# RohanDoshi2018/ZeroshotSemanticSegmentation

Hardware: AMD Instinct MI355X
Metric: train_Mpixels_per_sec (higher is better)
Workload: dtype bf16; 1 GPU; PASCAL-Context 512x512 phase 1: FCN32s (the reference has no FCN8s) + 300-d pixel projection, 512x512, K=59 (49 seen / 10 unseen), Adam lr 1e-5, train step fwd+cosine loss+infer_lbl+bwd+optimizer; per_gpu_batch=8, global_batch=8, head=fused-from-coarse, parallelism=dp1

## Files before the change

include/szn.h:

```cpp
#ifndef SZN_H_
#define SZN_H_
#include <stddef.h>
#include <stdint.h>
#ifdef __cplusplus
extern "C" {
#endif

typedef void* szn_stream_t;

enum { SZN_OK = 0, SZN_ERR_ARG = -1, SZN_ERR_LAUNCH = -2, SZN_ERR_UNSUPPORTED = -3 };
enum { SZN_F32 = 0, SZN_BF16 = 1, SZN_F16 = 2, SZN_BF16X3 = 3 };

#define SZN_MAX_CLASSES 256
typedef struct szn_class_set {
    uint64_t w[4];
} szn_class_set;

const char* szn_last_error(void);
const char* szn_last_kernel(void);
const char* szn_prev_kernel(void);
int szn_version(void);
int szn_knob_count(void);
const char* szn_knob_name(int i);
typedef struct {
    char name[128];
    char arch[32];
    int compute_units;
    int wavefront;
    int lds_bytes_per_block;
    int64_t hbm_bytes;
    int clock_mhz;
} szn_device_info_t;
int szn_device_info(int device, szn_device_info_t* out );
int szn_stream_create_cu_mask(int n_words, const uint32_t* mask , szn_stream_t* out );
int szn_stream_destroy(szn_stream_t stream);

typedef struct szn_call_result {
    int colsum_rows;
    float work_fraction;
} szn_call_result_t;

typedef struct {
    int dtype;
    int B, Hi, Wi, Ci;
    int Ho, Wo, Co;
    int KH, KW, pad;
    int ldi, ldo, ldg;
    int relu;
    int out_f32;
    void* workspace;
    size_t workspace_bytes;
    float* colsum;
    void* pool_out;
    float* colsum_slab;
    int colsum_slab_rows;
    void* pool_code;
    int pool_only;
    int cb_on;
    int cb_rect[4];
    int cb_const[4];
    int reserved_cus;
    void* dw_lp;
    int dw_lp_dtype;
    szn_call_result_t* result;
} szn_conv_desc_t;

int szn_conv2d_fwd(const szn_conv_desc_t* d, const void* in, const void* w, const float* bias,
                   const void* gate, const float* chan_scale, void* out, szn_stream_t stream);

int szn_pack_weight_dgrad(int dtype, int Co, int KH, int KW, int Ci, const void* w, void* wT,
                          szn_stream_t stream);
int szn_pack_weight_dgrad_batch(int dtype, int n, const void* const* w, void* const* wT, const int* Co, const int* K,
                                const int* Ci, szn_stream_t stream);

int szn_conv2d_dgrad(const szn_conv_desc_t* d, const void* dout, const void* wT, const void* gate,
                     const float* chan_scale, void* din, szn_stream_t stream);
int szn_conv2d_dgrad_border_region(const szn_conv_desc_t* d, int region[8]);
int szn_conv2d_dgrad_border_finish(const szn_conv_desc_t* d, const void* dout, const void* wT, const void* gate,
                                   const float* skip_sum, float* colsum, void* workspace, szn_stream_t stream);

size_t szn_conv2d_dgrad_gemm_workspace_bytes(const szn_conv_desc_t* d);
int szn_conv2d_dgrad_gemm(const szn_conv_desc_t* d, const void* dout, const void* wG, void* din,
                          szn_stream_t stream);
int szn_conv2d_dgrad_gemm_native_supported(const szn_conv_desc_t* d);
size_t szn_conv2d_dgrad_gemm_native_workspace_bytes(const szn_conv_desc_t* d);
int szn_conv2d_dgrad_gemm_native(const szn_conv_desc_t* d, const void* dout, const void* w, void* din,
                                 szn_stream_t stream);

int szn_conv2d_wgrad(const szn_conv_desc_t* d, const void* in, const void* dout, float* dw,
                     int accumulate, szn_stream_t stream);
typedef struct szn_adam_args {
    float* param; float* exp_avg; float* exp_avg_sq;
    void* w_lp; int w_lp_dtype;
    float lr, beta1, beta2, eps, weight_decay;
    int step;
    float grad_scale;
    int grad_optional;
} szn_adam_args_t;
int szn_conv2d_wgrad_adam_supported(const szn_conv_desc_t* d);
int szn_conv2d_wgrad_adam(const szn_conv_desc_t* d, const void* x, const void* dout, float* dw,
                          const szn_adam_args_t* opt, szn_stream_t stream);

int szn_bias_grad(int dtype, long M, int Co, int ldd, const void* dout, float* db, int accumulate,
                  szn_stream_t stream);
int szn_bias_grad_slab(int dtype, long M, int Co, int ldd, const void* dout, float* db, int accumulate,
                       float* colsum_slab, int colsum_slab_rows, int* colsum_rows_out , szn_stream_t stream);
int szn_colsum_reduce_batch(int n, const float* const* slabs, const int* rows, const int* C, float* const* out,
                            szn_stream_t stream);

int szn_gemm_proj_fwd(int dtype, long M, int K, int N, int ldo, const void* x, const void* w,
                      const float* bias, float* out_f32, szn_stream_t stream);
int szn_gemm_proj_dgrad(int dtype, long M, int K, int N, int ldd, const void* dout, const void* wT,
                        const void* gate, const float* chan_scale, void* dx, szn_stream_t stream);
int szn_gemm_proj_wgrad(int dtype, long M, int K, int N, int ldd, const void* x, const void* dout,
                        float* dw, int accumulate, szn_stream_t stream);

int szn_conv1_1_fwd(int dtype, int B, int H, int W, int pad, const float* x_nchw, const float* w,
                    const float* bias, void* out, szn_stream_t stream);
int szn_conv1_1_fwd_c(int dtype, int B, int H, int W, int pad, const float* x_nchw, const float* w,
                      const float* bias, void* out, const int cut[8], szn_stream_t stream);
int szn_conv1_1_wgrad_c(int dtype, int B, int H, int W, int pad, const float* x_nchw, const void* dout, float* dw,
                        int accumulate, void* workspace, const int cut[8], szn_stream_t stream);
size_t szn_conv1_1_wgrad_workspace_bytes(int dtype, int B, int H, int W, int pad);
int szn_conv1_1_wgrad(int dtype, int B, int H, int W, int pad, const float* x_nchw,
                      const void* dout, float* dw, float* db, int accumulate, void* workspace,
                      szn_stream_t stream);
int szn_conv1_1_wgrad_reads(int dtype, int B, int H, int W, int pad, int rect[4]);

int szn_maxpool2x2_ceil_fwd(int dtype, int B, int Hi, int Wi, int C, const void* in, void* out,
                            szn_stream_t stream);
int szn_maxpool2x2_ceil_bwd(int dtype, int B, int Hi, int Wi, int C, const void* in,
                            const void* out, const void* dout, void* din, float* colsum ,
                            float* colsum_slab , int colsum_slab_rows,
                            int* colsum_rows_out , szn_stream_t stream);
int szn_maxpool2x2_ceil_fwd_code(int dtype, int B, int Hi, int Wi, int C, const void* in, void* out, void* code ,
                                 szn_stream_t stream);
int szn_maxpool2x2_ceil_bwd_code(int dtype, int B, int Hi, int Wi, int C, const void* code, const void* dout, void* din,
                                 float* colsum, float* colsum_slab, int colsum_slab_rows, int* colsum_rows_out, szn_stream_t stream);
int szn_maxpool2x2_ceil_bwd_code_gather(int dtype, int B, int Hi, int Wi, int C, const void* code, const void* dsrc, int Hs, int Ws,
                                        const int* ytab, const int* xtab, void* din, float* colsum, float* colsum_slab,
                                        int colsum_slab_rows, int* colsum_rows_out, szn_stream_t stream);
int szn_maxpool2x2_ceil_bwd_code_cb(int dtype, int B, int Hi, int Wi, int C, const void* code, const void* dout, void* din,
                                    float* colsum, float* colsum_slab, int colsum_slab_rows, int* colsum_rows_out, const int* skip_regions,
                                    int n_regions, float* skip_sum, float* skip_slab, szn_stream_t stream);
int szn_conv2d_wgrad_cb_region(const szn_conv_desc_t* d, int region[8]);

int szn_bilinear_up32_crop_fwd(int B, int h, int w, int E, int ldc, int c0, int H, int W, int crop,
                               const float* coarse, float* score_nchw, szn_stream_t stream);
int szn_bilinear_up32_crop_bwd(int B, int h, int w, int E, int ldc, int c0, int H, int W, int crop,
                               const float* dscore_nchw, float* dcoarse, szn_stream_t stream);

int szn_bilinear_up_crop_fwd(int stride, int B, int h, int w, int E, int ldc, int c0, int H, int W, int crop,
                             const float* coarse, float* score_nchw, szn_stream_t stream);
int szn_bilinear_up_crop_bwd(int stride, int B, int h, int w, int E, int ldc, int c0, int H, int W, int crop,
                             const float* dscore_nchw, float* dcoarse, szn_stream_t stream);
int szn_bilinear_up2_nhwc_fwd(int B, int h, int w, int C, int ld, const float* in, float* out, szn_stream_t stream);
int szn_bilinear_up2_nhwc_bwd(int B, int h, int w, int C, int ld, const float* dout, float* din, szn_stream_t stream);

int szn_deconv64s32_fwd(int B, int h, int w, int C, int ldc, int c0, int H, int W, int crop,
                        const float* coarse, const float* weight, float* out_nchw,
                        szn_stream_t stream);
int szn_deconv64s32_dgrad(int B, int h, int w, int C, int ldc, int c0, int H, int W, int crop,
                          const float* dout_nchw, const float* weight, float* dcoarse,
                          szn_stream_t stream);
int szn_deconv64s32_wgrad(int B, int h, int w, int C, int ldc, int c0, int H, int W, int crop,
                          const float* coarse, const float* dout_nchw, float* dweight,
                          int accumulate, szn_stream_t stream);

size_t szn_seenmask_head_workspace_bytes(int B, int h, int w, int H, int W, int crop);
int szn_seenmask_head(int B, int h, int w, int ldc, int c0, int H, int W, int crop, const float* coarse,
                      const float* weight, const int64_t* target, int n_class, uint64_t seen_bits, float* loss,
                      float* stats, int64_t* conf, int64_t* pred, float* dscore2, float* dweight, void* workspace,
                      szn_stream_t stream);
int szn_seenmask_head_k(int B, int h, int w, int ldc, int c0, int H, int W, int crop, const float* coarse,
                        const float* weight, const int64_t* target, int n_class, const szn_class_set* seen, float* loss,
                        float* stats, int64_t* conf, int64_t* pred, float* dscore2, float* dweight, void* workspace,
                        szn_stream_t stream);
int szn_seenmask_margin(int B, int h, int w, int ldc, int c0, int H, int W, int crop,
                        const float* coarse, const float* weight, float* margin, szn_stream_t stream);
size_t szn_seenmask_score_wgrad_workspace_bytes(long M, int F);
int szn_seenmask_score_wgrad(int dtype, long M, int F, int ldf, const void* feat, const float* dscore2, float* dw,
                             float* db, void* workspace, szn_stream_t stream);

size_t szn_loss_workspace_bytes(int B, int H, int W);
int szn_cosine_loss_fwd(int B, int E, int H, int W, int K, const float* score,
                        const int64_t* target, const float* embed, const float* target_embed,
                        float* loss, float* stats, void* workspace, szn_stream_t stream);
int szn_cosine_loss_bwd(int B, int E, int H, int W, int K, const float* score,
                        const int64_t* target, const float* embed, const float* target_embed,
                        const float* stats, const float* gout, float* dscore, szn_stream_t stream);
int szn_mse_loss_fwd(int B, int E, int H, int W, int K, const float* score, const int64_t* target,
                     const float* embed, const float* target_embed, float* loss, float* stats,
                     void* workspace, szn_stream_t stream);
int szn_mse_loss_bwd(int B, int E, int H, int W, int K, const float* score, const int64_t* target,
                     const float* embed, const float* target_embed, const float* stats,
                     const float* gout, float* dscore, szn_stream_t stream);
int szn_ce2d_fwd(int B, int C, int H, int W, const float* score, const int64_t* target, const float* weight,
                 int size_average, float* loss, float* stats, int64_t* pred, void* workspace, szn_stream_t stream);
int szn_ce2d_bwd(int B, int C, int H, int W, const float* score, const int64_t* target, const float* weight,
                 int size_average, const float* stats, const float* gout, float* dscore, szn_stream_t stream);

int szn_embed_argmax(int B, int E, int H, int W, int K, const float* score, const float* embed,
                     int mode, uint64_t unseen_bits, const float* seenmask, const int64_t* target,
                     int64_t* pred, szn_stream_t stream);
int szn_embed_argmax_k(int B, int E, int H, int W, int K, const float* score, const float* embed,
                       int mode, const szn_class_set* unseen, const float* seenmask, const int64_t* target,
                       int64_t* pred, szn_stream_t stream);

int szn_confusion_hist(long npix, int K, const int64_t* label_true, const int64_t* label_pred,
                       uint64_t unseen_bits, int64_t* hist, szn_stream_t stream);
int szn_confusion_hist_k(long npix, int K, const int64_t* label_true, const int64_t* label_pred,
                         const szn_class_set* unseen, int64_t* hist, szn_stream_t stream);

size_t szn_fused_head_workspace_bytes(int B, int h, int w, int E, int K);
int szn_fused_head(int B, int h, int w, int E, int ldc, int c0, int H, int W, int crop, int K,
                   const float* coarse, const float* embed, const int64_t* target,
                   float* loss, float* stats, int64_t* pred, int dcoarse_dtype, void* dcoarse,
                   void* workspace, szn_stream_t stream);
int szn_fused_head_strided(int stride, int B, int h, int w, int E, int ldc, int c0, int H, int W, int crop, int K,
                           const float* coarse, const float* embed, const int64_t* target, float* loss, float* stats,
                           int64_t* pred, int dcoarse_dtype, void* dcoarse, void* workspace, szn_stream_t stream);
int szn_fused_head_prepare(int E, int K, const float* embed, void* workspace, szn_stream_t stream);
int szn_fused_head_prepared(int stride, int B, int h, int w, int E, int ldc, int c0, int H, int W, int crop, int K,
                            const float* coarse, const float* embed, const int64_t* target, float* loss, float* stats,
                            int64_t* pred, int dcoarse_dtype, void* dcoarse, void* workspace, szn_stream_t stream);
int szn_fused_head_grouped(int stride, int B, int h, int w, int E, int ldc, int c0, int H, int W, int crop, int K,
                           const float* coarse, const float* embed, const int64_t* target, const szn_class_set* unseen,
                           int group_mode, const int64_t* group_map, float* loss, float* stats, int64_t* pred,
                           int dcoarse_dtype, void* dcoarse, void* workspace, szn_stream_t stream);
// ... 161 lines not shown
```

zeroshotsemanticsegmentation_amd/_lib.py:

```python
import ctypes as C
import os

import torch

_HERE = os.path.dirname(os.path.abspath(__file__))
LIB_PATH = os.environ.get("SZN_LIB_PATH") or os.path.join(_HERE, "lib", "libszn_hip.so")

SZN_F32, SZN_BF16, SZN_F16 = 0, 1, 2
SZN_BF16X3 = 3


class SznError(RuntimeError):
    pass


class CallResult(C.Structure):
    _fields_ = [("colsum_rows", C.c_int), ("work_fraction", C.c_float)]


class ConvDesc(C.Structure):
    _fields_ = [(n, C.c_int) for n in (
        "dtype", "B", "Hi", "Wi", "Ci", "Ho", "Wo", "Co", "KH", "KW", "pad", "ldi", "ldo", "ldg", "relu", "out_f32")] + [
        ("workspace", C.c_void_p), ("workspace_bytes", C.c_size_t), ("colsum", C.c_void_p), ("pool_out", C.c_void_p),
        ("colsum_slab", C.c_void_p), ("colsum_slab_rows", C.c_int), ("pool_code", C.c_void_p), ("pool_only", C.c_int),
        ("cb_on", C.c_int), ("cb_rect", C.c_int * 4), ("cb_const", C.c_int * 4), ("reserved_cus", C.c_int),
        ("dw_lp", C.c_void_p), ("dw_lp_dtype", C.c_int), ("result", C.POINTER(CallResult))]

    def __init__(self, *a, **kw):
        super().__init__(*a, **kw)
        self.res = CallResult(0, 1.0)
        self.result = C.pointer(self.res)


class DeviceInfo(C.Structure):
    _fields_ = [("name", C.c_char * 128), ("arch", C.c_char * 32), ("compute_units", C.c_int),
                ("wavefront", C.c_int), ("lds_bytes_per_block", C.c_int), ("hbm_bytes", C.c_int64),
                ("clock_mhz", C.c_int)]


class AdamArgs(C.Structure):
    _fields_ = [("param", C.c_void_p), ("exp_avg", C.c_void_p), ("exp_avg_sq", C.c_void_p), ("w_lp", C.c_void_p),
                ("w_lp_dtype", C.c_int), ("lr", C.c_float), ("beta1", C.c_float), ("beta2", C.c_float), ("eps", C.c_float),
                ("weight_decay", C.c_float), ("step", C.c_int), ("grad_scale", C.c_float), ("grad_optional", C.c_int)]


MAX_CLASSES = 256
AUG_NPARAM = 9


class ClassSet(C.Structure):
    _fields_ = [("w", C.c_uint64 * 4)]


def class_set(classes):
    cs = ClassSet()
    any_ = False
    for k in classes or []:
        k = int(k)
        if not 0 <= k < MAX_CLASSES:
            raise SznError("class index %d outside [0, %d)" % (k, MAX_CLASSES))
        cs.w[k >> 6] |= 1 << (k & 63)
        any_ = True
    return C.byref(cs) if any_ else None


MS_MAX_VIEWS = 16
CALIB_MAX_GAMMAS = 64
SEEN_SWEEP_MAX_TAUS = 64
PSEUDO_BINS = 1024
OHEM_BINS = 1024


class MsView(C.Structure):
    _fields_ = [("coarse", C.c_void_p)] + [(n, C.c_int) for n in ("h", "w", "ldc", "c0", "Hs", "Ws", "flip")]


_P, _I, _L, _F, _U64, _SZ, _I64 = C.c_void_p, C.c_int, C.c_long, C.c_float, C.c_uint64, C.c_size_t, C.c_int64
_D = C.POINTER(ConvDesc)
_IP = C.POINTER(C.c_int)
_CS = C.POINTER(ClassSet)
_MV = C.POINTER(MsView)
_FP = C.POINTER(C.c_float)

SIGNATURES = {
    "szn_last_error": (C.c_char_p, []),
    "szn_last_kernel": (C.c_char_p, []),
    "szn_prev_kernel": (C.c_char_p, []),
    "szn_version": (_I, []),
    "szn_knob_count": (_I, []),
    "szn_knob_name": (C.c_char_p, [_I]),
    "szn_device_info": (_I, [_I, C.POINTER(DeviceInfo)]),
    "szn_stream_create_cu_mask": (_I, [_I, C.POINTER(C.c_uint32), C.POINTER(C.c_void_p)]),
    "szn_stream_destroy": (_I, [C.c_void_p]),
    "szn_conv2d_fwd": (_I, [_D, _P, _P, _P, _P, _P, _P, _P]),
    "szn_pack_weight_dgrad": (_I, [_I, _I, _I, _I, _I, _P, _P, _P]),
    "szn_pack_weight_dgrad_batch": (_I, [_I, _I, _P, _P, _P, _P, _P, _P]),
    "szn_conv2d_dgrad": (_I, [_D, _P, _P, _P, _P, _P, _P]),
    "szn_conv2d_dgrad_border_region": (_I, [_D, _P]),
    "szn_conv2d_dgrad_border_finish": (_I, [_D, _P, _P, _P, _P, _P, _P, _P]),
    "szn_conv2d_dgrad_gemm_workspace_bytes": (C.c_size_t, [_D]),
    "szn_conv2d_dgrad_gemm": (_I, [_D, _P, _P, _P, _P]),
    "szn_conv2d_dgrad_gemm_native_supported": (_I, [_D]),
    "szn_conv2d_dgrad_gemm_native_workspace_bytes": (C.c_size_t, [_D]),
    "szn_conv2d_dgrad_gemm_native": (_I, [_D, _P, _P, _P, _P]),
    "szn_conv2d_wgrad": (_I, [_D, _P, _P, _P, _I, _P]),
    "szn_conv2d_wgrad_adam_supported": (_I, [_D]),
    "szn_conv2d_wgrad_adam": (_I, [_D, _P, _P, _P, C.POINTER(AdamArgs), _P]),
    "szn_bias_grad": (_I, [_I, _L, _I, _I, _P, _P, _I, _P]),
    "szn_bias_grad_slab": (_I, [_I, _L, _I, _I, _P, _P, _I, _P, _I, _IP, _P]),
    "szn_colsum_reduce_batch": (_I, [_I, _P, _P, _P, _P, _P]),
    "szn_gemm_proj_fwd": (_I, [_I, _L, _I, _I, _I, _P, _P, _P, _P, _P]),
    "szn_gemm_proj_dgrad": (_I, [_I, _L, _I, _I, _I, _P, _P, _P, _P, _P, _P]),
    "szn_gemm_proj_wgrad": (_I, [_I, _L, _I, _I, _I, _P, _P, _P, _I, _P]),
    "szn_conv1_1_fwd": (_I, [_I, _I, _I, _I, _I, _P, _P, _P, _P, _P]),
    "szn_conv1_1_fwd_c": (_I, [_I, _I, _I, _I, _I, _P, _P, _P, _P, _P, _P]),
    "szn_conv1_1_wgrad_c": (_I, [_I, _I, _I, _I, _I, _P, _P, _P, _I, _P, _P, _P]),
    "szn_conv1_1_wgrad_workspace_bytes": (_SZ, [_I, _I, _I, _I, _I]),
    "szn_conv1_1_wgrad": (_I, [_I, _I, _I, _I, _I, _P, _P, _P, _P, _I, _P, _P]),
    "szn_conv1_1_wgrad_reads": (_I, [_I, _I, _I, _I, _I, C.POINTER(C.c_int)]),
    "szn_maxpool2x2_ceil_fwd": (_I, [_I, _I, _I, _I, _I, _P, _P, _P]),
    "szn_maxpool2x2_ceil_bwd": (_I, [_I, _I, _I, _I, _I, _P, _P, _P, _P, _P, _P, _I, _IP, _P]),
    "szn_maxpool2x2_ceil_fwd_code": (_I, [_I, _I, _I, _I, _I, _P, _P, _P, _P]),
    "szn_maxpool2x2_ceil_bwd_code": (_I, [_I, _I, _I, _I, _I, _P, _P, _P, _P, _P, _I, _IP, _P]),
    "szn_maxpool2x2_ceil_bwd_code_gather": (_I, [_I, _I, _I, _I, _I, _P, _P, _I, _I, _P, _P, _P, _P, _P, _I, _IP, _P]),
    "szn_maxpool2x2_ceil_bwd_code_cb": (_I, [_I, _I, _I, _I, _I, _P, _P, _P, _P, _P, _I, _IP, _P, _I, _P, _P, _P]),
    "szn_conv2d_wgrad_cb_region": (_I, [_D, _P]),
    "szn_bilinear_up32_crop_fwd": (_I, [_I] * 9 + [_P, _P, _P]),
    "szn_bilinear_up32_crop_bwd": (_I, [_I] * 9 + [_P, _P, _P]),
    "szn_bilinear_up_crop_fwd": (_I, [_I] * 10 + [_P, _P, _P]),
    "szn_bilinear_up_crop_bwd": (_I, [_I] * 10 + [_P, _P, _P]),
    "szn_bilinear_up2_nhwc_fwd": (_I, [_I] * 5 + [_P, _P, _P]),
    "szn_bilinear_up2_nhwc_bwd": (_I, [_I] * 5 + [_P, _P, _P]),
    "szn_deconv64s32_fwd": (_I, [_I] * 9 + [_P, _P, _P, _P]),
    "szn_deconv64s32_dgrad": (_I, [_I] * 9 + [_P, _P, _P, _P]),
    "szn_deconv64s32_wgrad": (_I, [_I] * 9 + [_P, _P, _P, _I, _P]),
    "szn_seenmask_head_workspace_bytes": (_SZ, [_I] * 6),
    "szn_seenmask_head": (_I, [_I] * 8 + [_P, _P, _P, _I, _U64] + [_P] * 8),
    "szn_seenmask_head_k": (_I, [_I] * 8 + [_P, _P, _P, _I, _CS] + [_P] * 8),
    "szn_seenmask_margin": (_I, [_I] * 8 + [_P, _P, _P, _P]),
    "szn_seenmask_score_wgrad_workspace_bytes": (_SZ, [_L, _I]),
    "szn_seenmask_score_wgrad": (_I, [_I, _L, _I, _I, _P, _P, _P, _P, _P, _P]),
    "szn_loss_workspace_bytes": (_SZ, [_I, _I, _I]),
    "szn_cosine_loss_fwd": (_I, [_I] * 5 + [_P] * 8),
    "szn_cosine_loss_bwd": (_I, [_I] * 5 + [_P] * 8),
    "szn_mse_loss_fwd": (_I, [_I] * 5 + [_P] * 8),
    "szn_mse_loss_bwd": (_I, [_I] * 5 + [_P] * 8),
    "szn_ce2d_fwd": (_I, [_I] * 4 + [_P, _P, _P, _I, _P, _P, _P, _P, _P]),
    "szn_ce2d_bwd": (_I, [_I] * 4 + [_P, _P, _P, _I, _P, _P, _P, _P]),
    "szn_embed_argmax": (_I, [_I] * 5 + [_P, _P, _I, _U64, _P, _P, _P, _P]),
    "szn_embed_argmax_k": (_I, [_I] * 5 + [_P, _P, _I, _CS, _P, _P, _P, _P]),
    "szn_confusion_hist": (_I, [_L, _I, _P, _P, _U64, _P, _P]),
    "szn_confusion_hist_k": (_I, [_L, _I, _P, _P, _CS, _P, _P]),
    "szn_fused_head_workspace_bytes": (_SZ, [_I] * 5),
    "szn_fused_head": (_I, [_I] * 10 + [_P] * 6 + [_I, _P, _P, _P]),
    "szn_fused_head_strided": (_I, [_I] * 11 + [_P] * 6 + [_I, _P, _P, _P]),
    "szn_fused_head_prepare": (_I, [_I, _I, _P, _P, _P]),
    "szn_fused_head_prepared": (_I, [_I] * 11 + [_P] * 6 + [_I, _P, _P, _P]),
    "szn_fused_head_grouped": (_I, [_I] * 11 + [_P, _P, _P, _CS, _I, _P, _P, _P, _P, _I, _P, _P, _P]),
    "szn_fused_head_grouped_prepared": (_I, [_I] * 11 + [_P, _P, _P, _CS, _I, _P, _P, _P, _P, _I, _P, _P, _P]),
    "szn_fused_mse_head": (_I, [_I] * 11 + [_P, _P, _P, _CS, _I, _P, _P, _P, _P, _I, _P, _P, _P]),
    "szn_fused_mse_head_prepared": (_I, [_I] * 11 + [_P, _P, _P, _CS, _I, _P, _P, _P, _P, _I, _P, _P, _P]),
    "szn_fused_simce_head": (_I, [_I] * 11 + [_P, _P, _P, _CS, _I, _P, _CS, _F, _P, _P, _P, _I, _P, _P, _P]),
    "szn_fused_simce_head_prepared": (_I, [_I] * 11 + [_P, _P, _P, _CS, _I, _P, _CS, _F, _P, _P, _P, _I, _P, _P, _P]),
    "szn_fused_rank_head": (_I, [_I] * 11 + [_P, _P, _P, _CS, _I, _P, _CS, _F, _I, _P, _P, _P, _I, _P, _P, _P]),
    "szn_fused_rank_head_prepared": (_I, [_I] * 11 + [_P, _P, _P, _CS, _I, _P, _CS, _F, _I, _P, _P, _P, _I, _P, _P, _P]),
    "szn_fused_simce_bias_head": (_I, [_I] * 11 + [_P, _P, _P, _CS, _I, _P, _CS, _F, _CS, _F, _I64, _P, _P, _P, _I, _P, _P, _P]),
    "szn_fused_simce_bias_head_prepared": (_I, [_I] * 11 + [_P, _P, _P, _CS, _I, _P, _CS, _F, _CS, _F, _I64, _P, _P, _P, _I, _P, _P, _P]),
    "szn_fused_ce_head_workspace_bytes": (_SZ, [_I] * 5),
    "szn_fused_ce_head": (_I, [_I] * 10 + [_P, _P, _P, _I, _P, _P, _P, _I, _P, _P, _P]),
    "szn_adam_step": (_I, [_L, _P, _P, _P, _P, _F, _F, _F, _F, _F, _I, _F, _P, _I, _P]),
    "szn_sgd_momentum_step": (_I, [_L, _P, _P, _P, _F, _F, _F, _I, _F, _P, _I, _P]),
    "szn_adam_step_g16": (_I, [_L, _P, _P, _I, _P, _P, _F, _F, _F, _F, _F, _I, _F, _P, _I, _P]),
    "szn_sgd_momentum_step_g16": (_I, [_L, _P, _P, _I, _P, _F, _F, _F, _I, _F, _P, _I, _P]),
    "szn_grad_check_finite": (_I, [_L, _P, _P, _P]),
    "szn_adam_step_scaled": (_I, [_L, _P, _P, _P, _P, _F, _F, _F, _F, _F, _P, _F, _P, _I, _P]),
    "szn_sgd_momentum_step_scaled": (_I, [_L, _P, _P, _P, _F, _F, _F, _P, _F, _P, _I, _P]),
    "szn_loss_scale_update": (_I, [_P, _F, _F, _I, _F, _F, _P]),
    "szn_cast": (_I, [_I, _I, _L, _P, _P, _P]),
    "szn_band_remap": (_I, [_I, _I, _I, _I, _I, _I, _I, _P, _P, _P, _P, _P]),
    "szn_band_fold": (_I, [_I, _I, _I, _I, _I, _P, _I, _P, _I, _P]),
    "szn_dropout2d_mask": (_I, [_L, _F, _U64, _U64, _P, _P]),
    "szn_proj_fp8_workspace_bytes": (_SZ, [_L, _I, _I]),
    "szn_proj_fp8_fwd": (_I, [_I, _I, _L, _I, _I, _I, _P, _P, _P, _P, _P, _P]),
    "szn_proj_fp8_bwd_workspace_bytes": (_SZ, [_L, _I, _I]),
    "szn_proj_fp8_dgrad": (_I, [_I, _I, _L, _I, _I, _I, _P, _P, _P, _I, _I, _P, _I, _I, _P, _I, _P, _P]),
    "szn_proj_fp8_wgrad": (_I, [_I, _I, _L, _I, _I, _I, _I, _P, _P, _P, _P, _P]),
    "szn_image_u8_to_bgr_f32": (_I, [_I, _I, _I, _P, C.POINTER(C.c_double), _P, _P]),
    "szn_augment_u8": (_I, [_I, _I, _I, _P, _P, _P, C.POINTER(C.c_double), _I, _I, _P, _P, _P]),
    "szn_resize_flip_f32": (_I, [_I, _I, _I, _P, _I, _I, _I, _P, _P]),
    "szn_ms_head_workspace_bytes": (_SZ, [_I, _I, _I, _I, _I, _MV]),
    "szn_ms_head": (_I, [_I] * 8 + [_MV, _P, _CS, _I, _P, _P, _P, _P, _P, _P]),
    "szn_calib_head_workspace_bytes": (_SZ, [_I] * 7),
    "szn_calib_head": (_I, [_I] * 11 + [_P, _P, _P, _CS, _I, _FP, _P, _I, _P, _P, _P]),
    "szn_seen_sweep_head_workspace_bytes": (_SZ, [_I] * 7),
    "szn_seen_sweep_head": (_I, [_I] * 11 + [_P, _P, _P, _CS, _P, _I, _FP, _P, _I, _P, _P, _P]),
    "szn_seen_sweep_head_tabled": (_I, [_I] * 11 + [_P, _P, _P, _CS, _P, _I, _FP, _P, _I, _P, _P, _P]),
    "szn_pseudo_head_workspace_bytes": (_SZ, [_I] * 8),
    "szn_pseudo_head": (_I, [_I] * 11 + [_P, _P, _P, _CS, _F, _F, _I, _I64] + [_P] * 8),
    "szn_ohem_head_workspace_bytes": (_SZ, [_I] * 8),
    "szn_ohem_head": (_I, [_I] * 11 + [_P, _P, _P, _CS, _I, _F, _I64] + [_P] * 7),
    "szn_viz_segmentation": (_I, [_I, _I, _I, _P, _I, C.POINTER(C.c_double), _P, _P, _I, _CS, _U64, _P, _L, _L, _P]),
    "szn_viz_seenmask": (_I, [_I, _I, _I, _P, _I, C.POINTER(C.c_double), _P, _P, _U64, _P, _L, _L, _P]),
}

_lib = None


def load():
    global _lib
    if _lib is not None:
        return _lib
    if not os.path.exists(LIB_PATH):
        raise SznError("libszn_hip.so not found at %s -- run `python -c 'import __graft_entry__ as g; g.build()'` "
                       "(the product path has no CPU fallback)" % LIB_PATH)
    lib = C.CDLL(LIB_PATH)
    for name, (res, args) in SIGNATURES.items():
        fn = getattr(lib, name)
        fn.restype = res
        fn.argtypes = args
    _lib = lib
    return lib


def check(rc, what):
    if rc != 0:
        raise SznError("%s failed (%d): %s" % (what, rc, load().szn_last_error().decode()))


def last_kernel():
    return load().szn_last_kernel().decode()


def rows_out():
    return C.c_int(0)


def prev_kernel():
    return load().szn_prev_kernel().decode()


def stream_ptr():
    return C.c_void_p(torch.cuda.current_stream().cuda_stream)


def ptr(t):
    if t is None:
        return None
    return C.c_void_p(t.data_ptr())


# ... 15 lines not shown
```

zeroshotsemanticsegmentation_amd/csrc/szn_conv.hip:

```cpp
#include "szn_common.h"

typedef __attribute__((ext_vector_type(4))) uint32_t u32x4_t;
typedef __attribute__((ext_vector_type(2))) uint32_t u32x2_t;

namespace {

template <typename T> struct Mma;
template <> struct Mma<bf16_raw> {
    static __device__ __forceinline__ u32x4_t frag(const u32x4_t& f) { return f; }
    static __device__ __forceinline__ void run(f32x4_t& acc, const u32x4_t& a, const u32x4_t& b) {
        acc = __builtin_amdgcn_mfma_f32_16x16x32_bf16(__builtin_bit_cast(bf16x8_t, a),
                                                      __builtin_bit_cast(bf16x8_t, b), acc, 0, 0, 0);
    }
};
template <> struct Mma<f16_raw> {
    static __device__ __forceinline__ u32x4_t frag(const u32x4_t& f) { return f; }
    static __device__ __forceinline__ void run(f32x4_t& acc, const u32x4_t& a, const u32x4_t& b) { acc = mfma16<f16_raw>(a, b, acc); }
};
template <> struct Mma<float> {
    static __device__ __forceinline__ u32x4_t frag(const u32x4_t& f) { return f; }
    static __device__ __forceinline__ void run(f32x4_t& acc, const u32x4_t& a, const u32x4_t& b) {
        acc = __builtin_amdgcn_mfma_f32_16x16x4f32(__uint_as_float(a.x), __uint_as_float(b.x), acc, 0, 0, 0);
        acc = __builtin_amdgcn_mfma_f32_16x16x4f32(__uint_as_float(a.y), __uint_as_float(b.y), acc, 0, 0, 0);
        acc = __builtin_amdgcn_mfma_f32_16x16x4f32(__uint_as_float(a.z), __uint_as_float(b.z), acc, 0, 0, 0);
// ... 424 lines not shown
template <typename T>
__global__ __launch_bounds__(256) void bias_grad_kernel(const T* __restrict__ dout, float* __restrict__ db, long M, int Co,
                                                        int ldd, int rows_per_block, float* __restrict__ slab) {
    constexpr int CH = elem<T>::kPer16B;
    __shared__ float red[256 * CH];
    const int cpr = (Co + CH - 1) / CH;
    const long r0 = (long)blockIdx.x * rows_per_block;
    const long r1 = min(M, r0 + rows_per_block);
    for (int cg = 0; cg < cpr; cg += 256) {
        const int ncg = min(256, cpr - cg);
        const int rl = 256 / ncg;
        const int chunk = threadIdx.x % ncg, lr = threadIdx.x / ncg;
        float acc[CH];
#pragma unroll
        for (int e = 0; e < CH; ++e) acc[e] = 0.f;
        if (lr < rl) {
            const T* p = dout + (long)(cg + chunk) * CH;
            for (long r = r0 + lr; r < r1; r += rl) {
                const u32x4_t v = *(const u32x4_t*)(p + r * ldd);
                const T* ve = (const T*)&v;
#pragma unroll
                for (int e = 0; e < CH; ++e) acc[e] += elem<T>::ld(ve + e);
            }
        }
        __syncthreads();
        if (lr < rl) {
#pragma unroll
            for (int e = 0; e < CH; ++e) red[(lr * ncg + chunk) * CH + e] = acc[e];
        }
        __syncthreads();
        for (int i = threadIdx.x; i < ncg * CH; i += 256) {
            float s = 0.f;
            for (int l = 0; l < rl; ++l) s += red[l * ncg * CH + i];
            const int n = cg * CH + i;
            if (n < Co) {
                if (slab) slab[(long)blockIdx.x * Co + n] = s;
                else if (s != 0.f) atomicAdd(db + n, s);
            }
        }
    }
}

template <typename T>
int launch_conv(const ConvArgs& a, hipStream_t st) {
    const size_t lds = 4 * OPB;
    static bool attr_done = false;
    if (!attr_done) {
        (void)hipFuncSetAttribute((const void*)conv_igemm<T>, hipFuncAttributeMaxDynamicSharedMemorySize, (int)lds);
        attr_done = true;
    }
    hipLaunchKernelGGL(conv_igemm<T>, dim3(a.mtiles * a.ntiles), dim3(256), lds, st, a);
    SZN_CHECK_LAUNCH((std::is_same<T, f32x3_t>::value ? "conv_igemm+bf16x3" : "conv_igemm"));
    return SZN_OK;
}

int check_desc(const szn_conv_desc_t* d) {
    if (!d) SZN_FAIL(SZN_ERR_ARG, "conv: null descriptor");
    if (!szn_store_f32(d->dtype) && !szn_is16(d->dtype)) SZN_FAIL(SZN_ERR_ARG, "conv: bad dtype %d", d->dtype);
    if (d->B <= 0 || d->Hi <= 0 || d->Wi <= 0 || d->Ci <= 0 || d->Co <= 0 || d->KH <= 0 || d->KW <= 0 || d->pad < 0)
        SZN_FAIL(SZN_ERR_ARG, "conv: non-positive dimension");
    if (d->Ho != d->Hi + 2 * d->pad - d->KH + 1 || d->Wo != d->Wi + 2 * d->pad - d->KW + 1 || d->Ho <= 0 || d->Wo <= 0)
        SZN_FAIL(SZN_ERR_ARG, "conv: Ho/Wo (%d,%d) inconsistent with Hi/Wi (%d,%d) pad %d k %dx%d", d->Ho, d->Wo, d->Hi,
                 d->Wi, d->pad, d->KH, d->KW);
    if ((long)d->B * d->Ho * d->Wo >= (1L << 31) || (long)d->B * d->Hi * d->Wi >= (1L << 31))
        SZN_FAIL(SZN_ERR_UNSUPPORTED, "conv: more than 2^31 pixels");
    return SZN_OK;
}

}

int szn_conv2d_fwd_v1(const szn_conv_desc_t* d, const void* in, const void* w, const float* bias, const void* gate,
                      const float* chan_scale, void* out, szn_stream_t stream) {
    int rc = check_desc(d);
    if (rc) return rc;
    const int bke = szn_is16(d->dtype) ? 64 : 32;
    if (d->Ci % bke) SZN_FAIL(SZN_ERR_UNSUPPORTED, "conv2d_fwd: Ci=%d must be a multiple of %d", d->Ci, bke);
    if (d->ldi < d->Ci || d->ldo < d->Co || (d->ldi % (bke / 8)))
        SZN_FAIL(SZN_ERR_ARG, "conv2d_fwd: bad pixel strides ldi=%d ldo=%d", d->ldi, d->ldo);
    if (!in || !w || !out) SZN_FAIL(SZN_ERR_ARG, "conv2d_fwd: null pointer");
    if (((uintptr_t)in | (uintptr_t)w | (uintptr_t)out) & 15) SZN_FAIL(SZN_ERR_ARG, "conv2d_fwd: pointers must be 16-B aligned");
    ConvArgs a;
    a.in = (const char*)in; a.w = (const char*)w; a.bias = bias; a.gate = (const char*)gate; a.cscale = chan_scale;
    a.out = (char*)out;
    a.B = d->B; a.Hi = d->Hi; a.Wi = d->Wi; a.Ci = d->Ci; a.Ho = d->Ho; a.Wo = d->Wo; a.Co = d->Co;
    a.KH = d->KH; a.KW = d->KW; a.pad = d->pad; a.ldi = d->ldi; a.ldo = d->ldo; a.ldg = d->ldg;
    a.relu = d->relu; a.out_f32 = d->out_f32;
    a.M = d->B * d->Ho * d->Wo; a.HoWo = d->Ho * d->Wo;
    a.mtiles = szn_div_up(a.M, TILE); a.ntiles = szn_div_up(a.Co, TILE);
    rc = d->dtype == SZN_BF16 ? launch_conv<bf16_raw>(a, (hipStream_t)stream)
       : d->dtype == SZN_F16 ? launch_conv<f16_raw>(a, (hipStream_t)stream)
       : d->dtype == SZN_BF16X3 ? launch_conv<f32x3_t>(a, (hipStream_t)stream) : launch_conv<float>(a, (hipStream_t)stream);
    if (rc || !d->colsum) return rc;
    if (d->out_f32 && szn_is16(d->dtype)) SZN_FAIL(SZN_ERR_UNSUPPORTED, "conv2d_fwd(v1): colsum with out_f32 is unsupported");
    return szn_bias_grad_slab(szn_store_f32(d->dtype) ? SZN_F32 : d->dtype, a.M, d->Co, d->ldo, out, d->colsum, 1, d->colsum_slab,
                              d->colsum_slab_rows, nullptr, stream);
}

extern "C" int szn_pack_weight_dgrad(int dtype, int Co, int KH, int KW, int Ci, const void* w, void* wT,
                                     szn_stream_t stream) {
    if (!w || !wT || Co <= 0 || Ci <= 0 || KH <= 0 || KW <= 0) SZN_FAIL(SZN_ERR_ARG, "pack_weight_dgrad: bad argument");
    dim3 grid(szn_div_up(Ci, 32), szn_div_up(Co, 32), KH * KW);
    if (szn_is16(dtype) && (Co & 7) == 0 && (Ci & 63) == 0 && !(((uintptr_t)w | (uintptr_t)wT) & 15)) {
        hipLaunchKernelGGL(pack_dgrad16_kernel, dim3(Ci / 64, (Co + 63) / 64, KH * KW), dim3(256), 0, (hipStream_t)stream,
                           (const uint16_t*)w, (uint16_t*)wT, Co, KH, KW, Ci);
        SZN_CHECK_LAUNCH("pack_dgrad16_kernel");
        return SZN_OK;
    }
    if (szn_is16(dtype))
        hipLaunchKernelGGL(pack_dgrad_kernel<uint16_t>, grid, dim3(256), 0, (hipStream_t)stream, (const uint16_t*)w,
                           (uint16_t*)wT, Co, KH, KW, Ci);
    else if (szn_store_f32(dtype))
        hipLaunchKernelGGL(pack_dgrad_kernel<float>, grid, dim3(256), 0, (hipStream_t)stream, (const float*)w, (float*)wT,
                           Co, KH, KW, Ci);
    else
        SZN_FAIL(SZN_ERR_ARG, "pack_weight_dgrad: bad dtype %d", dtype);
    SZN_CHECK_LAUNCH("pack_dgrad_kernel");
    return SZN_OK;
}

extern "C" int szn_pack_weight_dgrad_batch(int dtype, int n, const void* const* w, void* const* wT, const int* Co, const int* K,
                                           const int* Ci, szn_stream_t stream) {
    if (n <= 0 || !w || !wT || !Co || !K || !Ci) SZN_FAIL(SZN_ERR_ARG, "pack_weight_dgrad_batch: bad argument");
    if (!szn_is16(dtype)) SZN_FAIL(SZN_ERR_UNSUPPORTED, "pack_weight_dgrad_batch: 16-bit images only (use szn_pack_weight_dgrad)");
    if (n > kPackMax) SZN_FAIL(SZN_ERR_UNSUPPORTED, "pack_weight_dgrad_batch: at most %d layers per call", kPackMax);
    PackBatch pb;
    long blocks = 0;
    for (int i = 0; i < n; ++i) {
        if (!w[i] || !wT[i] || Co[i] <= 0 || K[i] <= 0 || Ci[i] <= 0) SZN_FAIL(SZN_ERR_ARG, "pack_weight_dgrad_batch: bad item %d", i);
        if ((Co[i] & 63) || (Ci[i] & 63) || (((uintptr_t)w[i] | (uintptr_t)wT[i]) & 15))
            SZN_FAIL(SZN_ERR_UNSUPPORTED, "pack_weight_dgrad_batch: item %d needs Co, Ci multiples of 64 and 16-B aligned images", i);
        pb.it[i].w = (const uint16_t*)w[i]; pb.it[i].wT = (uint16_t*)wT[i];
        pb.it[i].Co = Co[i]; pb.it[i].K = K[i]; pb.it[i].Ci = Ci[i]; pb.it[i].block0 = (int)blocks;
        blocks += (long)(Ci[i] / 64) * (Co[i] / 64) * K[i] * K[i];
        if (blocks > 0x7fffffffL) SZN_FAIL(SZN_ERR_UNSUPPORTED, "pack_weight_dgrad_batch: too many tiles");
    }
    pb.n = n;
    hipLaunchKernelGGL(pack_dgrad16_batch_kernel, dim3((unsigned)blocks), dim3(256), 0, (hipStream_t)stream, pb);
    SZN_CHECK_LAUNCH("pack_dgrad16_batch_kernel");
    return SZN_OK;
}

extern "C" int szn_conv2d_dgrad(const szn_conv_desc_t* d, const void* dout, const void* wT, const void* gate,
                                const float* chan_scale, void* din, szn_stream_t stream) {
    int rc = check_desc(d);
    if (rc) return rc;
    szn_conv_desc_t s = *d;
    s.Hi = d->Ho; s.Wi = d->Wo; s.Ci = d->Co;
    s.Ho = d->Hi; s.Wo = d->Wi; s.Co = d->Ci;
    s.pad = d->KH - 1 - d->pad;
    if (d->KH != d->KW || s.pad < 0) SZN_FAIL(SZN_ERR_UNSUPPORTED, "conv2d_dgrad: needs a square kernel with pad <= K-1");
    s.ldi = d->ldo; s.ldo = d->ldi;
    s.relu = 0;
    return szn_conv2d_fwd(&s, dout, wT, nullptr, gate, chan_scale, din, stream);
}

template <typename T>
__global__ __launch_bounds__(256) void col2im_kernel(const float* __restrict__ Y, T* __restrict__ din, int B, int Hi, int Wi,
                                                     int Ci, int Ho, int Wo, int KH, int KW, int pad, int ldi) {
    const int c4n = Ci >> 2;
    const long total = (long)B * Hi * Wi * c4n;
    const long N = (long)KH * KW * Ci;
    for (long idx = (long)blockIdx.x * 256 + threadIdx.x; idx < total; idx += (long)gridDim.x * 256) {
        const int c4 = (int)(idx % c4n);
        const long p = idx / c4n;
        const int iw = (int)(p % Wi);
        const long t = p / Wi;
        const int ih = (int)(t % Hi), b = (int)(t / Hi);
        const int kh0 = max(0, ih + pad - (Ho - 1)), kh1 = min(KH - 1, ih + pad);
        const int kw0 = max(0, iw + pad - (Wo - 1)), kw1 = min(KW - 1, iw + pad);
        f32x4_t acc = {0.f, 0.f, 0.f, 0.f};
        for (int kh = kh0; kh <= kh1; ++kh) {
            const int oh = ih + pad - kh;
            const float* yrow = Y + (((long)b * Ho + oh) * Wo + (iw + pad)) * N + (long)kh * KW * Ci + c4 * 4;
            f32x4_t a0 = {0.f, 0.f, 0.f, 0.f}, a1 = a0;
            int kw = kw0;
#pragma unroll 4
            for (; kw + 1 <= kw1; kw += 2) {
                a0 += *(const f32x4_t*)(yrow - (long)kw * N + (long)kw * Ci);
                a1 += *(const f32x4_t*)(yrow - (long)(kw + 1) * N + (long)(kw + 1) * Ci);
            }
            if (kw <= kw1) a0 += *(const f32x4_t*)(yrow - (long)kw * N + (long)kw * Ci);
            acc += a0 + a1;
        }
        T* o = din + p * ldi + c4 * 4;
#pragma unroll
        for (int e = 0; e < 4; ++e) elem<T>::st(o + e, acc[e]);
    }
}

static int launch_col2im(const szn_conv_desc_t* d, const float* Y, void* din, szn_stream_t stream);
int szn_conv_wgrad_wide_try(const szn_conv_desc_t* d, const void* in, const void* dout, float* dw, int accumulate,
                            int min_tiles, szn_stream_t stream, const szn_adam_args_t* opt = nullptr);

extern "C" size_t szn_conv2d_dgrad_gemm_workspace_bytes(const szn_conv_desc_t* d) {
    if (!d || d->B <= 0 || d->Ho <= 0 || d->Wo <= 0 || d->KH <= 0 || d->KW <= 0 || d->Ci <= 0) return 0;
    return (size_t)d->B * d->Ho * d->Wo * d->KH * d->KW * d->Ci * sizeof(float);
}

extern "C" int szn_conv2d_dgrad_gemm(const szn_conv_desc_t* d, const void* dout, const void* wG, void* din,
                                     szn_stream_t stream) {
    int rc = check_desc(d);
    if (rc) return rc;
    if (!dout || !wG || !din) SZN_FAIL(SZN_ERR_ARG, "conv2d_dgrad_gemm: null pointer");
    if (d->Ci & 3) SZN_FAIL(SZN_ERR_UNSUPPORTED, "conv2d_dgrad_gemm: Ci must be a multiple of 4");
    const size_t need = szn_conv2d_dgrad_gemm_workspace_bytes(d);
    if (!d->workspace || d->workspace_bytes < need || ((uintptr_t)d->workspace & 15))
        SZN_FAIL(SZN_ERR_ARG, "conv2d_dgrad_gemm: needs a 16-B aligned workspace of %zu bytes", need);
    if (d->B * d->Ho >= 32000 || d->Wo >= 32000) SZN_FAIL(SZN_ERR_UNSUPPORTED, "conv2d_dgrad_gemm: map too large");
    const long N = (long)d->KH * d->KW * d->Ci;
    if (N >= (1L << 31)) SZN_FAIL(SZN_ERR_UNSUPPORTED, "conv2d_dgrad_gemm: KH*KW*Ci too large");
    szn_conv_desc_t g = {};
    g.dtype = d->dtype; g.B = 1; g.Hi = d->B * d->Ho; g.Wi = d->Wo; g.Ci = d->Co;
    g.Ho = g.Hi; g.Wo = g.Wi; g.Co = (int)N; g.KH = 1; g.KW = 1; g.pad = 0;
    g.ldi = d->ldo; g.ldo = (int)N; g.ldg = 0; g.relu = 0; g.out_f32 = 1;
    g.workspace = nullptr; g.workspace_bytes = 0; g.colsum = nullptr;
    rc = szn_conv2d_fwd(&g, dout, wG, nullptr, nullptr, nullptr, d->workspace, stream);
    if (rc) return rc;
    return launch_col2im(d, (const float*)d->workspace, din, stream);
}

static int launch_col2im(const szn_conv_desc_t* d, const float* Y, void* din, szn_stream_t stream) {
    const long total = (long)d->B * d->Hi * d->Wi * (d->Ci >> 2);
    long blocks = (total + 255) / 256;
    if (blocks > 65536) blocks = 65536;
    if (d->dtype == SZN_BF16)
        hipLaunchKernelGGL(col2im_kernel<bf16_raw>, dim3((unsigned)blocks), dim3(256), 0, (hipStream_t)stream,
                           Y, (bf16_raw*)din, d->B, d->Hi, d->Wi, d->Ci, d->Ho, d->Wo, d->KH, d->KW,
                           d->pad, d->ldi);
    else if (d->dtype == SZN_F16)
        hipLaunchKernelGGL(col2im_kernel<f16_raw>, dim3((unsigned)blocks), dim3(256), 0, (hipStream_t)stream,
                           Y, (f16_raw*)din, d->B, d->Hi, d->Wi, d->Ci, d->Ho, d->Wo, d->KH, d->KW,
                           d->pad, d->ldi);
    else
        hipLaunchKernelGGL(col2im_kernel<float>, dim3((unsigned)blocks), dim3(256), 0, (hipStream_t)stream,
                           Y, (float*)din, d->B, d->Hi, d->Wi, d->Ci, d->Ho, d->Wo, d->KH, d->KW,
                           d->pad, d->ldi);
    SZN_CHECK_LAUNCH("col2im_kernel");
    return SZN_OK;
}

__global__ __launch_bounds__(256) void transpose_pad16_kernel(const uint16_t* __restrict__ src, uint16_t* __restrict__ dst, int M, int Mp,
                                                              int C) {
    __shared__ uint16_t tile[64][66];
    const int m0 = blockIdx.y * 64, c0 = blockIdx.x * 64;
    const int c8 = threadIdx.x & 7, r0 = threadIdx.x >> 3;
#pragma unroll
    for (int p = 0; p < 2; ++p) {
        const int r = r0 + 32 * p;
        uint4 v = make_uint4(0u, 0u, 0u, 0u);
        if (m0 + r < M) v = *(const uint4*)(src + (long)(m0 + r) * C + c0 + c8 * 8);
        uint32_t* d32 = (uint32_t*)&tile[r][c8 * 8];
        d32[0] = v.x; d32[1] = v.y; d32[2] = v.z; d32[3] = v.w;
    }
    __syncthreads();
#pragma unroll
    for (int p = 0; p < 2; ++p) {
        const int c = r0 + 32 * p;
        uint32_t o[4];
#pragma unroll
        for (int e = 0; e < 4; ++e)
            o[e] = (uint32_t)tile[c8 * 8 + 2 * e][c] | ((uint32_t)tile[c8 * 8 + 2 * e + 1][c] << 16);
        if (m0 + c8 * 8 < Mp) *(uint4*)(dst + (long)(c0 + c) * Mp + m0 + c8 * 8) = make_uint4(o[0], o[1], o[2], o[3]);
    }
}

static bool dgrad_native_shape_ok(const szn_conv_desc_t* d) {
    if (!d || !szn_is16(d->dtype) || d->KH != d->KW || d->ldo != d->Co || (d->Ci & 3)) return false;
    const long M = (long)d->B * d->Ho * d->Wo, N = (long)d->KH * d->KW * d->Ci;
    if (M < 256 || N < 256 || (N & 7) || (d->Co & 63) || M >= (1L << 22) || N >= (1L << 31)) return false;
    const long cot = (M + 255) / 256, cit = (N + 255) / 256;
    if (cot * cit < 96) return false;
    if (cot * 256 * cit * 256 > M * N * 5 / 4 && cot * cit > 256) return false;
    return (size_t)d->Co * N * 2 < 0xffff0000ul && (size_t)d->Co * M * 2 < 0xffff0000ul;
}

extern "C" int szn_conv2d_dgrad_gemm_native_supported(const szn_conv_desc_t* d) { return dgrad_native_shape_ok(d) ? 1 : 0; }

extern "C" size_t szn_conv2d_dgrad_gemm_native_workspace_bytes(const szn_conv_desc_t* d) {
    const size_t y = szn_conv2d_dgrad_gemm_workspace_bytes(d);
    if (!y) return 0;
    const size_t Mp = ((size_t)d->B * d->Ho * d->Wo + 7) / 8 * 8;
    return (y + 255) / 256 * 256 + (size_t)d->Co * Mp * 2;
}

extern "C" int szn_conv2d_dgrad_gemm_native(const szn_conv_desc_t* d, const void* dout, const void* w, void* din,
                                            szn_stream_t stream) {
    int rc = check_desc(d);
    if (rc) return rc;
    if (!dout || !w || !din) SZN_FAIL(SZN_ERR_ARG, "conv2d_dgrad_gemm_native: null pointer");
    if (!dgrad_native_shape_ok(d)) SZN_FAIL(SZN_ERR_UNSUPPORTED, "conv2d_dgrad_gemm_native: shape not supported (use szn_conv2d_dgrad_gemm)");
    const size_t need = szn_conv2d_dgrad_gemm_native_workspace_bytes(d);
    if (!d->workspace || d->workspace_bytes < need || ((uintptr_t)d->workspace & 15))
        SZN_FAIL(SZN_ERR_ARG, "conv2d_dgrad_gemm_native: needs a 16-B aligned workspace of %zu bytes", need);
    const int M = d->B * d->Ho * d->Wo;
    const long N = (long)d->KH * d->KW * d->Ci;
    float* Y = (float*)d->workspace;
    void* doutT = (char*)d->workspace + (szn_conv2d_dgrad_gemm_workspace_bytes(d) + 255) / 256 * 256;
    const int Mp = (M + 7) / 8 * 8;
    if (Mp == M) {
        rc = szn_pack_weight_dgrad(d->dtype, M, 1, 1, d->Co, dout, doutT, stream);
        if (rc) return rc;
    } else {
        if ((uintptr_t)dout & 15) SZN_FAIL(SZN_ERR_ARG, "conv2d_dgrad_gemm_native: dout must be 16-B aligned");
        hipLaunchKernelGGL(transpose_pad16_kernel, dim3(d->Co / 64, (Mp + 63) / 64), dim3(256), 0, (hipStream_t)stream, (const uint16_t*)dout,
                           (uint16_t*)doutT, M, Mp, d->Co);
        SZN_CHECK_LAUNCH("transpose_pad16_kernel");
// ... 111 lines not shown
```

zeroshotsemanticsegmentation_amd/csrc/szn_conv1_1_wgrad.hip:

```cpp
#include "szn_common.h"
#include "szn_cb.h"

typedef __attribute__((ext_vector_type(4))) uint32_t u32x4_t;
typedef __attribute__((ext_vector_type(2))) uint32_t u32x2_t;
typedef __attribute__((address_space(3))) void* ldsptr_t;

namespace {

struct C11Args {
    const char* dout; const float* x; float* ws;
    unsigned dout_bytes, x_bytes;
    int B, H, W, pad, Ho, Wo;
    int oh_lo, nrows, seg_lo, nsegx;
    long nseg;
    BandCut cut;
    int Hc, Wc;
};

constexpr unsigned kOOB1 = 0x80000000u;
constexpr int RING1 = 3;

constexpr int PS1 = 36;
constexpr int PATCH1 = 9 * PS1 * 4;

// ... 73 lines not shown
#pragma unroll
        for (int k = 0; k < 5; ++k) {
            const int idx = lane + 64 * k;
            const int row = (idx * 1928) >> 16;
            const int c = idx - row * 34;
            const int ci = (row * 11) >> 5, kh = row - ci * 3;
            const int ih = oh + kh - a.pad, iw = ow0 + c - a.pad;
            const bool ok = idx < 306 && (unsigned)ih < (unsigned)a.H && (unsigned)iw < (unsigned)a.W;
            const unsigned off = ok ? (((unsigned)(b * 3 + ci)) * plane + (unsigned)(ih * a.W + iw)) * 4u : kOOB1;
            xr[k] = __uint_as_float(__builtin_amdgcn_raw_buffer_load_b32(rsX, off, 0, 0));
        }
    };
    auto stage_store = [&](const float (&xr)[5]) {
#pragma unroll
        for (int k = 0; k < 5; ++k) {
            const int idx = lane + 64 * k;
            const int row = (idx * 1928) >> 16;
            if (idx < 306) patch[row * PS1 + (idx - row * 34)] = xr[k];
        }
    };
    int poff[2];
#pragma unroll
    for (int f = 0; f < 2; ++f) {
        const int t = r16 + 16 * f;
        poff[f] = t < 27 ? ((int)tci[f] * 3 + t / 9) * PS1 + tkw[f] + 4 * g : -1;
    }
    auto patch_read = [&](float (&xv)[2][8]) {
#pragma unroll
        for (int f = 0; f < 2; ++f) {
            const float* pp = patch + (poff[f] < 0 ? 0 : poff[f]);
#pragma unroll
            for (int e = 0; e < 8; ++e) {
                const float v = pp[e < 4 ? e : 16 + e - 4];
                xv[f][e] = poff[f] < 0 ? 0.f : v;
            }
        }
    };

    f32x4_t acc[4][2];
#pragma unroll
    for (int i = 0; i < 4; ++i)
#pragma unroll
        for (int f = 0; f < 2; ++f) acc[i][f] = f32x4_t{0.f, 0.f, 0.f, 0.f};

    const long nwaves = (long)gridDim.x * 4;
    const long s0 = (long)blockIdx.x * 4 + w;
    if constexpr (STAGED) {
        float xr[5] = {0.f, 0.f, 0.f, 0.f, 0.f};
        if (s0 < a.nseg) { issue_dma(s0, 0); stage_load(s0, xr); }
        if (s0 + nwaves < a.nseg) issue_dma(s0 + nwaves, 1);
        int stage = 0;
        for (long s = s0; s < a.nseg; s += nwaves) {
            stage_store(xr);
            float xn[2][8];
            patch_read(xn);
            u32x4_t xf[2];
#pragma unroll
            for (int f = 0; f < 2; ++f) {
                xf[f].x = pack2<T>(xn[f][0], xn[f][1]);
                xf[f].y = pack2<T>(xn[f][2], xn[f][3]);
                xf[f].z = pack2<T>(xn[f][4], xn[f][5]);
                xf[f].w = pack2<T>(xn[f][6], xn[f][7]);
            }
            const bool more1 = s + nwaves < a.nseg, more2 = s + 2 * nwaves < a.nseg;
            if (more1) stage_load(s + nwaves, xr);
            if (more2) issue_dma(s + 2 * nwaves, stage >= 1 ? stage - 1 : 2);
            if (more2) asm volatile("s_waitcnt vmcnt(13)" ::: "memory");
            else if (more1) asm volatile("s_waitcnt vmcnt(9)" ::: "memory");
            else asm volatile("s_waitcnt vmcnt(0)" ::: "memory");
            const char* sb = ring + stage * 4096;
            u32x4_t df[4];
#pragma unroll
            for (int i = 0; i < 4; ++i) {
                const bf16x4_t lo = __builtin_amdgcn_ds_read_tr16_b64_v4bf16((lp_t)(sb + offA[i]));
                const bf16x4_t hi = __builtin_amdgcn_ds_read_tr16_b64_v4bf16((lp_t)(sb + 2048 + offA[i]));
                const u32x2_t l2 = __builtin_bit_cast(u32x2_t, lo), h2 = __builtin_bit_cast(u32x2_t, hi);
                df[i] = u32x4_t{l2.x, l2.y, h2.x, h2.y};
            }
#pragma unroll
            for (int i = 0; i < 4; ++i)
#pragma unroll
                for (int f = 0; f < 2; ++f)
                    acc[i][f] = mfma16<T>(df[i], xf[f], acc[i][f]);
            asm volatile("s_waitcnt lgkmcnt(0)" ::: "memory");
            stage = stage == 2 ? 0 : stage + 1;
        }
    } else {
    float xn[2][8];
    if (s0 < a.nseg) { issue_dma(s0, 0); gather(s0, xn); }
    if (s0 + nwaves < a.nseg) issue_dma(s0 + nwaves, 1);
    int stage = 0;
    for (long s = s0; s < a.nseg; s += nwaves) {
        u32x4_t xf[2];
#pragma unroll
        for (int f = 0; f < 2; ++f) {
            xf[f].x = pack2<T>(xn[f][0], xn[f][1]);
            xf[f].y = pack2<T>(xn[f][2], xn[f][3]);
            xf[f].z = pack2<T>(xn[f][4], xn[f][5]);
            xf[f].w = pack2<T>(xn[f][6], xn[f][7]);
        }
        const bool more1 = s + nwaves < a.nseg, more2 = s + 2 * nwaves < a.nseg;
        if (more1) gather(s + nwaves, xn);
        if (more2) issue_dma(s + 2 * nwaves, stage >= 1 ? stage - 1 : 2);
        if (more2) asm volatile("s_waitcnt vmcnt(24)" ::: "memory");
        else if (more1) asm volatile("s_waitcnt vmcnt(20)" ::: "memory");
        else asm volatile("s_waitcnt vmcnt(0)" ::: "memory");
        const char* sb = ring + stage * 4096;
        u32x4_t df[4];
#pragma unroll
        for (int i = 0; i < 4; ++i) {
            const bf16x4_t lo = __builtin_amdgcn_ds_read_tr16_b64_v4bf16((lp_t)(sb + offA[i]));
            const bf16x4_t hi = __builtin_amdgcn_ds_read_tr16_b64_v4bf16((lp_t)(sb + 2048 + offA[i]));
            const u32x2_t l2 = __builtin_bit_cast(u32x2_t, lo), h2 = __builtin_bit_cast(u32x2_t, hi);
            df[i] = u32x4_t{l2.x, l2.y, h2.x, h2.y};
        }
#pragma unroll
        for (int i = 0; i < 4; ++i)
#pragma unroll
            for (int f = 0; f < 2; ++f)
                acc[i][f] = mfma16<T>(df[i], xf[f], acc[i][f]);
        asm volatile("s_waitcnt lgkmcnt(0)" ::: "memory");
        stage = stage == 2 ? 0 : stage + 1;
    }
    }

    __syncthreads();
    float* red = (float*)smem;
#pragma unroll
    for (int i = 0; i < 4; ++i)
#pragma unroll
        for (int f = 0; f < 2; ++f)
#pragma unroll
            for (int e = 0; e < 4; ++e) red[(w * 64 + 16 * i + 4 * g + e) * 32 + 16 * f + r16] = acc[i][f][e];
    __syncthreads();
    float* slab = a.ws + (size_t)blockIdx.x * 2048;
    for (int idx = tid; idx < 2048; idx += 256)
        slab[idx] = (red[idx] + red[2048 + idx]) + (red[4096 + idx] + red[6144 + idx]);
#endif
}

__global__ __launch_bounds__(256) void conv1_1_wgrad_reduce(const float* __restrict__ ws, float* __restrict__ dw, int nblocks,
                                                            int accumulate) {
    const int i = blockIdx.x * 8 + (threadIdx.x >> 5), l = threadIdx.x & 31;
    const bool ok = i < 64 * 27;
    const int co = ok ? i / 27 : 0, t = ok ? i - co * 27 : 0;
    float s = 0.f;
    if (ok)
        for (int b = l; b < nblocks; b += 32) s += ws[(size_t)b * 2048 + co * 32 + t];
#pragma unroll
    for (int d = 16; d >= 1; d >>= 1) s += __shfl_xor(s, d, 32);
    if (ok && l == 0) dw[i] = accumulate ? dw[i] + s : s;
}

}

static bool c11_geometry(int dtype, int B, int H, int W, int pad, int& oh_lo, int& oh_hi, int& seg_lo, int& seg_hi) {
    if (!szn_is16(dtype) || B <= 0 || H <= 0 || W <= 0 || pad < 0) return false;
    const int Ho = H + 2 * pad - 2, Wo = W + 2 * pad - 2;
    const size_t dout_bytes = (size_t)B * Ho * Wo * 128, x_bytes = (size_t)B * 3 * H * W * 4;
    if (Ho <= 0 || Wo <= 0 || dout_bytes >= 0x7fff0000ul || x_bytes >= 0x7fff0000ul) return false;
    oh_lo = pad - 2; if (oh_lo < 0) oh_lo = 0;
    oh_hi = pad + H; if (oh_hi > Ho) oh_hi = Ho;
    int ow_lo = pad - 2; if (ow_lo < 0) ow_lo = 0;
    int ow_hi = pad + W; if (ow_hi > Wo) ow_hi = Wo;
    if (oh_hi <= oh_lo || ow_hi <= ow_lo) return false;
    seg_lo = ow_lo / 32; seg_hi = (ow_hi + 31) / 32;
    return true;
}

extern "C" int szn_conv1_1_wgrad_reads(int dtype, int B, int H, int W, int pad, int rect[4]) {
    if (!rect) return 0;
    const int Ho = H + 2 * pad - 2, Wo = W + 2 * pad - 2;
    rect[0] = 0; rect[1] = Ho; rect[2] = 0; rect[3] = Wo;
    int oh_lo, oh_hi, seg_lo, seg_hi;
    if (!c11_geometry(dtype, B, H, W, pad, oh_lo, oh_hi, seg_lo, seg_hi)) return 0;
    rect[0] = oh_lo; rect[1] = oh_hi; rect[2] = seg_lo * 32; rect[3] = seg_hi * 32 < Wo ? seg_hi * 32 : Wo;
    return (rect[0] > 0 || rect[1] < Ho || rect[2] > 0 || rect[3] < Wo) ? 1 : 0;
}

int szn_conv1_1_wgrad_fused_try(int dtype, int B, int H, int W, int pad, const float* x, const void* dout, float* dw, int accumulate,
                                void* workspace, size_t workspace_bytes, szn_stream_t stream, const int* cutv) {
    const int Ho = H + 2 * pad - 2, Wo = W + 2 * pad - 2;
    int oh_lo, oh_hi, seg_lo, seg_hi;
    if (!c11_geometry(dtype, B, H, W, pad, oh_lo, oh_hi, seg_lo, seg_hi)) return 1;
    C11Args a;
    a.cut = BandCut{0, 0, Ho, Ho, 0, 0, Wo, Wo};
    if (cutv) a.cut = BandCut{cutv[0], cutv[1], cutv[2], cutv[3], cutv[4], cutv[5], cutv[6], cutv[7]};
    a.Hc = Ho - (a.cut.ye - a.cut.ya) - (a.cut.ye2 - a.cut.ya2); a.Wc = Wo - (a.cut.xe - a.cut.xa) - (a.cut.xe2 - a.cut.xa2);
    const size_t dout_bytes = (size_t)B * a.Hc * a.Wc * 128, x_bytes = (size_t)B * 3 * H * W * 4;
    a.dout = (const char*)dout; a.x = x; a.ws = (float*)workspace;
    a.dout_bytes = (unsigned)dout_bytes; a.x_bytes = (unsigned)x_bytes;
    a.B = B; a.H = H; a.W = W; a.pad = pad; a.Ho = Ho; a.Wo = Wo;
    a.oh_lo = oh_lo; a.nrows = oh_hi - oh_lo;
    a.seg_lo = seg_lo; a.nsegx = seg_hi - seg_lo;
    a.nseg = (long)B * a.nrows * a.nsegx;
    long blocks = (a.nseg + 4 * 16 - 1) / (4 * 16);
    if (blocks > 768) blocks = 768;
    if (blocks < 1) blocks = 1;
    if (workspace_bytes < (size_t)blocks * 2048 * sizeof(float)) return 1;
    hipStream_t st = (hipStream_t)stream;
    if (dtype == SZN_F16) hipLaunchKernelGGL((conv1_1_wgrad_kernel<f16_raw, true>), dim3((unsigned)blocks), dim3(256), 0, st, a);
    else hipLaunchKernelGGL((conv1_1_wgrad_kernel<bf16_raw, true>), dim3((unsigned)blocks), dim3(256), 0, st, a);
    SZN_CHECK_LAUNCH("conv1_1_wgrad_kernel");
    hipLaunchKernelGGL(conv1_1_wgrad_reduce, dim3(64 * 27 / 8), dim3(256), 0, st, (const float*)workspace, dw,
                       (int)blocks, accumulate);
    SZN_CHECK_LAUNCH("conv1_1_wgrad_reduce");
    return SZN_OK;
}
```

zeroshotsemanticsegmentation_amd/csrc/szn_conv_igemm.hip:

```cpp
#include "szn_common.h"
#include "szn_epilogue.h"
#include "szn_wide_args.h"

typedef __attribute__((ext_vector_type(4))) uint32_t u32x4_t;
typedef __attribute__((ext_vector_type(2))) uint32_t u32x2_t;
typedef __attribute__((address_space(3))) void* ldsptr_t;

int szn_conv2d_fwd_v1(const szn_conv_desc_t* d, const void* in, const void* w, const float* bias, const void* gate,
                      const float* chan_scale, void* out, szn_stream_t stream);
int szn_proj_stream_try(const szn_conv_desc_t* d, const void* in, const void* w, const float* bias, const void* gate,
                        const float* chan_scale, void* out, int min_tiles, szn_stream_t stream);
int szn_conv_8ph_launch(const void* args, int dtype, int bn, szn_stream_t stream);
int szn_conv_wide_try(const szn_conv_desc_t* d, const void* in, const void* w, const float* bias, const void* gate,
                      const float* chan_scale, void* out, unsigned in_bytes, unsigned w_bytes, int min_tiles,
                      float* ws, int nsplit, int chunks_per_split, szn_stream_t stream);
int szn_conv_regw_try(const szn_conv_desc_t* d, const void* in, const void* w, const float* bias, const void* gate,
                     const float* chan_scale, void* out, int min_tiles, szn_stream_t stream);
#include <stdlib.h>

namespace {

template <typename T> struct Mma2;
template <> struct Mma2<bf16_raw> {
    static __device__ __forceinline__ u32x4_t frag(const u32x4_t& f) { return f; }
    static __device__ __forceinline__ void run(f32x4_t& acc, const u32x4_t& a, const u32x4_t& b) {
        acc = __builtin_amdgcn_mfma_f32_16x16x32_bf16(__builtin_bit_cast(bf16x8_t, a), __builtin_bit_cast(bf16x8_t, b), acc,
                                                      0, 0, 0);
    }
};
template <> struct Mma2<f16_raw> {
    static __device__ __forceinline__ u32x4_t frag(const u32x4_t& f) { return f; }
    static __device__ __forceinline__ void run(f32x4_t& acc, const u32x4_t& a, const u32x4_t& b) { acc = mfma16<f16_raw>(a, b, acc); }
};
template <> struct Mma2<float> {
    static __device__ __forceinline__ u32x4_t frag(const u32x4_t& f) { return f; }
    static __device__ __forceinline__ void run(f32x4_t& acc, const u32x4_t& a, const u32x4_t& b) {
        acc = __builtin_amdgcn_mfma_f32_16x16x4f32(__uint_as_float(a.x), __uint_as_float(b.x), acc, 0, 0, 0);
        acc = __builtin_amdgcn_mfma_f32_16x16x4f32(__uint_as_float(a.y), __uint_as_float(b.y), acc, 0, 0, 0);
        acc = __builtin_amdgcn_mfma_f32_16x16x4f32(__uint_as_float(a.z), __uint_as_float(b.z), acc, 0, 0, 0);
        acc = __builtin_amdgcn_mfma_f32_16x16x4f32(__uint_as_float(a.w), __uint_as_float(b.w), acc, 0, 0, 0);
    }
};

template <> struct Mma2<f32x3_t> {
    static __device__ __forceinline__ u32x4_t frag(const u32x4_t& f) { return x3_split(f); }
    static __device__ __forceinline__ void run(f32x4_t& acc, const u32x4_t& a, const u32x4_t& b) { acc = x3_mma(a, b, acc); }
};

struct Conv2Args {
    const char* in; const char* w; const float* bias; const char* gate; const float* cscale; char* out;
    float* ws;
    float* colsum;
    float* cslab;
    unsigned in_bytes, w_bytes;
    int B, Hi, Wi, Ci, Ho, Wo, Co, KH, KW, pad;
    int ldi, ldo, ldg, relu, out_f32;
    int M, HoWo, mtiles, ntiles, nsplit, chunks_per_split;
    int direct_ep;
};

__device__ __forceinline__ int xcd_remap2(int bid, int nwg) {
    const int q = nwg >> 3, r = nwg & 7, xcd = bid & 7, idx = bid >> 3;
    return (xcd < r ? xcd * (q + 1) : r * (q + 1) + (xcd - r) * q) + idx;
}

constexpr unsigned kOOB = 0x80000000u;

template <typename T, int WNF>
__global__ __launch_bounds__(512, 2) void conv_igemm_v2(Conv2Args a) {
#if defined(__HIP_DEVICE_COMPILE__)
    constexpr int ES = sizeof(T);
    constexpr int BKE = 128 / ES;
    constexpr int BM = 256, BN = 32 * WNF;
    constexpr int STAGE = (BM + BN) * 128;
    constexpr int NB = BN / 64;
    constexpr int LPC = 4 + NB;
    extern __shared__ __attribute__((aligned(16))) char smem[];

    const int tid = threadIdx.x, lane = tid & 63;
    const int w = __builtin_amdgcn_readfirstlane(tid >> 6);
    const int wm = w >> 1, wn = w & 1;
    const int g = lane >> 4, r16 = lane & 15;

    const int nwg = a.mtiles * a.ntiles;
    const int lid = xcd_remap2(blockIdx.x, nwg);
    const int nt = lid % a.ntiles, mt = lid / a.ntiles;
    const int m0 = mt * BM, n0 = nt * BN;
    const int split = blockIdx.y;

    const auto rsA = __builtin_amdgcn_make_buffer_rsrc((void*)a.in, 0, (int)a.in_bytes, 0x00020000);
    const auto rsB = __builtin_amdgcn_make_buffer_rsrc((void*)a.w, 0, (int)a.w_bytes, 0x00020000);

    const int chunkA = (lane & 7) ^ (lane >> 3);
    unsigned baseA[4];
    int ohw[4];
#pragma unroll
    for (int i = 0; i < 4; ++i) {
        const int m = m0 + 32 * w + 8 * i + (lane >> 3);
        if (m < a.M) {
            const int b = m / a.HoWo, r = m - b * a.HoWo;
            const int oh = r / a.Wo, ow = r - oh * a.Wo;
            const int ih0 = oh - a.pad, iw0 = ow - a.pad;
            ohw[i] = (ih0 << 16) | (iw0 & 0xffff);
            const long px = ((long)(b * a.Hi + ih0) * a.Wi + iw0);
            baseA[i] = (unsigned)((px * a.ldi + chunkA * (16 / ES)) * ES);
        } else {
            ohw[i] = 0x7fff7fff;
            baseA[i] = 0;
        }
    }
    unsigned voffB[NB];
#pragma unroll
    for (int i = 0; i < NB; ++i) {
        const int n = n0 + (BN / 8) * w + 8 * i + (lane >> 3);
        voffB[i] = (n < a.Co) ? (unsigned)(((long)n * a.KH * a.KW * a.Ci + chunkA * (16 / ES)) * ES) : kOOB;
    }

    const int cpt = a.Ci / BKE;
    const int kbeg = split * a.chunks_per_split;
    const int kend = min(a.KH * a.KW * cpt, kbeg + a.chunks_per_split);
    const int nK = kend - kbeg;
    int itap = kbeg / cpt, ic = kbeg - itap * cpt;
    unsigned voffA[4];
    auto set_tap = [&]() {
        const int kh = itap / a.KW, kw = itap - kh * a.KW;
        const unsigned tapoff = (unsigned)((kh * a.Wi + kw) * a.ldi * ES);
#pragma unroll
        for (int i = 0; i < 4; ++i) {
            const int ih = (ohw[i] >> 16) + kh, iw = (int)(short)(ohw[i] & 0xffff) + kw;
            const bool ok = (unsigned)ih < (unsigned)a.Hi && (unsigned)iw < (unsigned)a.Wi;
            voffA[i] = ok ? baseA[i] + tapoff : kOOB;
        }
    };
    auto issue = [&](int stage) {
        char* sb = smem + stage * STAGE;
        const int soffA = ic * 128;
        const int soffB = (itap * a.Ci) * ES + ic * 128;
#pragma unroll
        for (int i = 0; i < 4; ++i)
            __builtin_amdgcn_raw_ptr_buffer_load_lds(rsA, (ldsptr_t)(sb + (32 * w + 8 * i) * 128), 16, voffA[i], soffA, 0, 0);
#pragma unroll
        for (int i = 0; i < NB; ++i)
            __builtin_amdgcn_raw_ptr_buffer_load_lds(rsB, (ldsptr_t)(sb + BM * 128 + ((BN / 8) * w + 8 * i) * 128), 16, voffB[i],
                                                     soffB, 0, 0);
        if (++ic == cpt) { ic = 0; ++itap; set_tap(); }
    };

    f32x4_t acc[WNF][4];
#pragma unroll
    for (int i = 0; i < WNF; ++i)
#pragma unroll
        for (int j = 0; j < 4; ++j) acc[i][j] = f32x4_t{0.f, 0.f, 0.f, 0.f};

    set_tap();
    if (nK > 0) issue(0);
    if (nK > 1) issue(1);
    const int offs0 = ((g ^ (r16 & 7)) << 4), offs1 = (((4 + g) ^ (r16 & 7)) << 4);
    int stage = 0;
    for (int kc = 0; kc < nK; ++kc) {
        if (kc + 1 < nK) asm volatile("s_waitcnt vmcnt(%0)" ::"i"(LPC) : "memory");
        else asm volatile("s_waitcnt vmcnt(0)" ::: "memory");
        __builtin_amdgcn_s_barrier();
        const bool fill = kc + 2 < nK;
        const int turn = w >> 1;
        if (fill && turn == 0) issue(stage >= 1 ? stage - 1 : 2);
        const char* sp = smem + stage * STAGE + (wm * 64 + r16) * 128;
        const char* sw = smem + stage * STAGE + BM * 128 + (wn * (BN / 2) + r16) * 128;
#pragma unroll
        for (int s = 0; s < 2; ++s) {
            const int off = s ? offs1 : offs0;
// ... 142 lines not shown
#pragma unroll
            for (int e = 0; e < 8; ++e) red[row0 * BN + cc * 8 + e] = cs[e];
        }
        __syncthreads();
        if (tid < BN && n0 + tid < a.Co) {
            float t = 0.f;
            for (int r = 0; r < 512 / CPR; ++r) t += red[r * BN + tid];
            if (a.cslab) a.cslab[(long)(m0 >> 8) * a.Co + n0 + tid] = t;
            else if (t != 0.f) atomicAdd(a.colsum + n0 + tid, t);
        }
    }
#endif
}

template <typename T>
__global__ __launch_bounds__(256) void splitk_epilogue(const float* __restrict__ ws, Conv2Args a) {
    const long total = (long)a.M * a.Co;
    const T* __restrict__ gate = (const T*)a.gate;
    const bool out32 = a.out_f32 || sizeof(T) == 4;
    const bool v4 = !(a.Co & 3) && !(a.ldo & 3) && (!gate || !(a.ldg & 3)) && !((uintptr_t)ws & 15) &&
                    !((uintptr_t)a.bias & 15) && !((uintptr_t)a.cscale & 15) && !((uintptr_t)a.out & (out32 ? 15 : 7));
    if (v4) {
        const int c4n = a.Co >> 2;
        const long tot4 = total >> 2;
        for (long i4 = (long)blockIdx.x * 256 + threadIdx.x; i4 < tot4; i4 += (long)gridDim.x * 256) {
            const int n = (int)(i4 % c4n) * 4;
            const long m = i4 / c4n;
            f32x4_t x = {0.f, 0.f, 0.f, 0.f};
            for (int sp = 0; sp < a.nsplit; ++sp) x += *(const f32x4_t*)(ws + (long)sp * total + i4 * 4);
            if (a.bias) x += *(const f32x4_t*)(a.bias + n);
            if (a.relu) { x[0] = fmaxf(x[0], 0.f); x[1] = fmaxf(x[1], 0.f); x[2] = fmaxf(x[2], 0.f); x[3] = fmaxf(x[3], 0.f); }
            if (gate) {
#pragma unroll
                for (int e = 0; e < 4; ++e) x[e] = (elem<T>::ld(gate + m * a.ldg + n + e) > 0.f) ? x[e] : 0.f;
            }
            if (a.cscale) x *= *(const f32x4_t*)(a.cscale + (m / a.HoWo) * a.Co + n);
            if (a.out_f32 || sizeof(T) == 4) *(f32x4_t*)((float*)a.out + m * a.ldo + n) = x;
            else {
                uint2 o;
                o.x = pack2<T>(x[0], x[1]); o.y = pack2<T>(x[2], x[3]);
                *(uint2*)((uint16_t*)a.out + m * a.ldo + n) = o;
            }
        }
        return;
    }
    for (long idx = (long)blockIdx.x * 256 + threadIdx.x; idx < total; idx += (long)gridDim.x * 256) {
        const int n = (int)(idx % a.Co);
        const long m = idx / a.Co;
        float x = 0.f;
        for (int sp = 0; sp < a.nsplit; ++sp) x += ws[(long)sp * total + idx];
        if (a.bias) x += a.bias[n];
        if (a.relu) x = fmaxf(x, 0.f);
        if (gate) x = (elem<T>::ld(gate + m * a.ldg + n) > 0.f) ? x : 0.f;
        if (a.cscale) x *= a.cscale[(m / a.HoWo) * a.Co + n];
        if (a.out_f32 || sizeof(T) == 4) ((float*)a.out)[m * a.ldo + n] = x;
        else ((uint16_t*)a.out)[m * a.ldo + n] = to_bits16<T>(x);
    }
}

template <typename T>
__global__ __launch_bounds__(256) void splitk_epilogue_cs(const float* __restrict__ ws, Conv2Args a, int rpb) {
    __shared__ f32x4_t part[256];
    const long total = (long)a.M * a.Co;
    const T* __restrict__ gate = (const T*)a.gate;
    const int c4n = a.Co >> 2, RL = 256 / c4n;
    const int c4 = threadIdx.x % c4n, rl = threadIdx.x / c4n, n = c4 * 4;
    const long m0 = (long)blockIdx.x * rpb, m1 = m0 + rpb < a.M ? m0 + rpb : a.M;
    f32x4_t cs = {0.f, 0.f, 0.f, 0.f};
    auto finish = [&](long m, f32x4_t x, uint2 gq) {
        if (a.bias) x += *(const f32x4_t*)(a.bias + n);
        if (a.relu) { x[0] = fmaxf(x[0], 0.f); x[1] = fmaxf(x[1], 0.f); x[2] = fmaxf(x[2], 0.f); x[3] = fmaxf(x[3], 0.f); }
        if (gate) {
            if (sizeof(T) == 2) {
                const uint16_t g0 = (uint16_t)(gq.x & 0xffffu), g1 = (uint16_t)(gq.x >> 16), g2 = (uint16_t)(gq.y & 0xffffu), g3 = (uint16_t)(gq.y >> 16);
                x[0] = from_bits16<T>(g0) > 0.f ? x[0] : 0.f; x[1] = from_bits16<T>(g1) > 0.f ? x[1] : 0.f;
                x[2] = from_bits16<T>(g2) > 0.f ? x[2] : 0.f; x[3] = from_bits16<T>(g3) > 0.f ? x[3] : 0.f;
            } else {
#pragma unroll
                for (int e = 0; e < 4; ++e) x[e] = (elem<T>::ld(gate + m * a.ldg + n + e) > 0.f) ? x[e] : 0.f;
            }
        }
        if (a.cscale) x *= *(const f32x4_t*)(a.cscale + (m / a.HoWo) * a.Co + n);
        cs += x;
        if (a.out_f32 || sizeof(T) == 4) *(f32x4_t*)((float*)a.out + m * a.ldo + n) = x;
        else {
            uint2 o;
            o.x = pack2<T>(x[0], x[1]); o.y = pack2<T>(x[2], x[3]);
            *(uint2*)((uint16_t*)a.out + m * a.ldo + n) = o;
        }
    };
    long m = m0 + rl;
    for (; m + 3L * RL < m1; m += 4L * RL) {
        f32x4_t x[4];
        uint2 gq[4];
#pragma unroll
        for (int u = 0; u < 4; ++u) {
            const long i4 = (m + (long)u * RL) * c4n + c4;
            x[u] = f32x4_t{0.f, 0.f, 0.f, 0.f};
            for (int sp = 0; sp < a.nsplit; ++sp) x[u] += *(const f32x4_t*)(ws + (long)sp * total + i4 * 4);
            gq[u] = uint2{0u, 0u};
            if (gate && sizeof(T) == 2) gq[u] = *(const uint2*)((const uint16_t*)gate + (m + (long)u * RL) * a.ldg + n);
        }
#pragma unroll
        for (int u = 0; u < 4; ++u) finish(m + (long)u * RL, x[u], gq[u]);
    }
    for (; m < m1; m += RL) {
        const long i4 = m * c4n + c4;
        f32x4_t x = {0.f, 0.f, 0.f, 0.f};
        for (int sp = 0; sp < a.nsplit; ++sp) x += *(const f32x4_t*)(ws + (long)sp * total + i4 * 4);
        uint2 gq = {0u, 0u};
        if (gate && sizeof(T) == 2) gq = *(const uint2*)((const uint16_t*)gate + m * a.ldg + n);
        finish(m, x, gq);
    }
    part[threadIdx.x] = cs;
    __syncthreads();
    if (rl == 0) {
        f32x4_t t = part[c4];
        for (int r = 1; r < RL; ++r) t += part[r * c4n + c4];
        if (a.cslab) *(f32x4_t*)(a.cslab + (long)blockIdx.x * a.Co + n) = t;
        else {
#pragma unroll
            for (int e = 0; e < 4; ++e) if (t[e] != 0.f) atomicAdd(a.colsum + n + e, t[e]);
        }
    }
}

template <typename T, int WNF>
int launch_v2(const Conv2Args& a, hipStream_t st) {
    constexpr int BN = 32 * WNF;
    const size_t lds = 3 * (256 + BN) * 128;
    static bool attr_done = false;
    if (!attr_done) {
        (void)hipFuncSetAttribute((const void*)conv_igemm_v2<T, WNF>, hipFuncAttributeMaxDynamicSharedMemorySize, (int)lds);
        attr_done = true;
    }
    hipLaunchKernelGGL((conv_igemm_v2<T, WNF>), dim3(a.mtiles * a.ntiles, a.nsplit), dim3(512), lds, st, a);
    SZN_CHECK_LAUNCH((std::is_same<T, f32x3_t>::value ? "conv_igemm_v2+bf16x3" : "conv_igemm_v2"));
    return SZN_OK;
}

}

extern "C" int szn_maxpool2x2_ceil_fwd(int dtype, int B, int Hi, int Wi, int C, const void* in, void* out, szn_stream_t stream);
static int conv2d_fwd_dispatch(const szn_conv_desc_t* d, const void* in, const void* w, const float* bias, const void* gate,
                               const float* chan_scale, void* out, szn_stream_t stream, int* pooled);

static int conv2d_fwd_entry(const szn_conv_desc_t* d, const void* in, const void* w, const float* bias,
                            const void* gate, const float* chan_scale, void* out, szn_stream_t stream);
extern "C" int szn_conv2d_fwd(const szn_conv_desc_t* d, const void* in, const void* w, const float* bias,
                              const void* gate, const float* chan_scale, void* out, szn_stream_t stream) {
    if (!d) SZN_FAIL(SZN_ERR_ARG, "conv2d_fwd: null descriptor");
    szn_note_colsum_rows(0);
    szn_note_work_fraction(1.f);
    const int rc = conv2d_fwd_entry(d, in, w, bias, gate, chan_scale, out, stream);
    szn_publish_result(d);
    return rc;
}

static int conv2d_fwd_entry(const szn_conv_desc_t* d, const void* in, const void* w, const float* bias,
                            const void* gate, const float* chan_scale, void* out, szn_stream_t stream) {
    if (d->colsum_slab && ((uintptr_t)d->colsum_slab & 15)) SZN_FAIL(SZN_ERR_ARG, "conv2d: colsum_slab must be 16-B aligned");
    if (d->pool_out && (!d->relu || d->ldo != d->Co || gate || chan_scale))
        SZN_FAIL(SZN_ERR_ARG, "conv2d_fwd: pool_out needs relu, ldo == Co and no gate / chan_scale");
    if ((d->pool_code || d->pool_only) && !d->pool_out) SZN_FAIL(SZN_ERR_ARG, "conv2d_fwd: pool_code / pool_only need pool_out");
    if (d->pool_code && (((uintptr_t)d->pool_code) & 7)) SZN_FAIL(SZN_ERR_ARG, "conv2d_fwd: pool_code must be 8-B aligned");
    int pooled = 0;
    const int rc = conv2d_fwd_dispatch(d, in, w, bias, gate, chan_scale, out, stream, &pooled);
    if (rc || !d->pool_out || pooled) return rc;
    return szn_maxpool2x2_ceil_fwd_code((d->out_f32 || szn_store_f32(d->dtype)) ? SZN_F32 : d->dtype, d->B, d->Ho, d->Wo, d->Co, out,
                                        d->pool_out, d->pool_code, stream);
}

static int conv2d_fwd_dispatch(const szn_conv_desc_t* d, const void* in, const void* w, const float* bias, const void* gate,
                               const float* chan_scale, void* out, szn_stream_t stream, int* pooled) {
    const size_t es = szn_esize(d->dtype);
    const size_t in_bytes = (size_t)d->B * d->Hi * d->Wi * d->ldi * es;
    const size_t w_bytes = (size_t)d->Co * d->KH * d->KW * d->Ci * es;
    const int bke = (int)(128 / es);
    const bool v2_ok = (szn_is16(d->dtype) || szn_store_f32(d->dtype)) && d->Ci > 0 && (d->Ci % bke) == 0 &&
                       in_bytes < 0x7fff0000ul && w_bytes < 0x7fff0000ul && d->Hi < 32000 && d->Wi < 32000 && d->pad < 16000 &&
                       ((size_t)d->ldi * es) % 16 == 0;
    {
        static const int wide_min0 = szn_knob("SZN_WIDE_MINTILES", 240);
        const int rc = szn_proj_stream_try(d, in, w, bias, gate, chan_scale, out, wide_min0, stream);
        if (rc <= 0) return rc;
    }
    if (!v2_ok) return szn_conv2d_fwd_v1(d, in, w, bias, gate, chan_scale, out, stream);
    if (d->B <= 0 || d->Hi <= 0 || d->Wi <= 0 || d->Co <= 0 || d->KH <= 0 || d->KW <= 0 || d->pad < 0 ||
        d->Ho != d->Hi + 2 * d->pad - d->KH + 1 || d->Wo != d->Wi + 2 * d->pad - d->KW + 1 || d->Ho <= 0 || d->Wo <= 0 ||
        d->ldi < d->Ci || d->ldo < d->Co || !in || !w || !out || (((uintptr_t)in | (uintptr_t)w | (uintptr_t)out) & 15) ||
        (long)d->B * d->Ho * d->Wo >= (1L << 31))
        return szn_conv2d_fwd_v1(d, in, w, bias, gate, chan_scale, out, stream);
    hipStream_t st = (hipStream_t)stream;
    if (d->KH == 3 && d->KW == 3 && d->Ci <= 128 && d->Co <= 128) {
        static const int regw_min = szn_knob("SZN_REGW_MINTILES", 128);
        const int rc = szn_conv_regw_try(d, in, w, bias, gate, chan_scale, out, regw_min, stream);
        if (rc == 0 && d->pool_out) *pooled = 1;
        if (rc <= 0) return rc;
    }
    Conv2Args a;
    a.in = (const char*)in; a.w = (const char*)w; a.bias = bias; a.gate = (const char*)gate; a.cscale = chan_scale;
    a.out = (char*)out; a.ws = nullptr; a.colsum = d->colsum;
    a.in_bytes = (unsigned)in_bytes; a.w_bytes = (unsigned)w_bytes;
    a.B = d->B; a.Hi = d->Hi; a.Wi = d->Wi; a.Ci = d->Ci; a.Ho = d->Ho; a.Wo = d->Wo; a.Co = d->Co;
    a.KH = d->KH; a.KW = d->KW; a.pad = d->pad; a.ldi = d->ldi; a.ldo = d->ldo; a.ldg = d->ldg;
    a.relu = d->relu; a.out_f32 = d->out_f32;
    a.M = d->B * d->Ho * d->Wo; a.HoWo = d->Ho * d->Wo;
    {
        static const int de = szn_knob("SZN_IGEMM_DIRECT", 1);
        const size_t oes = d->out_f32 ? 4 : 2;
        const uintptr_t al = (uintptr_t)out | (uintptr_t)gate | (uintptr_t)bias | (uintptr_t)chan_scale;
        a.direct_ep = de && szn_is16(d->dtype) && (d->Co % 8) == 0 && (((size_t)d->ldo * oes) & 15) == 0 && (al & 15) == 0 &&
                      (!gate || (((size_t)d->ldg * 2) & 15) == 0);
    }
    const bool narrow = d->Co <= 64;
    const int BN = narrow ? 64 : 128;
    a.mtiles = szn_div_up(a.M, 256); a.ntiles = szn_div_up(a.Co, BN);
    a.cslab = d->colsum ? d->colsum_slab : nullptr;
    if (a.cslab && d->colsum_slab_rows < a.mtiles) SZN_FAIL(SZN_ERR_ARG, "conv2d: colsum_slab holds %d rows, %d needed", d->colsum_slab_rows, a.mtiles);
    szn_note_colsum_rows(a.cslab ? a.mtiles : 0);
    const int nK = d->KH * d->KW * (d->Ci / bke);
    a.nsplit = 1; a.chunks_per_split = nK;
    const long tiles = (long)a.mtiles * a.ntiles;
    bool use_wide = false;
    const bool out32_ = d->out_f32 || szn_store_f32(d->dtype);
    const int cs_rpb = 32;
    const long cs_rows = ((long)a.M + cs_rpb - 1) / cs_rpb;
    const bool cs_ok = d->colsum && !(d->Co & 3) && (d->Co >> 2) <= 256 && 256 % (d->Co >> 2) == 0 && !(d->ldo & 3) &&
                       (!gate || !(d->ldg & 3)) && !((uintptr_t)d->workspace & 15) && !((uintptr_t)bias & 15) && !((uintptr_t)chan_scale & 15) &&
                       !((uintptr_t)out & (out32_ ? 15 : 7)) && (!d->colsum_slab || d->colsum_slab_rows >= cs_rows) &&
                       (long)a.mtiles * a.ntiles < 128;
    if (d->workspace && nK >= 64 && (!d->colsum || cs_ok)) {
        static int ncu = 0;
        if (!ncu) {
            int dev = 0; hipDeviceProp_t p;
            if (hipGetDevice(&dev) == hipSuccess && hipGetDeviceProperties(&p, dev) == hipSuccess) ncu = p.multiProcessorCount;
            if (ncu <= 0) ncu = 256;
        }
        const double flops = 2.0 * a.M * (double)d->Co * d->Ci * d->KH * d->KW;
        const double slab = (double)a.M * d->Co * 8.0;
        const long wtiles = (long)a.mtiles * szn_div_up(d->Co, 256);
        const bool wide_ok = d->Co >= 256 && (long)szn_div_up(d->Co, 256) * 256 - d->Co <= 64;
        long best = 1; double best_t = 0; bool best_wide = false;
        for (int cand = 0; cand < (wide_ok ? 2 : 1); ++cand) {
            const long tl = cand ? wtiles : tiles;
            const double rate = cand ? 1.15e15 : 0.95e15;
            for (long ns = 1; ns <= 16 && ns <= nK / 8; ++ns) {
                if (ns > 1 && (size_t)ns * a.M * a.Co * sizeof(float) > d->workspace_bytes) break;
                if (cand && ns == 1) continue;
                const long blocks = tl * ns;
                const double eff = (double)blocks / (double)((blocks + ncu - 1) / ncu * ncu);
                const double t = flops / (rate * eff) + (ns > 1 ? ns * slab / 3.0e12 + 5e-6 : 0.0);
                if ((cand == 0 && ns == 1) || t < best_t * 0.97) { best = ns; best_t = t; best_wide = cand != 0; }
            }
        }
        if (best > 1) {
            a.chunks_per_split = (int)((nK + best - 1) / best);
            a.nsplit = szn_div_up(nK, a.chunks_per_split);
            a.ws = (float*)d->workspace;
            use_wide = best_wide;
        }
    }
    int rc = 1;
    if (a.nsplit == 1 || use_wide) {
        static const int wide_min = szn_knob("SZN_WIDE_MINTILES", 240);
        rc = szn_conv_wide_try(d, in, w, bias, gate, chan_scale, out, a.in_bytes, a.w_bytes, use_wide ? 1 : wide_min, a.ws,
                               a.nsplit, a.chunks_per_split, stream);
        if (rc < 0 || (rc == 0 && a.nsplit == 1)) return rc;
    }
    if (rc != 0) {
        if (d->dtype == SZN_BF16) rc = narrow ? launch_v2<bf16_raw, 2>(a, st) : launch_v2<bf16_raw, 4>(a, st);
        else if (d->dtype == SZN_F16) rc = narrow ? launch_v2<f16_raw, 2>(a, st) : launch_v2<f16_raw, 4>(a, st);
        else if (d->dtype == SZN_BF16X3) rc = narrow ? launch_v2<f32x3_t, 2>(a, st) : launch_v2<f32x3_t, 4>(a, st);
        else rc = narrow ? launch_v2<float, 2>(a, st) : launch_v2<float, 4>(a, st);
        if (rc) return rc;
    }
    if (a.nsplit > 1 && a.colsum) {
        a.cslab = d->colsum_slab;
        szn_note_colsum_rows(a.cslab ? (int)cs_rows : 0);
        if (d->dtype == SZN_BF16)
            hipLaunchKernelGGL(splitk_epilogue_cs<bf16_raw>, dim3((unsigned)cs_rows), dim3(256), 0, st, (const float*)a.ws, a, cs_rpb);
        else if (d->dtype == SZN_F16)
            hipLaunchKernelGGL(splitk_epilogue_cs<f16_raw>, dim3((unsigned)cs_rows), dim3(256), 0, st, (const float*)a.ws, a, cs_rpb);
        else
            hipLaunchKernelGGL(splitk_epilogue_cs<float>, dim3((unsigned)cs_rows), dim3(256), 0, st, (const float*)a.ws, a, cs_rpb);
        SZN_CHECK_LAUNCH("splitk_epilogue_cs");
        return SZN_OK;
    }
    if (a.nsplit > 1) {
        long blocks = ((long)a.M * a.Co / 4 + 255) / 256;
        if (blocks > 8192) blocks = 8192;
        if (blocks < 1) blocks = 1;
        if (d->dtype == SZN_BF16)
            hipLaunchKernelGGL(splitk_epilogue<bf16_raw>, dim3((unsigned)blocks), dim3(256), 0, st, (const float*)a.ws, a);
        else if (d->dtype == SZN_F16)
            hipLaunchKernelGGL(splitk_epilogue<f16_raw>, dim3((unsigned)blocks), dim3(256), 0, st, (const float*)a.ws, a);
        else
            hipLaunchKernelGGL(splitk_epilogue<float>, dim3((unsigned)blocks), dim3(256), 0, st, (const float*)a.ws, a);
        SZN_CHECK_LAUNCH("splitk_epilogue");
    }
    return SZN_OK;
}
```

zeroshotsemanticsegmentation_amd/csrc/szn_conv_regw.hip:

```cpp
#include "szn_common.h"
#include "szn_cb.h"
#include <algorithm>

typedef __attribute__((ext_vector_type(4))) uint32_t u32x4_t;
typedef __attribute__((ext_vector_type(2))) uint32_t u32x2_t;
typedef __attribute__((address_space(3))) void* ldsptr_t;

namespace {

struct RwArgs {
    const char* in; const char* w; const float* bias; const char* gate; char* out; float* colsum;
    float* cslab;
    char* pool;
    unsigned char* pcode;
    int skip_x;
    CbGeom cb;
    int dg_on, gy0, gy1, gx0, gx1, sy0, sy1, sx0, sx1;
    unsigned gref;
    unsigned in_bytes, gate_bytes;
    unsigned out_bytes, pool_bytes;
    int Hp, Wp;
    int B, Hi, Wi, Ho, Wo, pad;
    int ldi, ldo, ldg, relu;
    int tiles_x, tiles_y, ntiles;
};

constexpr unsigned kOOBr = 0x80000000u;
constexpr unsigned kOOBst = 0xfffffff0u;
constexpr int PWr = 18;

__device__ __forceinline__ float row16_sum(float x) {
    x += __uint_as_float(__builtin_amdgcn_update_dpp(0u, __float_as_uint(x), 0xB1, 0xF, 0xF, true));
    x += __uint_as_float(__builtin_amdgcn_update_dpp(0u, __float_as_uint(x), 0x4E, 0xF, 0xF, true));
    x += __uint_as_float(__builtin_amdgcn_update_dpp(0u, __float_as_uint(x), 0x141, 0xF, 0xF, true));
    x += __uint_as_float(__builtin_amdgcn_update_dpp(0u, __float_as_uint(x), 0x140, 0xF, 0xF, true));
    return x;
}

template <int COG, int CIG>
struct RwGeom {
    static constexpr int PG = 8 / (COG * CIG);
    static constexpr int TR = 4 * PG;
    static constexpr int PROWS = (TR + 2) * PWr;
    static constexpr int RB = 128 * CIG;
    static constexpr int CPR = RB / 16;
    static constexpr int RPP = 1024 / RB;
    static constexpr int NPIECE = (PROWS * RB + 1023) / 1024;
    static constexpr int SLOTS = (NPIECE + 7) / 8;
    static constexpr int PATCHB = NPIECE * 1024;
    static constexpr int NBUF = CIG == 1 ? 3 : 2;
    static constexpr int CO = 32 * COG, CI = 64 * CIG;
    static constexpr int NJ = 4 / CIG;
    static constexpr int OFF_GATE = NBUF * PATCHB;
    static constexpr int OFF_XCH = OFF_GATE + 8 * NJ * 1024;
    static constexpr int OFF_DUMP = OFF_XCH + (CIG == 2 ? 8 * 4096 : 0);
    static constexpr int OFF_BIAS = OFF_DUMP + 1024;
    static constexpr int OFF_RED = OFF_BIAS + CO * 4;
    static constexpr int LDS = OFF_RED + CO * 4;
    static_assert(COG * CIG * PG == 8 && LDS <= 160 * 1024, "wave decomposition / LDS budget");
};

template <typename T, int COG, int CIG, bool GATED, bool COLSUM>
__global__ __launch_bounds__(512) void conv3x3_regw(RwArgs a) {
#if defined(__HIP_DEVICE_COMPILE__)
    typedef RwGeom<COG, CIG> G_;
    constexpr int PG = G_::PG, TR = G_::TR, PROWS = G_::PROWS, RB = G_::RB, CPR = G_::CPR, RPP = G_::RPP;
    constexpr int NPIECE = G_::NPIECE, SLOTS = G_::SLOTS, PATCHB = G_::PATCHB, NBUF = G_::NBUF, CO = G_::CO, CI = G_::CI;
    constexpr int NJ = G_::NJ;
    extern __shared__ __attribute__((aligned(16))) char smem[];
    const int tid = threadIdx.x, lane = tid & 63;
    const int w = __builtin_amdgcn_readfirstlane(tid >> 6);
    const int cig = w % CIG, cog = (w / CIG) % COG, pg = w / (CIG * COG);
    const int g = lane >> 4, r16 = lane & 15;

    const int G = gridDim.x;
    const int vb = (blockIdx.x & 7) * (G >> 3) + (blockIdx.x >> 3);
    const int first = (int)((long)a.ntiles * vb / G), last = (int)((long)a.ntiles * (vb + 1) / G);
    if (first >= last) {
        if constexpr (COLSUM) { if (a.cslab && tid < CO) a.cslab[(long)blockIdx.x * CO + tid] = 0.f; }
        return;
    }

    const auto rsA = __builtin_amdgcn_make_buffer_rsrc((void*)a.in, 0, (int)a.in_bytes, 0x00020000);
    const auto rsG = __builtin_amdgcn_make_buffer_rsrc((void*)(GATED ? a.gate : a.in), 0, (int)(GATED ? a.gate_bytes : 0u), 0x00020000);
    const auto rsO = __builtin_amdgcn_make_buffer_rsrc((void*)a.out, 0, (int)a.out_bytes, 0x00020000);
    const auto rsPo = __builtin_amdgcn_make_buffer_rsrc((void*)((!GATED && a.pool) ? a.pool : a.out), 0, (int)((!GATED && a.pool) ? a.pool_bytes : 0u), 0x00020000);
    const auto rsPc = __builtin_amdgcn_make_buffer_rsrc((void*)((!GATED && a.pcode) ? (char*)a.pcode : a.out), 0, (int)((!GATED && a.pcode) ? a.pool_bytes >> 1 : 0u), 0x00020000);

    u32x4_t W[9][2][2];
    {
        const char* wp = a.w + ((long)(cog * 32 + r16) * 9 * CI + cig * 64 + g * 8) * 2;
#pragma unroll
        for (int tap = 0; tap < 9; ++tap)
#pragma unroll
            for (int s = 0; s < 2; ++s)
#pragma unroll
                for (int i = 0; i < 2; ++i)
                    W[tap][s][i] = *(const u32x4_t*)(wp + ((long)(i * 16) * 9 * CI + tap * CI + s * 32) * 2);
    }
    if (tid < CO) {
        ((float*)(smem + G_::OFF_BIAS))[tid] = a.bias ? a.bias[tid] : 0.f;
        ((float*)(smem + G_::OFF_RED))[tid] = 0.f;
    }

    const int slot = lane % CPR, psub = lane / CPR;
    const unsigned chunkoff = (unsigned)((CPR == 8 ? (slot ^ psub) : (slot ^ ((4 * (w & 3) + psub) & 15))) << 4);
    const int q0 = RPP * w + psub;
    auto tile_of = [&](int t, int& b, int& ty, int& tx) {
        if (a.cb.on) {
            b = t / a.cb.per_image;
            cb_decode(a.cb, t - b * a.cb.per_image, ty, tx);
        } else {
            int bb = t;
            tx = bb % a.tiles_x; bb /= a.tiles_x;
            ty = bb % a.tiles_y; b = bb / a.tiles_y;
        }
    };
    auto step = [&](int& b, int& ty, int& tx) {
        ++tx;
        for (int pass = 0; pass < a.tiles_y + 2; ++pass) {
            if (a.cb.on && ty >= a.cb.fy0 && ty < a.cb.fy1 && tx >= a.cb.fx0 && tx < a.cb.fx1) {
                if (ty < a.cb.wy0 || ty >= a.cb.wy1) tx = a.cb.fx1;
                else if (tx < a.cb.wx0) tx = a.cb.wx0;
                else if (tx >= a.cb.wx1) tx = a.cb.fx1;
            }
            if (tx < a.tiles_x) break;
            tx = 0;
            if (++ty == a.tiles_y) { ty = 0; ++b; }
        }
    };
    int ib, ity, itx;
    tile_of(first, ib, ity, itx);
    int cb_b = ib, cb_ty = ity, cb_tx = itx;
    auto issue = [&](int buf) {
        const int b = ib, ty = ity, tx = itx;
        step(ib, ity, itx);
        const int ih0 = ty * TR - a.pad, iw0 = tx * 16 - a.pad;
        char* base = smem + buf * PATCHB;
        int q0v = q0;
        asm volatile("" : "+v"(q0v));
#pragma unroll
        for (int p = 0; p < SLOTS; ++p) {
            unsigned v = kOOBr;
            const int q = q0v + 8 * RPP * p;
            if (q < PROWS) {
                const int pr = (q * 3641) >> 16, pc = q - pr * PWr;
                const int ih = ih0 + pr, iw = iw0 + pc;
                if ((unsigned)ih < (unsigned)a.Hi && (unsigned)iw < (unsigned)a.Wi)
                    v = (unsigned)(((b * a.Hi + ih) * a.Wi + iw) * a.ldi * 2) + chunkoff;
            }
            const int piece = w + 8 * p;
            char* dst = (piece < NPIECE) ? base + piece * 1024 : smem + G_::OFF_DUMP;
            __builtin_amdgcn_raw_ptr_buffer_load_lds(rsA, (ldsptr_t)dst, 16, v, 0, 0, 0);
        }
    };

    const int cstart = cog * 32 + (g & 1) * 16 + (g >> 1) * 8;
    const int qb = (pg * 4) * PWr + r16;
    const int j0 = CIG == 2 ? 2 * cig : 0;

    issue(0);
    if constexpr (NBUF == 3) {
        if (first + 1 < last) {
            issue(1);
            asm volatile("s_waitcnt vmcnt(%0)" ::"i"(SLOTS) : "memory");
        } else {
            asm volatile("s_waitcnt vmcnt(0)" ::: "memory");
        }
    } else {
        asm volatile("s_waitcnt vmcnt(0)" ::: "memory");
    }
    __syncthreads();

    const bool grpB = CIG == 1 && w >= 4;
    float cst[8];
#pragma unroll
    for (int e = 0; e < 8; ++e) cst[e] = 0.f;
    const float relu_lo = a.relu ? 0.f : -__builtin_inff();
    int buf = 0;
    for (int t = first; t < last; ++t) {
        const bool more = t + NBUF - 1 < last;
        const int b = cb_b, ty = cb_ty, tx = cb_tx;
        step(cb_b, cb_ty, cb_tx);
        const int ow = tx * 16 + r16;
        const int oh0 = ty * TR + pg * 4 + j0;
        const unsigned m0 = (unsigned)((b * a.Ho + oh0) * a.Wo + ow);
        const bool okw = ow < a.Wo;
        bool gconst = false, nostore = false;
        if constexpr (GATED) {
            if (a.dg_on) {
                const int y0 = ty * TR, x0 = tx * 16;
                gconst = y0 + TR <= a.gy0 || y0 >= a.gy1 || x0 + 16 <= a.gx0 || x0 >= a.gx1;
                nostore = y0 + TR <= a.sy0 || y0 >= a.sy1 || x0 + 16 <= a.sx0 || x0 >= a.sx1;
            }
        }
        if constexpr (GATED) {
#pragma unroll
            for (int jj = 0; jj < NJ; ++jj) {
                const bool ok = okw && oh0 + jj < a.Ho;
                const unsigned v = ok ? ((gconst ? a.gref : m0 + jj * a.Wo) * a.ldg + cstart) * 2u : kOOBr;
                __builtin_amdgcn_raw_ptr_buffer_load_lds(rsG, (ldsptr_t)(smem + G_::OFF_GATE + (w * NJ + jj) * 1024), 16, v, 0, 0, 0);
            }
        }
        if (more) issue((buf + NBUF - 1) % NBUF);

        f32x4_t acc[2][4];
#pragma unroll
        for (int i = 0; i < 2; ++i)
#pragma unroll
            for (int j = 0; j < 4; ++j) acc[i][j] = f32x4_t{0.f, 0.f, 0.f, 0.f};
        const char* pb = smem + buf * PATCHB;
        int qbv = qb;
        asm volatile("" : "+v"(qbv));
        u32x4_t P[2][2];
        auto ldP = [&](int step, u32x4_t (&dst)[2]) {
            const int pr = step / 3, kw = step - pr * 3;
            const int q = qbv + pr * PWr + kw;
            const char* rowp = pb + q * RB;
            const int sw = q & (CPR - 1);
            dst[0] = *(const u32x4_t*)(rowp + (((cig * 8 + g) ^ sw) << 4));
            dst[1] = *(const u32x4_t*)(rowp + (((cig * 8 + 4 + g) ^ sw) << 4));
        };
        ldP(0, P[0]);
#pragma unroll
        for (int step = 0; step < 18; ++step) {
            const int pr = step / 3, kw = step - pr * 3;
            if (step + 1 < 18) ldP(step + 1, P[(step + 1) & 1]);
#pragma unroll
            for (int s = 0; s < 2; ++s)
#pragma unroll
                for (int kh = 0; kh < 3; ++kh) {
                    const int j = pr - kh;
                    if (j < 0 || j > 3) continue;
#pragma unroll
                    for (int i = 0; i < 2; ++i)
                        acc[i][j] = mfma16<T>(W[kh * 3 + kw][s][i], P[step & 1][s], acc[i][j]);
                }
            __builtin_amdgcn_sched_barrier(0);
        }

        if constexpr (CIG == 2) {
            f32x4_t* xw = (f32x4_t*)(smem + G_::OFF_XCH + w * 4096) + lane;
            const f32x4_t* xr = (const f32x4_t*)(smem + G_::OFF_XCH + (w ^ 1) * 4096) + lane;
            if (cig == 0) {
#pragma unroll
                for (int jj = 0; jj < 2; ++jj)
#pragma unroll
                    for (int i = 0; i < 2; ++i) xw[(jj * 2 + i) * 64] = acc[i][2 + jj];
            } else {
#pragma unroll
                for (int jj = 0; jj < 2; ++jj)
#pragma unroll
                    for (int i = 0; i < 2; ++i) xw[(jj * 2 + i) * 64] = acc[i][jj];
            }
            asm volatile("s_waitcnt lgkmcnt(0)" ::: "memory");
            __builtin_amdgcn_s_barrier();
            if (cig == 0) {
#pragma unroll
                for (int jj = 0; jj < 2; ++jj)
#pragma unroll
                    for (int i = 0; i < 2; ++i) acc[i][jj] += xr[(jj * 2 + i) * 64];
            } else {
#pragma unroll
                for (int jj = 0; jj < 2; ++jj)
#pragma unroll
                    for (int i = 0; i < 2; ++i) acc[i][jj] = acc[i][2 + jj] + xr[(jj * 2 + i) * 64];
            }
        }

        float bv[8];
        *(f32x4_t*)&bv[0] = *(const f32x4_t*)(smem + G_::OFF_BIAS + cstart * 4);
        *(f32x4_t*)&bv[4] = *(const f32x4_t*)(smem + G_::OFF_BIAS + cstart * 4 + 16);
        if (NBUF == 3 && more) asm volatile("s_waitcnt vmcnt(%0)" ::"i"(SLOTS) : "memory");
        else asm volatile("s_waitcnt vmcnt(0)" ::: "memory");
        if (grpB) {
            asm volatile("s_waitcnt lgkmcnt(0)" ::: "memory");
            __builtin_amdgcn_s_barrier();
        }
        float pm[8];
        u32x4_t pkm = {0u, 0u, 0u, 0u};
#pragma unroll
        for (int e = 0; e < 8; ++e) pm[e] = 0.f;
#pragma unroll
        for (int j = 0; j < NJ; ++j) {
            const bool ok = okw && oh0 + j < a.Ho;
            float v[8];
            u32x4_t gq;
            if constexpr (GATED) gq = *(const u32x4_t*)(smem + G_::OFF_GATE + (w * NJ + j) * 1024 + lane * 16);
#pragma unroll
            for (int c = 0; c < 4; ++c) {
                const auto r = __builtin_amdgcn_permlane16_swap(__float_as_uint(acc[0][j][c]), __float_as_uint(acc[1][j][c]), false, false);
                v[c] = __uint_as_float(r[0]);
                v[4 + c] = __uint_as_float(r[1]);
            }
#pragma unroll
            for (int e = 0; e < 8; ++e) {
                float x = fmaxf(v[e] + bv[e], relu_lo);
                if constexpr (GATED) {
                    const uint32_t gw = gq[e >> 1];
                    const float gv = __uint_as_float((e & 1) ? (gw & 0xffff0000u) : (gw << 16));
                    x = (gv > 0.f) ? x : 0.f;
                }
                v[e] = x;
                if constexpr (COLSUM) cst[e] += ok ? x : 0.f;
            }
            u32x4_t pk;
            pk.x = pack2<T>(v[0], v[1]);
            pk.y = pack2<T>(v[2], v[3]);
            pk.z = pack2<T>(v[4], v[5]);
            pk.w = pack2<T>(v[6], v[7]);
            if (!a.skip_x && !nostore)
                __builtin_amdgcn_raw_buffer_store_b128(pk, rsO, ok ? ((m0 + j * a.Wo) * a.ldo + cstart) * 2u : kOOBst, 0, 0);
            if constexpr (!GATED) {
                if (a.pool && a.pcode) {
                    const u32x4_t pz = ok ? pk : u32x4_t{0u, 0u, 0u, 0u};
                    if ((j & 1) == 0) pkm = pz;
                    else {
                        u32x4_t Mo, Co4;
                        auto pk_max = [](uint32_t x, uint32_t y) { uint32_t r; asm volatile("v_pk_max_u16 %0, %1, %2" : "=v"(r) : "v"(x), "v"(y)); return r; };
                        auto pk_min = [](uint32_t x, uint32_t y) { uint32_t r; asm volatile("v_pk_min_u16 %0, %1, %2" : "=v"(r) : "v"(x), "v"(y)); return r; };
                        auto pk_sub = [](uint32_t x, uint32_t y) { uint32_t r; asm volatile("v_pk_sub_u16 %0, %1, %2" : "=v"(r) : "v"(x), "v"(y)); return r; };
                        auto pk_mad = [](uint32_t x, uint32_t y, uint32_t z) { uint32_t r; asm volatile("v_pk_mad_u16 %0, %1, %2, %3" : "=v"(r) : "v"(x), "v"(y), "v"(z)); return r; };
                        const uint32_t one = 0x00010001u, four = 0x00040004u;
#pragma unroll
                        for (int i = 0; i < 4; ++i) {
                            const uint32_t A = pkm[i], Cq = pz[i];
                            const uint32_t Bq = (uint32_t)__builtin_amdgcn_update_dpp(0, (int)A, 0xB1, 0xF, 0xF, true);
                            const uint32_t Dq = (uint32_t)__builtin_amdgcn_update_dpp(0, (int)Cq, 0xB1, 0xF, 0xF, true);
                            const uint32_t M = pk_max(pk_max(A, Bq), pk_max(Cq, Dq));
                            const uint32_t na = pk_min(pk_sub(M, A), one), nb = pk_min(pk_sub(M, Bq), one), nc = pk_min(pk_sub(M, Cq), one);
                            const uint32_t t = pk_mad(nb, pk_mad(nc, one, one), one);
                            uint32_t code = pk_mad(na, t, 0u);
                            const uint32_t z = pk_min(M, one);
                            code = pk_mad(pk_sub(code, four), z, four);
                            Mo[i] = M;
                            Co4[i] = code;
                        }
                        const int poh = (oh0 + j) >> 1, pw = ow >> 1;
                        const bool pst = (r16 & 1) == 0 && okw && poh < a.Hp;
                        const unsigned pe = (unsigned)((b * a.Hp + poh) * a.Wp + pw) * (32 * COG) + cstart;
                        __builtin_amdgcn_raw_buffer_store_b128(Mo, rsPo, pst ? pe * 2u : kOOBst, 0, 0);
                        u32x2_t cb;
                        cb.x = __builtin_amdgcn_perm(Co4[1], Co4[0], 0x06040200u);
                        cb.y = __builtin_amdgcn_perm(Co4[3], Co4[2], 0x06040200u);
                        __builtin_amdgcn_raw_buffer_store_b64(cb, rsPc, pst ? pe : kOOBst, 0, 0);
                    }
                } else
                if (a.pool) {
                    if ((j & 1) == 0) {
#pragma unroll
                        for (int e = 0; e < 8; ++e) pm[e] = ok ? v[e] : 0.f;
                    } else {
                        float mx[8];
#pragma unroll
                        for (int e = 0; e < 8; ++e) {
                            const float m2 = fmaxf(pm[e], ok ? v[e] : 0.f);
                            const float nb = __uint_as_float(__builtin_amdgcn_update_dpp(0u, __float_as_uint(m2), 0xB1, 0xF, 0xF, true));
                            mx[e] = fmaxf(m2, nb);
                        }
                        const int poh = (oh0 + j) >> 1, pw = ow >> 1;
                        if ((r16 & 1) == 0 && okw && poh < a.Hp) {
                            u32x4_t pq;
                            pq.x = pack2<T>(mx[0], mx[1]);
                            pq.y = pack2<T>(mx[2], mx[3]);
                            pq.z = pack2<T>(mx[4], mx[5]);
                            pq.w = pack2<T>(mx[6], mx[7]);
                            *(u32x4_t*)(a.pool + ((size_t)((b * a.Hp + poh) * a.Wp + pw) * (32 * COG) + cstart) * 2) = pq;
                        }
                    }
                }
            }
        }
        if (!grpB) {
            asm volatile("s_waitcnt lgkmcnt(0)" ::: "memory");
            __builtin_amdgcn_s_barrier();
        }
        buf = (buf == NBUF - 1) ? 0 : buf + 1;
    }
    if constexpr (COLSUM) {
        asm volatile("s_waitcnt vmcnt(0) lgkmcnt(0)" ::: "memory");
        __syncthreads();
        float* pw = (float*)smem;
#pragma unroll
        for (int e = 0; e < 8; ++e) {
            const float x = row16_sum(cst[e]);
            if (r16 == 0) pw[(w * 4 + g) * 8 + e] = x;
        }
        __syncthreads();
        if (tid < CO) {
            const int cogc = tid >> 5, rem = tid & 31;
            const int gc = (((rem & 15) >> 3) << 1) | (rem >> 4), ec = rem & 7;
            float s = 0.f;
#pragma unroll
            for (int ww = 0; ww < 8; ++ww)
                if ((ww / CIG) % COG == cogc) s += pw[(ww * 4 + gc) * 8 + ec];
            if (a.cslab) a.cslab[(long)blockIdx.x * CO + tid] = s;
            else if (s != 0.f) atomicAdd(a.colsum + tid, s);
        }
    }
#endif
}

constexpr int CB_FILL_G = 8;
__global__ __launch_bounds__(256) void regw_const_fill_kernel(CbGeom c, int TR, int Co, int Ho, int Wo, int Hp, int Wp, uint16_t* __restrict__ out,
                                                             int ldo, uint16_t* __restrict__ pool, unsigned char* __restrict__ pcode,
                                                             int ref_oh, int ref_ow) {
    const int ngrp = (c.tiles_x + CB_FILL_G - 1) / CB_FILL_G;
    const int grp = blockIdx.x % ngrp, ty = (blockIdx.x / ngrp) % c.tiles_y, b = blockIdx.x / (ngrp * c.tiles_y);
    if (ty < c.fy0 || ty >= c.fy1) return;
    const int g0 = grp * CB_FILL_G, g1 = g0 + CB_FILL_G;
    const int cpp = Co / 8;
    const bool inwin = ty >= c.wy0 && ty < c.wy1;
    for (int run = 0; run < 2; ++run) {
        int t0, t1;
        if (!inwin) { if (run) break; t0 = c.fx0; t1 = c.fx1; }
        else if (run == 0) { t0 = c.fx0; t1 = c.wx0; }
        else { t0 = c.wx1; t1 = c.fx1; }
        t0 = t0 > g0 ? t0 : g0; t1 = t1 < g1 ? t1 : g1;
        if (t1 <= t0) continue;
        const int x0 = t0 * 16, nx = (t1 - t0) * 16;
        if (out) {
            const uint4* ref = (const uint4*)(out + ((long)ref_oh * Wo + ref_ow) * ldo);
            for (int i = threadIdx.x; i < TR * nx * cpp; i += 256) {
                const int cc = i % cpp, px = i / cpp;
                const int oh = ty * TR + px / nx, ow = x0 + px % nx;
                *(uint4*)(out + ((long)(b * Ho + oh) * Wo + ow) * ldo + cc * 8) = ref[cc];
            }
        }
        if (pool) {
            const int rp = ref_oh >> 1, rq = ref_ow >> 1;
            const uint4* pref = (const uint4*)(pool + ((long)rp * Wp + rq) * Co);
            const uint2* cref = pcode ? (const uint2*)(pcode + ((long)rp * Wp + rq) * Co) : nullptr;
            const int px0 = x0 >> 1, npx = nx >> 1;
            for (int i = threadIdx.x; i < (TR / 2) * npx * cpp; i += 256) {
                const int cc = i % cpp, px = i / cpp;
                const int ph = ty * (TR / 2) + px / npx, pw = px0 + px % npx;
                const long pe = ((long)(b * Hp + ph) * Wp + pw) * Co + cc * 8;
                *(uint4*)(pool + pe) = pref[cc];
                if (cref) *(uint2*)(pcode + pe) = cref[cc];
            }
        }
    }
}

template <typename T, int COG, int CIG, bool GATED, bool COLSUM>
int launch_regw(const RwArgs& a, int grid, hipStream_t st) {
    constexpr int lds = RwGeom<COG, CIG>::LDS;
    static bool attr_done = false;
    if (!attr_done) {
        (void)hipFuncSetAttribute((const void*)conv3x3_regw<T, COG, CIG, GATED, COLSUM>, hipFuncAttributeMaxDynamicSharedMemorySize, lds);
        attr_done = true;
    }
    hipLaunchKernelGGL((conv3x3_regw<T, COG, CIG, GATED, COLSUM>), dim3((unsigned)grid), dim3(512), lds, st, a);
    SZN_CHECK_LAUNCH("conv3x3_regw");
    return SZN_OK;
}

template <typename T, int COG, int CIG>
int launch_regw_flags(const RwArgs& a, int grid, hipStream_t st) {
    if (a.gate) return a.colsum ? launch_regw<T, COG, CIG, true, true>(a, grid, st) : launch_regw<T, COG, CIG, true, false>(a, grid, st);
    return a.colsum ? launch_regw<T, COG, CIG, false, true>(a, grid, st) : launch_regw<T, COG, CIG, false, false>(a, grid, st);
}

}

static bool regw_dgrad_skip_geom(const szn_conv_desc_t* d, int tr, CbGeom& c) {
    const int ty_n = szn_div_up(d->Ho, tr), tx_n = szn_div_up(d->Wo, 16);
    const int y0 = std::max(std::min(d->cb_rect[0], d->cb_const[0]), 0), y1 = std::min(std::max(d->cb_rect[1], d->cb_const[1]), d->Ho);
    const int x0 = std::max(std::min(d->cb_rect[2], d->cb_const[2]), 0), x1 = std::min(std::max(d->cb_rect[3], d->cb_const[3]), d->Wo);
    if (y1 <= y0 || x1 <= x0 || d->pad != 1) return false;
    c = CbGeom{};
    c.on = 1; c.tiles_y = ty_n; c.tiles_x = tx_n;
    c.fy0 = 0; c.fy1 = ty_n; c.fx0 = 0; c.fx1 = tx_n;
    c.wy0 = y0 / tr; c.wy1 = (y1 + tr - 1) / tr; c.wx0 = x0 / 16; c.wx1 = (x1 + 15) / 16;
    cb_finish(c);
    const long all = (long)ty_n * tx_n;
    return c.per_image > 0 && (all - c.per_image) * 10 >= all;
}

int szn_conv_regw_try(const szn_conv_desc_t* d, const void* in, const void* w, const float* bias, const void* gate,
                      const float* chan_scale, void* out, int min_tiles, szn_stream_t stream) {
    if (!szn_is16(d->dtype) || d->KH != 3 || d->KW != 3 || d->pad > 2 || d->out_f32 || chan_scale) return 1;
    if ((d->Ci != 64 && d->Ci != 128) || (d->Co != 64 && d->Co != 128)) return 1;
    if ((d->ldo & 7) || (d->ldi & 7) || (gate && (d->ldg & 7))) return 1;
    if (d->pool_out && (gate || (size_t)d->B * ((d->Ho + 1) / 2) * ((d->Wo + 1) / 2) * d->Co * 2 >= 0xffff0000ul)) return 1;
    const size_t in_bytes = (size_t)d->B * d->Hi * d->Wi * d->ldi * 2;
    const size_t gate_bytes = gate ? (size_t)d->B * d->Ho * d->Wo * d->ldg * 2 : 0;
    if (in_bytes >= 0x7fff0000ul || gate_bytes >= 0x7fff0000ul || (size_t)d->B * d->Ho * d->Wo * d->ldo * 2 >= 0xffff0000ul)
        return 1;
    const int cog = d->Co / 32, cig = d->Ci / 64;
    const int tr = 4 * (8 / (cog * cig));
    RwArgs a;
    a.in = (const char*)in; a.w = (const char*)w; a.bias = bias; a.gate = (const char*)gate; a.out = (char*)out;
    a.colsum = d->colsum;
    a.cslab = d->colsum ? d->colsum_slab : nullptr;
    a.pool = (char*)d->pool_out; a.Hp = (d->Ho + 1) / 2; a.Wp = (d->Wo + 1) / 2;
    a.pcode = a.pool ? (unsigned char*)d->pool_code : nullptr;
    a.skip_x = (a.pool && d->pool_only) ? 1 : 0;
    a.in_bytes = (unsigned)in_bytes; a.gate_bytes = (unsigned)gate_bytes;
    a.out_bytes = (unsigned)((size_t)d->B * d->Ho * d->Wo * d->ldo * 2);
    a.pool_bytes = a.pool ? (unsigned)((size_t)d->B * a.Hp * a.Wp * d->Co * 2) : 0u;
    a.B = d->B; a.Hi = d->Hi; a.Wi = d->Wi; a.Ho = d->Ho; a.Wo = d->Wo; a.pad = d->pad;
    a.ldi = d->ldi; a.ldo = d->ldo; a.ldg = d->ldg; a.relu = d->relu;
    a.tiles_x = szn_div_up(d->Wo, 16); a.tiles_y = szn_div_up(d->Ho, tr);
    const long nt = (long)a.B * a.tiles_y * a.tiles_x;
    if (nt >= (1L << 30) || nt * tr * 16 < (long)min_tiles * 256) return 1;
    a.ntiles = (int)nt;
    CbGeom cb = {};
    bool use_cb = false;
    int ref_oh = 0, ref_ow = 0;
    {
        static const int cbe = szn_knob("SZN_CONST_BORDER", 1);
        if (cbe && d->cb_on && !gate && !d->colsum) {
            cb.tiles_y = a.tiles_y; cb.tiles_x = a.tiles_x;
            cb.fy0 = (std::max(d->cb_const[0], 0) + tr - 1) / tr; cb.fy1 = std::min(d->cb_const[1], d->Ho) / tr;
            cb.fx0 = (std::max(d->cb_const[2], 0) + 15) / 16;     cb.fx1 = std::min(d->cb_const[3], d->Wo) / 16;
            cb.wy0 = std::max(d->cb_rect[0], 0) / tr;             cb.wy1 = (std::min(d->cb_rect[1], d->Ho) + tr - 1) / tr;
            cb.wx0 = std::max(d->cb_rect[2], 0) / 16;             cb.wx1 = (std::min(d->cb_rect[3], d->Wo) + 15) / 16;
            if (cb.fy1 > cb.fy0 && cb.fx1 > cb.fx0 && cb.wy0 - 1 >= cb.fy0 && cb.wy0 - 1 < cb.fy1 && cb.wy1 > cb.wy0 && cb.wx1 > cb.wx0 && cb.wx0 >= cb.fx0 && cb.wx0 < cb.fx1) {
                const int ry = cb.wy0 - 1, rx = cb.wx0;
                cb.wy0 -= 1;
                cb_finish(cb);
                const long kept = (long)cb.per_image * a.B;
                if (kept * 10 <= nt * 9 && cb.nF > 0 && cb.nW > 0) {
                    use_cb = true;
                    cb.on = 1;
                    a.ntiles = (int)kept;
                    ref_oh = ry * tr; ref_ow = rx * 16;
                    szn_note_work_fraction((float)((double)kept / (double)nt));
                }
            }
        }
    }
    a.cb = cb;
    a.dg_on = 0; a.gy0 = a.gy1 = a.gx0 = a.gx1 = a.sy0 = a.sy1 = a.sx0 = a.sx1 = 0; a.gref = 0;
    {
        static const int cbe = szn_knob("SZN_CONST_BORDER", 1);
        if (cbe && d->cb_on && gate && d->cb_rect[0] >= 1 && d->cb_rect[0] <= d->Ho && d->cb_rect[2] >= 0 && d->cb_rect[2] < d->Wo) {
            a.dg_on = 1;
            a.gy0 = d->cb_rect[0]; a.gy1 = d->cb_rect[1]; a.gx0 = d->cb_rect[2]; a.gx1 = d->cb_rect[3];
            a.sy0 = d->cb_const[0]; a.sy1 = d->cb_const[1]; a.sx0 = d->cb_const[2]; a.sx1 = d->cb_const[3];
            a.gref = (unsigned)((d->cb_rect[0] - 1) * d->Wo + d->cb_rect[2]);
            CbGeom sk;
            if (d->cb_on == 2 && d->colsum && regw_dgrad_skip_geom(d, tr, sk)) {
                a.cb = sk;
                a.ntiles = a.B * sk.per_image;
                szn_note_work_fraction((float)sk.per_image / (float)(a.tiles_y * a.tiles_x));
            }
        }
    }
    static int ncu = 0;
    if (!ncu) {
        int dev = 0; hipDeviceProp_t p;
        if (hipGetDevice(&dev) == hipSuccess && hipGetDeviceProperties(&p, dev) == hipSuccess) ncu = p.multiProcessorCount;
        if (ncu <= 0) ncu = 256;
        ncu &= ~7;
        if (ncu < 8) ncu = 8;
    }
    const int ncu_all = ncu;
    int grid_cus = ncu_all;
    if (d->reserved_cus > 0) { grid_cus = (ncu_all - d->reserved_cus) & ~7; if (grid_cus < 8) grid_cus = 8; }
    hipStream_t st = (hipStream_t)stream;
    if (a.cslab && d->colsum_slab_rows < grid_cus) SZN_FAIL(SZN_ERR_ARG, "conv2d: colsum_slab holds %d rows, %d needed", d->colsum_slab_rows, grid_cus);
    szn_note_colsum_rows(a.cslab ? grid_cus : 0);
    int rc;
    if (d->dtype == SZN_F16) {
        if (cog == 2 && cig == 1) rc = launch_regw_flags<f16_raw, 2, 1>(a, grid_cus, st);
        else if (cog == 4 && cig == 1) rc = launch_regw_flags<f16_raw, 4, 1>(a, grid_cus, st);
        else if (cog == 2 && cig == 2) rc = launch_regw_flags<f16_raw, 2, 2>(a, grid_cus, st);
        else rc = launch_regw_flags<f16_raw, 4, 2>(a, grid_cus, st);
    } else if (cog == 2 && cig == 1) rc = launch_regw_flags<bf16_raw, 2, 1>(a, grid_cus, st);
    else if (cog == 4 && cig == 1) rc = launch_regw_flags<bf16_raw, 4, 1>(a, grid_cus, st);
    else if (cog == 2 && cig == 2) rc = launch_regw_flags<bf16_raw, 2, 2>(a, grid_cus, st);
    else rc = launch_regw_flags<bf16_raw, 4, 2>(a, grid_cus, st);
    if (rc || !use_cb) return rc;
    hipLaunchKernelGGL(regw_const_fill_kernel, dim3((unsigned)(a.B * a.tiles_y * ((a.tiles_x + CB_FILL_G - 1) / CB_FILL_G))), dim3(256), 0, st, cb, tr, d->Co, d->Ho, d->Wo, a.Hp, a.Wp,
                       a.skip_x ? nullptr : (uint16_t*)a.out, d->ldo, (uint16_t*)a.pool, a.pcode, ref_oh, ref_ow);
    SZN_CHECK_LAUNCH("conv3x3_regw");
    return SZN_OK;
}

namespace {
struct StripArgs {
    const char* dout; int B, H, W, Co, ldd, is_f16;
    int rect[2][4];
    float* prim;
};
__global__ __launch_bounds__(256) void border_strips_kernel(StripArgs a) {
    __shared__ float red[256][9];
    const int item = blockIdx.x, r = blockIdx.y, b = blockIdx.z;
    const int y0 = a.rect[r][0], y1 = a.rect[r][1], x0 = a.rect[r][2], x1 = a.rect[r][3];
    const int ys[4] = {y0 - 1, y0, y1 - 1, y1}, xs[4] = {x0 - 1, x0, x1 - 1, x1};
    int py, px, n, dy, dx;
    if (item < 4) { py = ys[item]; px = x0; n = x1 - x0; dy = 0; dx = 1; }
    else if (item < 8) { py = y0; px = xs[item - 4]; n = y1 - y0; dy = 1; dx = 0; }
    else { py = ys[(item - 8) >> 2]; px = xs[(item - 8) & 3]; n = 1; dy = 0; dx = 0; }
    const int chunks = a.Co >> 3, ppi = 256 / chunks;
    const int ch = threadIdx.x % chunks, pl = threadIdx.x / chunks;
    float s[8] = {0.f, 0.f, 0.f, 0.f, 0.f, 0.f, 0.f, 0.f};
    auto ld = [&](int i) -> uint4 {
        const int y = py + dy * i, x = px + dx * i;
        if (i >= n || y < 0 || y >= a.H || x < 0 || x >= a.W) return make_uint4(0u, 0u, 0u, 0u);
        return *(const uint4*)(a.dout + ((size_t)((b * a.H + y) * a.W + x) * a.ldd + ch * 8) * 2);
    };
    auto add = [&](const uint4& v) {
        const uint32_t wv[4] = {v.x, v.y, v.z, v.w};
#pragma unroll
        for (int e = 0; e < 4; ++e) {
            const uint16_t lo = (uint16_t)(wv[e] & 0xffffu), hi = (uint16_t)(wv[e] >> 16);
            s[2 * e] += a.is_f16 ? f16_bits_to_f32(lo) : bf16_bits_to_f32(lo);
            s[2 * e + 1] += a.is_f16 ? f16_bits_to_f32(hi) : bf16_bits_to_f32(hi);
        }
    };
    if (pl < ppi)
        for (int q = pl; q < n; q += 8 * ppi) {
            uint4 v[8];
#pragma unroll
            for (int u = 0; u < 8; ++u) v[u] = ld(q + u * ppi);
#pragma unroll
            for (int u = 0; u < 8; ++u) add(v[u]);
        }
#pragma unroll
    for (int e = 0; e < 8; ++e) red[threadIdx.x][e] = s[e];
    __syncthreads();
    for (int co = threadIdx.x; co < a.Co; co += 256) {
        const int c8 = co >> 3, e = co & 7;
        float t = 0.f;
        for (int p = 0; p < ppi; ++p) t += red[p * chunks + c8][e];
        a.prim[(((size_t)r * 24 + item) * a.B + b) * a.Co + co] = t;
    }
}

struct FinishArgs {
    const float* prim; const float* s0; const char* wT; const char* gate; float* colsum;
    int B, Co, Ci, is_f16; unsigned gref_bytes;
};
__device__ __forceinline__ float border_delta(const float* P, int dy, int dx) {
    auto row = [&](int i) { return P[i]; };
    auto col = [&](int i) { return P[4 + i]; };
    auto pix = [&](int yi, int xi) { return P[8 + yi * 4 + xi]; };
    float d = 0.f;
    if (dy == 1) d += row(3) - row(1);
    else if (dy == -1) d += row(0) - row(2);
    auto colshift = [&](int xi) {
        float c = col(xi);
        if (dy == 1) c += pix(3, xi) - pix(1, xi);
        else if (dy == -1) c += pix(0, xi) - pix(2, xi);
        return c;
    };
    if (dx == 1) d += colshift(3) - colshift(1);
    else if (dx == -1) d += colshift(0) - colshift(2);
    return d;
}
__global__ __launch_bounds__(256) void border_finish_kernel(FinishArgs a) {
    __shared__ float D[9][128];
    __shared__ float Pl[48][128];
    {
        const int co = threadIdx.x % a.Co, grp = threadIdx.x / a.Co, ngrp = 256 / a.Co;
        for (int pr = grp; pr < 48; pr += ngrp) {
            const float* src = a.prim + (size_t)pr * a.B * a.Co + co;
            float t = 0.f;
            int b = 0;
            for (; b + 8 <= a.B; b += 8) {
                float v[8];
#pragma unroll
                for (int u = 0; u < 8; ++u) v[u] = src[(size_t)(b + u) * a.Co];
#pragma unroll
                for (int u = 0; u < 8; ++u) t += v[u];
            }
            for (; b < a.B; ++b) t += src[(size_t)b * a.Co];
            Pl[pr][co] = t;
        }
    }
    __syncthreads();
    for (int co = threadIdx.x; co < a.Co; co += 256) {
        float P[2][24];
#pragma unroll
        for (int r = 0; r < 2; ++r)
#pragma unroll
            for (int it = 0; it < 24; ++it) P[r][it] = Pl[r * 24 + it][co];
#pragma unroll
        for (int kh = 0; kh < 3; ++kh)
#pragma unroll
            for (int kw = 0; kw < 3; ++kw)
                D[kh * 3 + kw][co] = a.s0[co] + border_delta(P[0], kh - 1, kw - 1) - border_delta(P[1], kh - 1, kw - 1);
    }
    __syncthreads();
    const int qtr = threadIdx.x & 3, cq = a.Co >> 2;
    for (int ci = threadIdx.x >> 2; ci < a.Ci; ci += 64) {
        float acc = 0.f;
        for (int tap = 0; tap < 9; ++tap) {
            const uint16_t* wr = (const uint16_t*)a.wT + ((size_t)ci * 9 + tap) * a.Co + qtr * cq;
            for (int c8 = 0; c8 < cq; c8 += 8) {
                const uint4 v = *(const uint4*)(wr + c8);
                const uint32_t wv[4] = {v.x, v.y, v.z, v.w};
#pragma unroll
                for (int e = 0; e < 4; ++e) {
                    const uint16_t lo = (uint16_t)(wv[e] & 0xffffu), hi = (uint16_t)(wv[e] >> 16);
                    acc = fmaf(a.is_f16 ? f16_bits_to_f32(lo) : bf16_bits_to_f32(lo), D[tap][qtr * cq + c8 + 2 * e], acc);
                    acc = fmaf(a.is_f16 ? f16_bits_to_f32(hi) : bf16_bits_to_f32(hi), D[tap][qtr * cq + c8 + 2 * e + 1], acc);
                }
            }
        }
        const float a1 = __shfl_xor(acc, 1, 64);
        const float s01 = (qtr & 1) ? a1 + acc : acc + a1;
        const float s23 = __shfl_xor(s01, 2, 64);
        const float tot = (qtr & 2) ? s23 + s01 : s01 + s23;
        if (qtr == 0) {
            const uint16_t gb = *(const uint16_t*)(a.gate + a.gref_bytes + (size_t)ci * 2);
            const float gv = a.is_f16 ? f16_bits_to_f32(gb) : bf16_bits_to_f32(gb);
            if (gv > 0.f) a.colsum[ci] += tot;
        }
    }
}
}

static bool border_desc_ok(const szn_conv_desc_t* d) {
// ... 43 lines not shown
```

zeroshotsemanticsegmentation_amd/models.py:

```python
import atexit
import contextlib
import ctypes as C
import math
import os
import os.path as osp

import numpy as np
import torch
import torch.nn as nn

from . import _lib as L
from . import heads, synth
from .heads import CROP, CROP_UP8
PAD1 = 100


def get_upsampling_weight(in_channels, out_channels, kernel_size):
    return torch.from_numpy(synth.bilinear_weight(in_channels, out_channels, kernel_size))


def _round_up(a, b):
    return (a + b - 1) // b * b


# ... 39 lines not shown
def _cumask_spec():
    n, _, how = os.environ.get("SZN_FC6_CUMASK", _FC6_CUMASK).partition(":")
    try:
        return max(int(n or 0), 0), (how or "low")
    except ValueError:
        raise L.SznError("SZN_FC6_CUMASK: expected <n>[:low|:even], got %r" % os.environ.get("SZN_FC6_CUMASK"))


_MASKED_HANDLES = []


@atexit.register
def _destroy_masked_streams():
    while _MASKED_HANDLES:
        h = _MASKED_HANDLES.pop()
        try:
            torch.cuda.synchronize()
            L.call("szn_stream_destroy", h)
        except Exception:
            pass


def masked_stream_wanted(pixels):
    return _cumask_spec()[0] > 0 and pixels <= _SMALL_STEP_PX and os.environ.get("SZN_WGRAD_STREAM", "auto") != "0"


def _band_cut(reg, n, L=3):
    r0, r1, c0, c1 = reg
    cuts = []
    a = c0 + L + 2
    a += a & 1
    e = (r0 - L) & ~1
    if e - a >= 4:
        cuts.append((a, e, a // 2 - 1, a // 2 - 1))
    a2 = r1 + L
    a2 += a2 & 1
    e2 = (min(c1, n) - L - 2) & ~1
    if e2 - a2 >= 4 and c1 <= n:
        cuts.append((a2, e2, e2 // 2, a2 // 2))
    return cuts


def _gather_form(dev, ty, tx):
    out = {}
    for key, t in (("y", ty), ("x", tx)):
        runs = [[s0, c] for s0, c in t if c > 1]
        out["runs_" + key] = dev(runs) if runs else None
    out["tabs"] = (dev([[s0, min(c, 1)] for s0, c in ty]), dev([[s0, min(c, 1)] for s0, c in tx]))
    return out


class _BandPlan(object):

    def __init__(self, regy, regx, H, W, device, L=3):
        self.H, self.W = H, W
        ty, tx = self._axis(regy, H, L), self._axis(regx, W, L)
        cut8 = []
        for reg, n in ((regy, H), (regx, W)):
            top, bot = (0, 0), (n, n)
            for a, e, _, _ in _band_cut(reg, n, L):
                if e <= reg[0]:
                    top = (a, e)
                else:
                    bot = (a, e)
            cut8 += [top[0], top[1], bot[0], bot[1]]
        self.cut8 = (C.c_int * 8)(*cut8)
        self.ok = ty is not None and tx is not None and (ty["n"] < H or tx["n"] < W)
        if not self.ok:
            return
        self.Hc, self.Wc = ty["n"], tx["n"]
        self.Hp, self.Wp = (H + 1) // 2, (W + 1) // 2
        self.Hpc, self.Wpc = (self.Hc + 1) // 2, (self.Wc + 1) // 2
        dev = lambda t: torch.tensor(t, dtype=torch.int32, device=device).contiguous()
        self.tabs = {k: (dev(ty[k]), dev(tx[k])) for k in ("crop", "crop_bwd", "uncrop", "uncrop_bwd")}
        self.host = {k: (ty[k], tx[k]) for k in ("crop", "crop_bwd", "uncrop", "uncrop_bwd")}
        self._dev, self._fused = dev, {}
        ident = lambda n: dev([[i, 1] for i in range(n)])
        self.tabs["uncrop_bwd_y"] = (self.tabs["uncrop_bwd"][0], ident(self.Wp))
        self.tabs["uncrop_bwd_x"] = (ident(self.Hpc), self.tabs["uncrop_bwd"][1])
        self.gather_uncrop = _gather_form(dev, *self.host["uncrop_bwd"])
        self.x = None

    def fused_with(self, nxt):
        key = id(nxt)
        if key not in self._fused:
            dev = self._dev
            out = {}
            per_axis = []
            for ax in (0, 1):
                un, ub = self.host["uncrop"][ax], self.host["uncrop_bwd"][ax]
                cr, cb = nxt.host["crop"][ax], nxt.host["crop_bwd"][ax]
                fwd = [[un[y][0], 1] for y, _ in cr]
                bwd = []
                for s0, cnt in ub:
                    kept = [p for p in range(s0, s0 + cnt) if cb[p][1] == 1]
                    assert all(cb[kept[i + 1]][0] == cb[kept[i]][0] + 1 for i in range(len(kept) - 1))
                    bwd.append([cb[kept[0]][0], len(kept)] if kept else [0, 0])
                per_axis.append((fwd, bwd))
            ident = lambda n: [[i, 1] for i in range(n)]
            out["fwd"] = (dev(per_axis[0][0]), dev(per_axis[1][0]))
            out["bwd_y"] = (dev(per_axis[0][1]), dev(ident(nxt.Wc)))
            out["bwd_x"] = (dev(ident(self.Hpc)), dev(per_axis[1][1]))
            out["bwd_gather"] = _gather_form(dev, per_axis[0][1], per_axis[1][1])
            self._fused[key] = out
        return self._fused[key]

    @staticmethod
    def _axis(reg, n, L=3):
        cuts = _band_cut(reg, n, L)
        removed = set()
        for a, e, _, _ in cuts:
            removed.update(range(a, e))
        kept = [y for y in range(n) if y not in removed]
        pos = {y: i for i, y in enumerate(kept)}
        npool = (n + 1) // 2
        removed_p, rep_of = set(), {}
        for a, e, rep, _ in cuts:
            for p in range(a // 2, e // 2):
                removed_p.add(p)
                rep_of[p] = rep
        kept_p = [p for p in range(npool) if p not in removed_p]
        pos_p = {p: i for i, p in enumerate(kept_p)}
        if len(kept_p) != (len(kept) + 1) // 2:
            return None
        t = {"n": len(kept)}
        t["crop"] = [[y, 1] for y in kept]
        t["crop_bwd"] = [[pos[y], 1] if y in pos else [0, 0] for y in range(n)]
        t["uncrop"] = [[pos_p[p] if p in pos_p else pos_p[rep_of[p]], 1] for p in range(npool)]
        ub = [[p, 1] for p in kept_p]
        for a, e, rep, first in cuts:
            ub[pos_p[rep]] = [first, (e - a) // 2 + 1]
        t["uncrop_bwd"] = ub
        return t


class _Ctx(object):
    __slots__ = ("x", "acts", "pools", "relu6", "relu7", "masks", "coarse", "B", "H", "W", "h", "w", "train", "cb_in", "crop")


class _Engine(object):

    def __init__(self, model):
        self.model = model
        self.dtype = torch.float32
        self.bf16x3 = False
        self._versions = None
        self._images = {}
        self._layer_versions = {}
        self.dropout_seed = 1337
        self.dropout_calls = 0
        self._splitk_ws = None
        self._gemm_ws = None
        self._wg_ws = None
        self._wg_stream = None
        self._wg_masked = None
        self.keep_prepool = False
        self.fused_opt = None
        self.fused_done = set()
        self.reserved_cus = 0
        self.head_fp8 = False
        self.head_fp8_bwd = False
        self._fp8_ws = None
        self._fp8_bws = None
        self.lp_views = {}
        self.deterministic = os.environ.get("SZN_DETERMINISTIC", "1") != "0"
        self._cs_pool, self._cs_off, self._cs_jobs = None, 0, []
        self._seen_versions = None
        self.weight_gate = None
        self._pack_pending = None

    def _workspace(self, desc, nbytes, device):
        if nbytes > (64 << 20):
            return
        nbytes = min(16 * nbytes, 256 << 20)
        if self._splitk_ws is None or self._splitk_ws.numel() < nbytes or self._splitk_ws.device != device:
            self._splitk_ws = torch.empty(max(nbytes, 64 << 20), dtype=torch.uint8, device=device)
        desc.workspace, desc.workspace_bytes = self._splitk_ws.data_ptr(), self._splitk_ws.numel()

    def set_precision(self, dtype):
        x3 = isinstance(dtype, str) and dtype == "bf16x3"
        if x3:
            dtype = torch.float32
        if isinstance(dtype, str) or dtype not in (torch.float32, torch.bfloat16, torch.float16):
            raise L.SznError("compute dtype must be float32, bfloat16, float16 or 'bf16x3'")
        self.bf16x3 = x3
        if dtype != self.dtype:
            self.dtype = dtype
            self._versions = None
            self._layer_versions = {}

    @property
    def precision(self):
        return "bf16x3" if self.bf16x3 else self.dtype

    def _gemm_code(self, name):
        return L.SZN_BF16X3 if (self.bf16x3 and name in _X3_LAYERS) else L.dtype_code(self.dtype)

    def mark_dirty(self):
        self._versions = None
        self._layer_versions = {}

    def _param_versions(self):
        return tuple((p.data_ptr(), p._version) for p in self.model.parameters())

    def _ohwi(self, p):
        t = p.detach()
        if t.dtype != torch.float32:
            t = t.float()
        return t.permute(0, 2, 3, 1).contiguous()

    def sync_weights(self):
        v = self._param_versions()
        if v == self._versions:
            return
        m = self.model
        dev = m.conv1_1.weight.device
        if dev.type != "cuda":
            raise L.SznError("FCN32s parameters live on %s: the HIP path needs them on the GPU (model.cuda())" % dev)
        dt, code = self.dtype, L.dtype_code(self.dtype)
        img = dict(self._images) if (self._images and self._layer_versions.get("_dtype") == (dt, dev)) else {}
        if not img:
            self._layer_versions = {"_dtype": (dt, dev)}
        lv = self._layer_versions
        st = L.stream_ptr()
        jobs = []
        for name, co, ci, k in synth.CONV_LAYERS:
            layer = getattr(m, name)
            ver = (layer.weight.data_ptr(), layer.weight._version, layer.bias.data_ptr(), layer.bias._version,
                   id(self.lp_views.get(name)))
            if lv.get(name) == ver and (name + ".w") in img:
                continue
            lv[name] = ver
            w32 = self._ohwi(layer.weight)
            img[name + ".b"] = layer.bias.detach().float().contiguous()
            if name == "conv1_1":
                img[name + ".w"] = w32
                continue
            if dt == torch.float32:
                wc = w32
            elif name in self.lp_views and self.lp_views[name].dtype == dt:
                wc = self.lp_views[name]
            else:
                self._gate(name)
                wc = w32.to(dt)
            img[name + ".w"] = wc
            if k >= 5:
                img[name + ".wG"] = img.get(name + ".wG")
                img[name + ".wG.stale"] = True
                continue
            wt = torch.empty(ci, k, k, co, device=dev, dtype=dt)
            jobs.append((wc, wt, co, k, ci))
            img[name + ".wT"] = wt
        E, CP, F = m.n_class, m.head_width, m.fc7.out_channels
        hver = tuple((p.data_ptr(), p._version) for p in (m.score_fr.weight, m.score_fr.bias, m.seenmask_score.weight,
                                                          m.seenmask_score.bias)) + (id(self.lp_views.get("head")),)
        uver = (m.seenmask_upscore.weight.data_ptr(), m.seenmask_upscore.weight._version)
        if lv.get("up") != uver or "up.w" not in img:
            img["up.w"] = m.seenmask_upscore.weight.detach().float().contiguous()
            lv["up"] = uver
        if lv.get("head") == hver and "head.w" in img:
            self._pack_or_defer(jobs, code, st)
            self._images = img
            self._versions = v
            return
        lv["head"] = hver
        hv = self.lp_views.get("head")
        if hv is not None and hv[0].dtype == dt:
            whc, bh = hv
            sv = (m.seenmask_score.weight._version, m.seenmask_score.bias._version)
            if sv != self._seen_versions:
                whc[E:E + 2].copy_(m.seenmask_score.weight.detach().reshape(2, F))
                bh[E:E + 2].copy_(m.seenmask_score.bias.detach())
                self._seen_versions = sv
        else:
            self._gate("head")
            wh = torch.zeros(CP, F, device=dev, dtype=torch.float32)
            bh = torch.zeros(CP, device=dev, dtype=torch.float32)
            wh[:E] = m.score_fr.weight.detach().float().reshape(E, F)
            wh[E:E + 2] = m.seenmask_score.weight.detach().float().reshape(2, F)
            bh[:E] = m.score_fr.bias.detach().float()
            bh[E:E + 2] = m.seenmask_score.bias.detach().float()
            whc = wh if dt == torch.float32 else wh.to(dt)
        wht = torch.empty(F, CP, device=dev, dtype=dt)
        jobs.append((whc, wht, CP, 1, F))
        self._pack_or_defer(jobs, code, st)
        img["head.w"], img["head.b"], img["head.wT"] = whc.view(CP, 1, 1, F), bh, wht.view(F, 1, 1, CP)
        self._images = img
        self._versions = v

    def _gate(self, name):
        if self.weight_gate is not None:
            self.weight_gate(name)

    def _pack_or_defer(self, jobs, code, st):
        if self.weight_gate is not None:
            self._pack_pending = (self._pack_pending[0] if self._pack_pending else []) + list(jobs), code
        else:
            self._pack(jobs, code, st)

    def _flush_pack(self):
        if self._pack_pending:
            if self.weight_gate is not None:
                self.weight_gate(None)
            jobs, code = self._pack_pending
            self._pack_pending = None
            self._pack(jobs, code, L.stream_ptr())
# ... 241 lines not shown
        if dbh is not None:
            slab, rows = self._cs_slab(M, CP, dc.device)
            ro = L.rows_out()
            L.call("szn_bias_grad_slab", L.dtype_code(dc.dtype), M, CP, CP, L.ptr(dc), L.ptr(dbh), 0, L.ptr(slab), rows, C.byref(ro), st)
            self._cs_register(slab, CP, dbh, ro)

    def _head_dgrad_fp8(self, dc, feat, scale, colsum):
        B, h, w, F = feat.shape
        CP, M = self.model.head_width, B * h * w
        ws = self._fp8_bwd_ws(M, F, CP, feat.device)
        wimg = self._images["head.w"]
        code = L.dtype_code(self.dtype)
        d = torch.empty(B, h, w, F, device=feat.device, dtype=self.dtype)
        st = L.stream_ptr()
        L.call("szn_proj_fp8_dgrad", L.dtype_code(dc.dtype), L.dtype_code(wimg.dtype), M, F, CP, CP, L.ptr(dc), L.ptr(wimg),
               L.ptr(feat), L.dtype_code(feat.dtype), F, L.ptr(scale), h * w, code, L.ptr(d), F, L.ptr(ws), st)
        if colsum is not None:
            slab, rows = self._cs_slab(M, F, d.device)
            ro = L.rows_out()
            L.call("szn_bias_grad_slab", code, M, F, F, L.ptr(d), L.ptr(colsum), 1, L.ptr(slab), rows, C.byref(ro), st)
            self._cs_register(slab, F, colsum, ro)
        return d

    def upscore(self, ctx):
        m = self.model
        f = torch.empty(ctx.B, m.n_class, ctx.H, ctx.W, device=ctx.coarse.device, dtype=torch.float32)
        L.call("szn_bilinear_up32_crop_fwd", ctx.B, ctx.h, ctx.w, m.n_class, m.head_width, 0, ctx.H, ctx.W, CROP,
               L.ptr(ctx.coarse), L.ptr(f), L.stream_ptr())
        return f

    def seenmask_upscore(self, ctx):
        m = self.model
        s = torch.empty(ctx.B, 2, ctx.H, ctx.W, device=ctx.coarse.device, dtype=torch.float32)
        L.call("szn_deconv64s32_fwd", ctx.B, ctx.h, ctx.w, 2, m.head_width, m.n_class, ctx.H, ctx.W, CROP,
               L.ptr(ctx.coarse), L.ptr(self._images["up.w"]), L.ptr(s), L.stream_ptr())
        return s

    def head_backward(self, ctx, df=None, ds=None, dcoarse=None):
        m = self.model
        dev = ctx.coarse.device
        if dcoarse is None:
            dcoarse = torch.zeros(ctx.B, ctx.h, ctx.w, m.head_width, device=dev, dtype=torch.float32)
        dup = None
        if df is not None:
            df = df.contiguous().float()
            L.call("szn_bilinear_up32_crop_bwd", ctx.B, ctx.h, ctx.w, m.n_class, m.head_width, 0, ctx.H, ctx.W, CROP,
                   L.ptr(df), L.ptr(dcoarse), L.stream_ptr())
        if ds is not None:
            ds = ds.contiguous().float()
            L.call("szn_deconv64s32_dgrad", ctx.B, ctx.h, ctx.w, 2, m.head_width, m.n_class, ctx.H, ctx.W, CROP,
                   L.ptr(ds), L.ptr(self._images["up.w"]), L.ptr(dcoarse), L.stream_ptr())
            dup = torch.empty(2, 2, 64, 64, device=dev, dtype=torch.float32)
            L.call("szn_deconv64s32_wgrad", ctx.B, ctx.h, ctx.w, 2, m.head_width, m.n_class, ctx.H, ctx.W, CROP,
                   L.ptr(ctx.coarse), L.ptr(ds), L.ptr(dup), 0, L.stream_ptr())
        return dcoarse, dup

    @contextlib.contextmanager
    def _wgrad_stream(self, *tensors, heavy=False):
        if not getattr(self, "_wg_on", False):
            yield
            return
        if self._wg_stream is None:
            self._wg_stream = torch.cuda.Stream(device=tensors[0].device)
        side = self._wg_stream
        dev = tensors[0].device
        if heavy and torch.cuda.current_stream(dev) != torch.cuda.default_stream(dev):
            side = self._masked_stream(dev) or side
        side.wait_stream(torch.cuda.current_stream())
        with torch.cuda.stream(side):
            yield
        for t in tensors:
            t.record_stream(side)

    def _masked_stream(self, dev):
        if self._wg_masked is None:
            self._wg_masked = False
            n, how = _cumask_spec()
            info = L.DeviceInfo()
            L.call("szn_device_info", dev.index or 0, C.byref(info))
            ncu = info.compute_units
            if 0 < n < ncu:
                words = (ncu + 31) // 32
                mask = (C.c_uint32 * words)()
                picked = range(n) if how == "low" else sorted({(i * ncu) // n for i in range(n)})
                for cu in picked:
                    mask[cu // 32] |= 1 << (cu % 32)
                h = C.c_void_p()
                L.call("szn_stream_create_cu_mask", words, mask, C.byref(h))
                self._wg_masked = torch.cuda.ExternalStream(h.value, device=dev)
                _MASKED_HANDLES.append(h)
        return self._wg_masked or None

    def _join_wgrad(self):
        if self._wg_stream and getattr(self, "_wg_on", False):
            torch.cuda.current_stream().wait_stream(self._wg_stream)
            if self._wg_masked:
                torch.cuda.current_stream().wait_stream(self._wg_masked)
        self._flush_colsum()

    def _conv1_1_dgrad_cb(self, ctx):
        ry, rx = _cb_conv1_1(ctx.H, PAD1), _cb_conv1_1(ctx.W, PAD1)
        reads = (C.c_int * 4)()
        sub = L.load().szn_conv1_1_wgrad_reads(L.dtype_code(self.dtype), ctx.B, ctx.H, ctx.W, PAD1, reads)
        if sub not in (0, 1):
            raise L.SznError("szn_conv1_1_wgrad_reads failed (%d)" % sub)
        return ((ry[0], ry[1], rx[0], rx[1]), tuple(reads))

    def _wgrad_desc(self, x, dout_shape, ci, co, k, pad, ldo=None, cb=None, name=None):
        B, Hi, Wi, _ = x.shape
        Ho, Wo = dout_shape[1:3]
        ldo = dout_shape[3] if ldo is None else ldo
        d = L.ConvDesc(self._gemm_code(name), B, Hi, Wi, ci, Ho, Wo, co, k, k, pad, ci, ldo, 0, 0, 0)
        d.reserved_cus = self.reserved_cus
        nb = 2 * 256 * 64 * 9 * 64 * 4
        if self._wg_ws is None or self._wg_ws.device != x.device:
            self._wg_ws = torch.empty(nb, dtype=torch.uint8, device=x.device)
        d.workspace, d.workspace_bytes = self._wg_ws.data_ptr(), nb
        if cb is not None and _CONST_BORDER and self.dtype != torch.float32:
            (ry, rx) = cb
            d.cb_on = 1
            d.cb_rect[0], d.cb_rect[1], d.cb_rect[2], d.cb_rect[3] = ry[0], ry[1], rx[0], rx[1]
            d.cb_const[0], d.cb_const[1], d.cb_const[2], d.cb_const[3] = ry[2], ry[3], rx[2], rx[3]
        return d

    def _wgrad(self, x, dout, dw, db, ci, co, k, pad, ldo=None, after=None, fuse=None, cb=None, csum=None, dw_lp=None, name=None):
        B, Hi, Wi, _ = x.shape
        Ho, Wo = dout.shape[1:3]
        code = L.dtype_code(self.dtype)
        d = self._wgrad_desc(x, dout.shape, ci, co, k, pad, ldo=ldo, cb=cb, name=name)
        ldo = d.ldo
        if dw_lp is not None:
            d.dw_lp, d.dw_lp_dtype = dw_lp.data_ptr(), L.dtype_code(dw_lp.dtype)
        if csum is not None and d.cb_on:
            d.colsum = csum.data_ptr()
        opt = self.fused_opt.get(fuse) if (self.fused_opt and fuse) else None
        if opt is not None and L.load().szn_conv2d_wgrad_adam_supported(C.byref(d)) != 1:
            opt = None
        with self._wgrad_stream(*([x, dout] + ([csum] if csum is not None else [])), heavy=opt is not None):
            st = L.stream_ptr()
            if opt is not None:
                opt[0].grad_optional = 0 if opt[1] else 1
                L.call("szn_conv2d_wgrad_adam", C.byref(d), L.ptr(x), L.ptr(dout), L.ptr(dw), C.byref(opt[0]), st)
                self.fused_done.add(fuse)
            else:
                L.call("szn_conv2d_wgrad", C.byref(d), L.ptr(x), L.ptr(dout), L.ptr(dw), 0, st)
            if db is not None:
                slab, rows = self._cs_slab(B * Ho * Wo, co, dout.device)
                ro = L.rows_out()
                L.call("szn_bias_grad_slab", code, B * Ho * Wo, co, ldo, L.ptr(dout), L.ptr(db), 0, L.ptr(slab), rows, C.byref(ro), st)
                self._cs_register(slab, co, db, ro)
            if after is not None:
                after()

    def _dgrad(self, dout, name, in_shape, pad, gate=None, scale=None, colsum=None, wT=None, cb=None, border_sum=None):
        B, Hi, Wi, Ci = in_shape
        Ho, Wo, Co = dout.shape[1:]
        din = torch.empty(B, Hi, Wi, Ci, device=dout.device, dtype=self.dtype)
        if wT is None and (name + ".wG") in self._images:
            if gate is not None or scale is not None or colsum is not None:
                raise L.SznError("dgrad of %s: the GEMM form has no gate / scale / colsum epilogue" % name)
            img = self._images
            wf = img[name + ".w"]
            k = wf.shape[1]
            code = L.dtype_code(self.dtype)
            d = L.ConvDesc(self._gemm_code(name), B, Hi, Wi, Ci, Ho, Wo, Co, k, k, pad, Ci, Co, 0, 0, 0)
            lib = L.load()
            native = dout.is_contiguous() and lib.szn_conv2d_dgrad_gemm_native_supported(C.byref(d)) == 1
            nb = (lib.szn_conv2d_dgrad_gemm_native_workspace_bytes if native else lib.szn_conv2d_dgrad_gemm_workspace_bytes)(C.byref(d))
            if self._gemm_ws is None or self._gemm_ws.numel() < nb or self._gemm_ws.device != dout.device:
                self._gemm_ws = torch.empty(nb, dtype=torch.uint8, device=dout.device)
            d.workspace, d.workspace_bytes = self._gemm_ws.data_ptr(), self._gemm_ws.numel()
            if native:
                L.call("szn_conv2d_dgrad_gemm_native", C.byref(d), L.ptr(dout), L.ptr(wf), L.ptr(din), L.stream_ptr())
                return din
            if img.get(name + ".wG.stale", True) or img[name + ".wG"] is None:
                if img[name + ".wG"] is None:
                    img[name + ".wG"] = torch.empty(k * k * Ci, Co, device=dout.device, dtype=self.dtype)
                L.call("szn_pack_weight_dgrad", code, Co, 1, 1, k * k * Ci, L.ptr(wf), L.ptr(img[name + ".wG"]), L.stream_ptr())
                img[name + ".wG.stale"] = False
            L.call("szn_conv2d_dgrad_gemm", C.byref(d), L.ptr(dout), L.ptr(img[name + ".wG"]), L.ptr(din), L.stream_ptr())
            return din
        wT = self._images[name + ".wT"] if wT is None else wT
        k = wT.shape[1]
        d = L.ConvDesc(self._gemm_code(name), B, Hi, Wi, Ci, Ho, Wo, Co, k, k, pad, Ci, Co, Ci, 0, 0)
        d.reserved_cus = self.reserved_cus
        slab = None
        M = B * Hi * Wi
        if colsum is not None:
            d.colsum = colsum.data_ptr()
            slab, rows = self._cs_slab(M, Ci, dout.device)
            if slab is not None:
                d.colsum_slab, d.colsum_slab_rows = slab.data_ptr(), rows
        if colsum is None or cb is None:
            self._workspace(d, M * Ci * 4, dout.device)
        if cb is not None and gate is not None and _CONST_BORDER and self.dtype != torch.float32:
            grect, srect = cb
            d.cb_on = 2 if (border_sum is not None and colsum is not None) else 1
            for i in range(4):
                d.cb_rect[i], d.cb_const[i] = grect[i], srect[i]
        L.call("szn_conv2d_dgrad", C.byref(d), L.ptr(dout), L.ptr(wT), L.ptr(gate), L.ptr(scale), L.ptr(din), L.stream_ptr())
        cs_rows = d.res.colsum_rows
        if d.cb_on == 2 and d.res.work_fraction < 1.0:
            bws = torch.empty(2 * 24 * B * Co, device=dout.device)
            L.call("szn_conv2d_dgrad_border_finish", C.byref(d), L.ptr(dout), L.ptr(wT), L.ptr(gate), L.ptr(border_sum), L.ptr(colsum),
                   L.ptr(bws), L.stream_ptr())
        self._cs_register(slab, Ci, colsum, cs_rows)
        return din

    def backward(self, ctx, dcoarse, grads, backbone=True, layer_done=None, head_first=None, skips=None):
        m = self.model
        dt = self.dtype
        code = L.dtype_code(dt)
        st = L.stream_ptr()
        mode = os.environ.get("SZN_WGRAD_STREAM", "auto")
        self._wg_on = (mode == "1" or (mode == "auto" and ctx.B * ctx.H * ctx.W <= _SMALL_STEP_PX)) and \
            not (mode != "1" and torch.cuda.is_current_stream_capturing())
        dc = dcoarse if dcoarse.dtype == dt else dcoarse.to(dt)
        feat = ctx.relu7
        F = m.fc7.out_channels
        flat_bias = grads.get("_flat_bias")
        if flat_bias is not None and backbone:
            flat_bias.zero_()
        fp8b = self.head_fp8_bwd and self.head_fp8
        lp = grads.get("_lp") or {}
        if "head" in grads:
            dwh, dbh = grads["head"]
            if fp8b:
                self._head_wgrad_fp8(feat, dc, dwh, dbh)
                if "head" in lp:
                    L.call("szn_cast", L.SZN_F32, L.dtype_code(lp["head"].dtype), dwh.numel(), L.ptr(dwh), L.ptr(lp["head"]), st)
                if head_first is not None:
                    head_first()
            else:
                self._wgrad(feat, dc, dwh, dbh, F, m.head_width, 1, 0, after=head_first, dw_lp=lp.get("head"))
        if not backbone:
            self._join_wgrad()
            return
        done = layer_done if layer_done is not None else (lambda name: None)
        s6 = ctx.masks[0] if ctx.masks is not None else None
        s7 = ctx.masks[1] if ctx.masks is not None else None
        if flat_bias is None:
            for name in grads:
                if name != "head" and not name.startswith("_"):
                    grads[name][1].zero_()
        if fp8b:
            d = self._head_dgrad_fp8(dc, feat, s7, grads["fc7"][1])
        else:
            d = self._dgrad(dc, "head", feat.shape, 0, gate=feat, scale=s7, colsum=grads["fc7"][1])
        self._wgrad(ctx.relu6, d, grads["fc7"][0], None, F, F, 1, 0, after=lambda: done("fc7"), fuse="fc7", dw_lp=lp.get("fc7"), name="fc7")
        d = self._dgrad(d, "fc7", ctx.relu6.shape, 0, gate=ctx.relu6, scale=s6, colsum=grads["fc6"][1])
        pool5 = ctx.pools[4][1]
        if self.fused_opt and "fc6" in self.fused_opt:
            d6 = d
            d = self._dgrad(d6, "fc6", pool5.shape, 0)
            self._wgrad(pool5, d6, grads["fc6"][0], None, pool5.shape[3], F, 7, 0, after=lambda: done("fc6"), fuse="fc6", name="fc6")
        else:
            self._wgrad(pool5, d, grads["fc6"][0], None, pool5.shape[3], F, 7, 0, after=lambda: done("fc6"), dw_lp=lp.get("fc6"), name="fc6")
            d = self._dgrad(d, "fc6", pool5.shape, 0)
        pi = 4
        prev_out = None
        pending_gather = None
        cb_sums, border_sums = {}, {}
        items = _BACKBONE
        for idx in range(len(items) - 1, -1, -1):
            item = items[idx]
            if item == "P":
                pin, pout = ctx.pools[pi][:2]
                pcode = ctx.pools[pi][2] if len(ctx.pools[pi]) > 2 else None
                pi -= 1
                producer = items[idx - 1][0]
                gather = None
                if ctx.crop and ("out", producer) in ctx.crop and not ctx.crop.get(("fusedout", producer)):
                    band = ctx.crop[("out", producer)]
                    if pcode is not None:
                        gather = band.gather_uncrop
                    else:
                        d = self._band_remap(d, band, "uncrop_bwd_y", band.Hpc, band.Wp)
                        d = self._band_remap(d, band, "uncrop_bwd_x", band.Hpc, band.Wpc)
                elif pending_gather is not None:
                    if pcode is not None:
                        gather = pending_gather[0]
                    else:
                        for tab, ho, wo in pending_gather[1]:
                            d = self._band_remap(d, pending_gather[2], tab, ho, wo)
                pending_gather = None
                B, Hi, Wi, Cc = ctx.pools[pi + 1][3] if pcode is not None else pin.shape
                dn = torch.empty(B, Hi, Wi, Cc, device=d.device, dtype=pout.dtype)
                slab, rows = self._cs_slab(B * Hi * Wi, Cc, d.device)
                ro = L.rows_out()
                regions, want = [], []
                cbp = (getattr(ctx, "cb_in", None) or {}).get(producer)
                if pcode is not None and slab is not None and idx >= 2 and self.dtype != torch.float32 and _CONST_BORDER:
                    prev2 = items[idx - 2]
                    xin2 = ctx.pools[pi][1] if prev2 == "P" else ctx.acts[prev2[0]]
                    lay = getattr(m, producer)
                    if cbp is not None:
                        dd = self._wgrad_desc(xin2, (B, Hi, Wi, Cc), lay.in_channels, lay.out_channels, 3, items[idx - 1][1], cb=cbp)
                        r8 = (C.c_int * 8)()
                        if dd.cb_on and L.load().szn_conv2d_wgrad_cb_region(C.byref(dd), r8) == 1:
                            regions += list(r8)
                            want.append("w")
                    if prev2 != "P" and prev2[0] == "conv1_1" and _DGRAD_BORDER and B * Hi * Wi >= 1000000 and \
                            ("in", producer) not in (ctx.crop or {}):
                        grect, srect = self._conv1_1_dgrad_cb(ctx)
                        ci2 = lay.in_channels
                        dq = L.ConvDesc(code, B, Hi, Wi, ci2, Hi, Wi, Cc, 3, 3, items[idx - 1][1], ci2, Cc, ci2, 0, 0)
                        dq.cb_on = 2
                        for i in range(4):
                            dq.cb_rect[i], dq.cb_const[i] = grect[i], srect[i]
                        r8 = (C.c_int * 8)()
                        if L.load().szn_conv2d_dgrad_border_region(C.byref(dq), r8) == 1 and all(v % 2 == 0 for v in r8):
                            regions += list(r8)
                            want.append("d")
                if regions and gather is not None:
                    raise L.SznError("pool backward of %s: a band map and constant-border regions at once" % producer)
                if regions:
                    n = len(want)
                    ssum = torch.empty(n, Cc, device=d.device)
                    slab2 = torch.empty(n * rows * Cc, device=d.device)
                    L.call("szn_maxpool2x2_ceil_bwd_code_cb", code, B, Hi, Wi, Cc, L.ptr(pcode), L.ptr(d), L.ptr(dn),
                           L.ptr(grads[producer][1]), L.ptr(slab), rows, C.byref(ro), (C.c_int * len(regions))(*regions), n, L.ptr(ssum),
                           L.ptr(slab2), st)
                    for i, kind in enumerate(want):
                        (cb_sums if kind == "w" else border_sums)[producer] = ssum[i]
                elif gather is not None:
                    d = d.contiguous()
                    for axis, runs in ((0, gather["runs_y"]), (1, gather["runs_x"])):
                        if runs is not None:
                            L.call("szn_band_fold", code, B, d.shape[1], d.shape[2], Cc, L.ptr(d), axis, L.ptr(runs), runs.shape[0], st)
                    ty, tx = gather["tabs"]
                    L.call("szn_maxpool2x2_ceil_bwd_code_gather", code, B, Hi, Wi, Cc, L.ptr(pcode), L.ptr(d), d.shape[1], d.shape[2],
                           L.ptr(ty), L.ptr(tx), L.ptr(dn), L.ptr(grads[producer][1]), L.ptr(slab), rows, C.byref(ro), st)
                elif pcode is not None:
                    L.call("szn_maxpool2x2_ceil_bwd_code", code, B, Hi, Wi, Cc, L.ptr(pcode), L.ptr(d), L.ptr(dn),
                           L.ptr(grads[producer][1]), L.ptr(slab), rows, C.byref(ro), st)
                else:
                    L.call("szn_maxpool2x2_ceil_bwd", code, B, Hi, Wi, Cc, L.ptr(pin), L.ptr(pout), L.ptr(d), L.ptr(dn),
                           L.ptr(grads[producer][1]), L.ptr(slab), rows, C.byref(ro), st)
                self._cs_register(slab, Cc, grads[producer][1], ro)
                d = dn
                continue
            name, pad = item
            if name == "conv1_1":
                dw, db = grads[name]
                nb = L.load().szn_conv1_1_wgrad_workspace_bytes(code, ctx.B, ctx.H, ctx.W, PAD1)
                ws = torch.empty(nb, dtype=torch.uint8, device=d.device)
                with self._wgrad_stream(d, ws):
                    if ctx.crop and "c11cut" in ctx.crop:
                        L.call("szn_conv1_1_wgrad_c", code, ctx.B, ctx.H, ctx.W, PAD1, L.ptr(ctx.x), L.ptr(d), L.ptr(dw), 0,
                               L.ptr(ws), ctx.crop["c11cut"], L.stream_ptr())
                    else:
                        L.call("szn_conv1_1_wgrad", code, ctx.B, ctx.H, ctx.W, PAD1, L.ptr(ctx.x), L.ptr(d), L.ptr(dw), None, 0,
                               L.ptr(ws), L.stream_ptr())
                    if name in lp:
                        L.call("szn_cast", L.SZN_F32, L.dtype_code(lp[name].dtype), dw.numel(), L.ptr(dw), L.ptr(lp[name]), L.stream_ptr())
                    done(name)
                break
            prev = items[idx - 1]
            xin = ctx.pools[pi][1] if prev == "P" else ctx.acts[prev[0]]
            cropped_in = bool(ctx.crop) and ("in", name) in ctx.crop
            if cropped_in:
                xin = ctx.crop[("in", name)][1]
            layer = getattr(m, name)
            self._wgrad(xin, d, grads[name][0], None, layer.in_channels, layer.out_channels, 3, pad,
                        after=lambda name=name: done(name), cb=(getattr(ctx, "cb_in", None) or {}).get(name),
                        csum=cb_sums.pop(name, None), dw_lp=lp.get(name), name=name)
            if prev == "P":
                d = self._dgrad(d, name, xin.shape, pad)
                if cropped_in:
                    band = ctx.crop[("in", name)][0]
                    prev_band = ctx.crop.get(("fused", name))
                    if prev_band is not None:
                        ft = prev_band.fused_with(band)
                        two = [(ft["bwd_y"], prev_band.Hpc, band.Wc), (ft["bwd_x"], prev_band.Hpc, prev_band.Wpc)]
                        if not (skips and skips.get(pi) is not None):
                            pending_gather = (ft["bwd_gather"], two, band)
                        else:
                            for tab, ho, wo in two:
                                d = self._band_remap(d, band, tab, ho, wo)
                    else:
                        d = self._band_remap(d, band, "crop_bwd", band.H, band.W)
                side = skips.get(pi) if skips else None
                if side is not None:
                    d = d + side.to(d.dtype)
            else:
                cb = self._conv1_1_dgrad_cb(ctx) if (prev[0] == "conv1_1" and not cropped_in) else None
                d = self._dgrad(d, name, xin.shape, pad, gate=xin, colsum=grads[prev[0]][1], cb=cb, border_sum=border_sums.pop(name, None))
                if cropped_in and "c11cut" not in ctx.crop:
                    band = ctx.crop[("in", name)][0]
                    d = self._band_remap(d, band, "crop_bwd", band.H, band.W)
        self._join_wgrad()


def _backbone_backward(ctx, dcoarse, skips=None):
    model, c = ctx.model, ctx.c
    eng = model._engine
    dev = dcoarse.device
    need = ctx.needs_input_grad[4:]
    names = [n for n, _ in model.named_parameters()]
    need_of = dict(zip(names, need))
    backbone = any(need_of.get(n + ".weight", False) for n in _TRUNK)
    grads = {}
    for name, co, ci, k in synth.CONV_LAYERS:
        if backbone:
            grads[name] = (torch.empty(co, k, k, ci, device=dev), torch.empty(co, device=dev))
    CP, F, E = model.head_width, model.fc7.out_channels, model.n_class
    grads["head"] = (torch.empty(CP, 1, 1, F, device=dev), torch.empty(CP, device=dev))
    eng.backward(c, dcoarse.contiguous(), grads, backbone=backbone, skips=skips)
    out = []
    for n in names:
        layer, kind = n.rsplit(".", 1)
        if not need_of[n] or layer in ("upscore", "seenmask_upscore"):
            out.append(None)
        elif layer == "score_fr":
            g = grads["head"][0][:E].reshape(E, F, 1, 1) if kind == "weight" else grads["head"][1][:E]
            out.append(g.clone())
        elif layer == "seenmask_score":
            g = grads["head"][0][E:E + 2].reshape(2, F, 1, 1) if kind == "weight" else grads["head"][1][E:E + 2]
            out.append(g.clone())
        elif layer in grads:
            out.append(grads[layer][0].permute(0, 3, 1, 2) if kind == "weight" else grads[layer][1])
        else:
            out.append(None)
    return (None, None, None, None) + tuple(out)


class _Backbone(torch.autograd.Function):

    @staticmethod
    def forward(ctx, model, x, train, masks, *params):
        eng = model._engine
        c = eng.forward(x, train=train, masks=masks)
        ctx.model, ctx.c = model, c
        model._last_ctx = c
        return c.coarse

    @staticmethod
    def backward(ctx, dcoarse):
        return _backbone_backward(ctx, dcoarse)


class _Upscore(torch.autograd.Function):
    @staticmethod
    def forward(ctx, model, coarse):
        c = model._last_ctx
        ctx.model, ctx.c = model, c
        return model._engine.upscore(c)

    @staticmethod
    def backward(ctx, df):
        dcoarse, _ = ctx.model._engine.head_backward(ctx.c, df=df)
        return None, dcoarse


class _SeenmaskUpscore(torch.autograd.Function):
    @staticmethod
    def forward(ctx, model, coarse, weight):
        c = model._last_ctx
        ctx.model, ctx.c = model, c
        return model._engine.seenmask_upscore(c)

    @staticmethod
    def backward(ctx, ds):
        dcoarse, dup = ctx.model._engine.head_backward(ctx.c, ds=ds)
        return None, dcoarse, dup


class FCN32s(nn.Module):

    pretrained_model = 'data/fcn32s_from_caffe.pth'

    def __init__(self, n_class=21):
        super(FCN32s, self).__init__()
        self.n_class = n_class
        self.head_width = _round_up(n_class + 2, 64)
        chans = {n: (ci, co, k) for n, co, ci, k in synth.CONV_LAYERS}

        def conv(name, pad):
            ci, co, k = chans[name]
            return nn.Conv2d(ci, co, k, padding=pad)

        self.conv1_1 = conv("conv1_1", PAD1); self.relu1_1 = nn.ReLU(inplace=True)
        self.conv1_2 = conv("conv1_2", 1); self.relu1_2 = nn.ReLU(inplace=True)
        self.pool1 = nn.MaxPool2d(2, stride=2, ceil_mode=True)
        self.conv2_1 = conv("conv2_1", 1); self.relu2_1 = nn.ReLU(inplace=True)
        self.conv2_2 = conv("conv2_2", 1); self.relu2_2 = nn.ReLU(inplace=True)
        self.pool2 = nn.MaxPool2d(2, stride=2, ceil_mode=True)
        self.conv3_1 = conv("conv3_1", 1); self.relu3_1 = nn.ReLU(inplace=True)
        self.conv3_2 = conv("conv3_2", 1); self.relu3_2 = nn.ReLU(inplace=True)
        self.conv3_3 = conv("conv3_3", 1); self.relu3_3 = nn.ReLU(inplace=True)
        self.pool3 = nn.MaxPool2d(2, stride=2, ceil_mode=True)
        self.conv4_1 = conv("conv4_1", 1); self.relu4_1 = nn.ReLU(inplace=True)
        self.conv4_2 = conv("conv4_2", 1); self.relu4_2 = nn.ReLU(inplace=True)
        self.conv4_3 = conv("conv4_3", 1); self.relu4_3 = nn.ReLU(inplace=True)
        self.pool4 = nn.MaxPool2d(2, stride=2, ceil_mode=True)
        self.conv5_1 = conv("conv5_1", 1); self.relu5_1 = nn.ReLU(inplace=True)
        self.conv5_2 = conv("conv5_2", 1); self.relu5_2 = nn.ReLU(inplace=True)
        self.conv5_3 = conv("conv5_3", 1); self.relu5_3 = nn.ReLU(inplace=True)
        self.pool5 = nn.MaxPool2d(2, stride=2, ceil_mode=True)
        self.fc6 = nn.Conv2d(512, 4096, 7); self.relu6 = nn.ReLU(inplace=True); self.drop6 = nn.Dropout2d()
        self.fc7 = nn.Conv2d(4096, 4096, 1); self.relu7 = nn.ReLU(inplace=True); self.drop7 = nn.Dropout2d()
        self.score_fr = nn.Conv2d(4096, n_class, 1)
        self.upscore = nn.ConvTranspose2d(n_class, n_class, 64, stride=32, bias=False)
        self.seenmask_score = nn.Conv2d(4096, 2, 1)
        self.seenmask_upscore = nn.ConvTranspose2d(2, 2, 64, stride=32, bias=False)
        self._initialize_weights()
        for mod in self.modules():
            if isinstance(mod, nn.Conv2d):
                mod.weight.data = mod.weight.data.contiguous(memory_format=torch.channels_last)
        object.__setattr__(self, "_engine", _Engine(self))
        object.__setattr__(self, "_last_ctx", None)
        object.__setattr__(self, "_last_pred", None)
        object.__setattr__(self, "_last_group", None)
        object.__setattr__(self, "_last_margin", None)

    def _initialize_weights(self):
        for mod in self.modules():
            if isinstance(mod, nn.ConvTranspose2d):
                assert mod.kernel_size[0] == mod.kernel_size[1]
                mod.weight.data.copy_(get_upsampling_weight(mod.in_channels, mod.out_channels, mod.kernel_size[0]))

    def set_precision(self, dtype):
        self._engine.set_precision(dtype)
        return self

    def set_head_precision(self, kind):
        if kind not in ("native", "fp8", "fp8_bwd"):
            raise L.SznError("head precision must be 'native', 'fp8' or 'fp8_bwd'")
        self._engine.head_fp8 = kind in ("fp8", "fp8_bwd")
        self._engine.head_fp8_bwd = kind == "fp8_bwd"
        return self

    def load_synthetic(self, seed=1337, device=None):
        if device is None:
            sd = self.state_dict()
            for k, v in synth.make_params(self.n_class, seed).items():
                sd[k].copy_(torch.from_numpy(v))
        else:
            self.to(device)
            g = torch.Generator(device=device)
# ... 400 lines not shown
```

Before: 267.9 Mpixels/s.

## Fold conv1_1 weight gradient into conv1_2 dgrad kernel, skip its input-grad output

When conv1_2's backward data gradient feeds conv1_1, the regw dgrad kernel now computes conv1_1's weight gradient in place. It loads the 3-channel input patch, multiplies it with the gated output tile held in LDS using MFMA, and writes per-block partial sums to a slab that a small reduce kernel folds together. The full-resolution 64-channel din tensor is never written, and the separate conv1_1 wgrad pass that re-read it is dropped. In exchange the regw kernel carries extra loads, LDS traffic and registers, and the Python side gains a query that checks the fused path applies and otherwise falls back to the old route.

Result: no change. 270.1 Mpixels/s, median of 6 (+0.8%).

```diff
diff --git a/include/szn.h b/include/szn.h
--- a/include/szn.h
+++ b/include/szn.h
@@ -38,6 +38,7 @@
 typedef struct szn_call_result {
     int colsum_rows;
     float work_fraction;
+    int c11_fused;
 } szn_call_result_t;
 
 typedef struct {
@@ -63,6 +64,13 @@
     void* dw_lp;
     int dw_lp_dtype;
     szn_call_result_t* result;
+    const float* c11_x;
+    int c11_B, c11_H, c11_W, c11_pad;
+    int c11_cut_on;
+    int c11_cut[8];
+    void* c11_ws;
+    size_t c11_ws_bytes;
+    float* c11_dw;
 } szn_conv_desc_t;
 
 int szn_conv2d_fwd(const szn_conv_desc_t* d, const void* in, const void* w, const float* bias,
@@ -75,6 +83,7 @@
 
 int szn_conv2d_dgrad(const szn_conv_desc_t* d, const void* dout, const void* wT, const void* gate,
                      const float* chan_scale, void* din, szn_stream_t stream);
+int szn_conv2d_dgrad_c11_fusable(const szn_conv_desc_t* d);
 int szn_conv2d_dgrad_border_region(const szn_conv_desc_t* d, int region[8]);
 int szn_conv2d_dgrad_border_finish(const szn_conv_desc_t* d, const void* dout, const void* wT, const void* gate,
                                    const float* skip_sum, float* colsum, void* workspace, szn_stream_t stream);
diff --git a/zeroshotsemanticsegmentation_amd/_lib.py b/zeroshotsemanticsegmentation_amd/_lib.py
--- a/zeroshotsemanticsegmentation_amd/_lib.py
+++ b/zeroshotsemanticsegmentation_amd/_lib.py
@@ -15,7 +15,7 @@
 
 
 class CallResult(C.Structure):
-    _fields_ = [("colsum_rows", C.c_int), ("work_fraction", C.c_float)]
+    _fields_ = [("colsum_rows", C.c_int), ("work_fraction", C.c_float), ("c11_fused", C.c_int)]
 
 
 class ConvDesc(C.Structure):
@@ -24,11 +24,14 @@
         ("workspace", C.c_void_p), ("workspace_bytes", C.c_size_t), ("colsum", C.c_void_p), ("pool_out", C.c_void_p),
         ("colsum_slab", C.c_void_p), ("colsum_slab_rows", C.c_int), ("pool_code", C.c_void_p), ("pool_only", C.c_int),
         ("cb_on", C.c_int), ("cb_rect", C.c_int * 4), ("cb_const", C.c_int * 4), ("reserved_cus", C.c_int),
-        ("dw_lp", C.c_void_p), ("dw_lp_dtype", C.c_int), ("result", C.POINTER(CallResult))]
+        ("dw_lp", C.c_void_p), ("dw_lp_dtype", C.c_int), ("result", C.POINTER(CallResult)),
+        ("c11_x", C.c_void_p), ("c11_B", C.c_int), ("c11_H", C.c_int), ("c11_W", C.c_int), ("c11_pad", C.c_int),
+        ("c11_cut_on", C.c_int), ("c11_cut", C.c_int * 8), ("c11_ws", C.c_void_p), ("c11_ws_bytes", C.c_size_t),
+        ("c11_dw", C.c_void_p)]
 
     def __init__(self, *a, **kw):
         super().__init__(*a, **kw)
-        self.res = CallResult(0, 1.0)
+        self.res = CallResult(0, 1.0, 0)
         self.result = C.pointer(self.res)
 
 
@@ -96,6 +99,7 @@
     "szn_pack_weight_dgrad": (_I, [_I, _I, _I, _I, _I, _P, _P, _P]),
     "szn_pack_weight_dgrad_batch": (_I, [_I, _I, _P, _P, _P, _P, _P, _P]),
     "szn_conv2d_dgrad": (_I, [_D, _P, _P, _P, _P, _P, _P]),
+    "szn_conv2d_dgrad_c11_fusable": (_I, [_D]),
     "szn_conv2d_dgrad_border_region": (_I, [_D, _P]),
     "szn_conv2d_dgrad_border_finish": (_I, [_D, _P, _P, _P, _P, _P, _P, _P]),
     "szn_conv2d_dgrad_gemm_workspace_bytes": (C.c_size_t, [_D]),
diff --git a/zeroshotsemanticsegmentation_amd/csrc/szn_conv.hip b/zeroshotsemanticsegmentation_amd/csrc/szn_conv.hip
--- a/zeroshotsemanticsegmentation_amd/csrc/szn_conv.hip
+++ b/zeroshotsemanticsegmentation_amd/csrc/szn_conv.hip
@@ -600,6 +600,19 @@
     s.ldi = d->ldo; s.ldo = d->ldi;
     s.relu = 0;
     return szn_conv2d_fwd(&s, dout, wT, nullptr, gate, chan_scale, din, stream);
+}
+
+int szn_conv2d_c11_query(const szn_conv_desc_t* s);
+extern "C" int szn_conv2d_dgrad_c11_fusable(const szn_conv_desc_t* d) {
+    if (!d || !d->c11_x || check_desc(d) || d->KH != d->KW || d->KH - 1 - d->pad < 0) return 0;
+    szn_conv_desc_t s = *d;
+    s.Hi = d->Ho; s.Wi = d->Wo; s.Ci = d->Co;
+    s.Ho = d->Hi; s.Wo = d->Wi; s.Co = d->Ci;
+    s.pad = d->KH - 1 - d->pad;
+    s.ldi = d->ldo; s.ldo = d->ldi;
+    s.relu = 0;
+    s.result = nullptr;
+    return szn_conv2d_c11_query(&s);
 }
 
 template <typename T>
diff --git a/zeroshotsemanticsegmentation_amd/csrc/szn_conv1_1_wgrad.hip b/zeroshotsemanticsegmentation_amd/csrc/szn_conv1_1_wgrad.hip
--- a/zeroshotsemanticsegmentation_amd/csrc/szn_conv1_1_wgrad.hip
+++ b/zeroshotsemanticsegmentation_amd/csrc/szn_conv1_1_wgrad.hip
@@ -249,6 +249,12 @@
     if (ok && l == 0) dw[i] = accumulate ? dw[i] + s : s;
 }
 
+}
+
+int szn_conv1_1_wgrad_reduce_launch(const float* ws, float* dw, int nblocks, szn_stream_t stream) {
+    hipLaunchKernelGGL(conv1_1_wgrad_reduce, dim3(64 * 27 / 8), dim3(256), 0, (hipStream_t)stream, ws, dw, nblocks, 0);
+    SZN_CHECK_LAUNCH("conv1_1_wgrad_reduce");
+    return SZN_OK;
 }
 
 static bool c11_geometry(int dtype, int B, int H, int W, int pad, int& oh_lo, int& oh_hi, int& seg_lo, int& seg_hi) {
diff --git a/zeroshotsemanticsegmentation_amd/csrc/szn_conv_igemm.hip b/zeroshotsemanticsegmentation_amd/csrc/szn_conv_igemm.hip
--- a/zeroshotsemanticsegmentation_amd/csrc/szn_conv_igemm.hip
+++ b/zeroshotsemanticsegmentation_amd/csrc/szn_conv_igemm.hip
@@ -15,7 +15,7 @@
                       const float* chan_scale, void* out, unsigned in_bytes, unsigned w_bytes, int min_tiles,
                       float* ws, int nsplit, int chunks_per_split, szn_stream_t stream);
 int szn_conv_regw_try(const szn_conv_desc_t* d, const void* in, const void* w, const float* bias, const void* gate,
-                     const float* chan_scale, void* out, int min_tiles, szn_stream_t stream);
+                     const float* chan_scale, void* out, int min_tiles, szn_stream_t stream, int* c11_query = nullptr);
 #include <stdlib.h>
 
 namespace {
@@ -464,6 +464,7 @@
     if (!d) SZN_FAIL(SZN_ERR_ARG, "conv2d_fwd: null descriptor");
     szn_note_colsum_rows(0);
     szn_note_work_fraction(1.f);
+    if (d->result) d->result->c11_fused = 0;
     const int rc = conv2d_fwd_entry(d, in, w, bias, gate, chan_scale, out, stream);
     szn_publish_result(d);
     return rc;
@@ -481,6 +482,22 @@
     if (rc || !d->pool_out || pooled) return rc;
     return szn_maxpool2x2_ceil_fwd_code((d->out_f32 || szn_store_f32(d->dtype)) ? SZN_F32 : d->dtype, d->B, d->Ho, d->Wo, d->Co, out,
                                         d->pool_out, d->pool_code, stream);
+}
+
+static int regw_min_tiles() {
+    static const int regw_min = szn_knob("SZN_REGW_MINTILES", 128);
+    return regw_min;
+}
+
+int szn_conv2d_c11_query(const szn_conv_desc_t* s) {
+    if (!s->c11_x || !szn_is16(s->dtype) || s->KH != 3 || s->KW != 3 || s->Ci != 64 || s->Co != 64) return 0;
+    if (s->B <= 0 || s->Hi <= 0 || s->Wi <= 0 || s->pad < 0 || s->Ho != s->Hi + 2 * s->pad - 2 || s->Wo != s->Wi + 2 * s->pad - 2 ||
+        s->Ho <= 0 || s->Wo <= 0 || s->Hi >= 32000 || s->Wi >= 32000 || s->ldi < s->Ci || s->ldo < s->Co || ((size_t)s->ldi * 2) % 16 ||
+        (size_t)s->B * s->Hi * s->Wi * s->ldi * 2 >= 0x7fff0000ul || (long)s->B * s->Ho * s->Wo >= (1L << 31))
+        return 0;
+    int q = 0;
+    const int rc = szn_conv_regw_try(s, s, s, nullptr, s , nullptr, nullptr, regw_min_tiles(), nullptr, &q);
+    return rc == 0 && q;
 }
 
 static int conv2d_fwd_dispatch(const szn_conv_desc_t* d, const void* in, const void* w, const float* bias, const void* gate,
@@ -500,16 +517,16 @@
     if (!v2_ok) return szn_conv2d_fwd_v1(d, in, w, bias, gate, chan_scale, out, stream);
     if (d->B <= 0 || d->Hi <= 0 || d->Wi <= 0 || d->Co <= 0 || d->KH <= 0 || d->KW <= 0 || d->pad < 0 ||
         d->Ho != d->Hi + 2 * d->pad - d->KH + 1 || d->Wo != d->Wi + 2 * d->pad - d->KW + 1 || d->Ho <= 0 || d->Wo <= 0 ||
-        d->ldi < d->Ci || d->ldo < d->Co || !in || !w || !out || (((uintptr_t)in | (uintptr_t)w | (uintptr_t)out) & 15) ||
+        d->ldi < d->Ci || d->ldo < d->Co || !in || !w || (!out && !d->c11_x) || (((uintptr_t)in | (uintptr_t)w | (uintptr_t)out) & 15) ||
         (long)d->B * d->Ho * d->Wo >= (1L << 31))
         return szn_conv2d_fwd_v1(d, in, w, bias, gate, chan_scale, out, stream);
     hipStream_t st = (hipStream_t)stream;
     if (d->KH == 3 && d->KW == 3 && d->Ci <= 128 && d->Co <= 128) {
-        static const int regw_min = szn_knob("SZN_REGW_MINTILES", 128);
-        const int rc = szn_conv_regw_try(d, in, w, bias, gate, chan_scale, out, regw_min, stream);
+        const int rc = szn_conv_regw_try(d, in, w, bias, gate, chan_scale, out, regw_min_tiles(), stream);
         if (rc == 0 && d->pool_out) *pooled = 1;
         if (rc <= 0) return rc;
     }
+    if (!out) SZN_FAIL(SZN_ERR_ARG, "conv2d_dgrad: din is NULL and the call does not take the kernel that folds conv1_1's weight gradient in");
     Conv2Args a;
     a.in = (const char*)in; a.w = (const char*)w; a.bias = bias; a.gate = (const char*)gate; a.cscale = chan_scale;
     a.out = (char*)out; a.ws = nullptr; a.colsum = d->colsum;
diff --git a/zeroshotsemanticsegmentation_amd/csrc/szn_conv_regw.hip b/zeroshotsemanticsegmentation_amd/csrc/szn_conv_regw.hip
--- a/zeroshotsemanticsegmentation_amd/csrc/szn_conv_regw.hip
+++ b/zeroshotsemanticsegmentation_amd/csrc/szn_conv_regw.hip
@@ -23,6 +23,9 @@
     int B, Hi, Wi, Ho, Wo, pad;
     int ldi, ldo, ldg, relu;
     int tiles_x, tiles_y, ntiles;
+    const float* c11_x; float* c11_slab;
+    unsigned c11_xbytes;
+    int c11_H, c11_W, c11_iy0, c11_ix0, c11_wy0, c11_wy1, c11_wx0, c11_wx1;
 };
 
 constexpr unsigned kOOBr = 0x80000000u;
@@ -60,9 +63,10 @@
     static_assert(COG * CIG * PG == 8 && LDS <= 160 * 1024, "wave decomposition / LDS budget");
 };
 
-template <typename T, int COG, int CIG, bool GATED, bool COLSUM>
+template <typename T, int COG, int CIG, bool GATED, bool COLSUM, bool C11 = false>
 __global__ __launch_bounds__(512) void conv3x3_regw(RwArgs a) {
 #if defined(__HIP_DEVICE_COMPILE__)
+    static_assert(!C11 || (COG == 2 && CIG == 1 && GATED && COLSUM), "C11: the gated, column-summing 64 -> 64 instantiation only");
     typedef RwGeom<COG, CIG> G_;
     constexpr int PG = G_::PG, TR = G_::TR, PROWS = G_::PROWS, RB = G_::RB, CPR = G_::CPR, RPP = G_::RPP;
     constexpr int NPIECE = G_::NPIECE, SLOTS = G_::SLOTS, PATCHB = G_::PATCHB, NBUF = G_::NBUF, CO = G_::CO, CI = G_::CI;
@@ -78,6 +82,9 @@
     const int first = (int)((long)a.ntiles * vb / G), last = (int)((long)a.ntiles * (vb + 1) / G);
     if (first >= last) {
         if constexpr (COLSUM) { if (a.cslab && tid < CO) a.cslab[(long)blockIdx.x * CO + tid] = 0.f; }
+        if constexpr (C11) {
+            for (int idx = tid; idx < 2048; idx += 512) a.c11_slab[(size_t)blockIdx.x * 2048 + idx] = 0.f;
+        }
         return;
     }
 
@@ -154,6 +161,23 @@
             __builtin_amdgcn_raw_ptr_buffer_load_lds(rsA, (ldsptr_t)dst, 16, v, 0, 0, 0);
         }
     };
+
+    [[maybe_unused]] f32x4_t dwa[2][2];
+    [[maybe_unused]] int c11_la = 0, c11_lb[2] = {0, 0};
+    [[maybe_unused]] const auto rsX = __builtin_amdgcn_make_buffer_rsrc((void*)(C11 ? (const void*)a.c11_x : (const void*)a.in), 0, (int)(C11 ? a.c11_xbytes : 0u), 0x00020000);
+    if constexpr (C11) {
+#pragma unroll
+        for (int i = 0; i < 2; ++i)
+#pragma unroll
+            for (int f = 0; f < 2; ++f) dwa[i][f] = f32x4_t{0.f, 0.f, 0.f, 0.f};
+        const int q = r16 >> 2, p = r16 & 3;
+        c11_la = G_::OFF_GATE + w * (NJ * 1024) + (p >> 1) * 512 + (4 * g + q) * 16 + (p & 1) * 8;
+#pragma unroll
+        for (int f = 0; f < 2; ++f) {
+            const int t = r16 + 16 * f;
+            c11_lb[f] = G_::OFF_GATE + w * (NJ * 1024) + ((((t % 3) * 6 + t / 9) * PWr + (t / 3) % 3 + 4 * g) << 1);
+        }
+    }
 
     const int cstart = cog * 32 + (g & 1) * 16 + (g >> 1) * 8;
     const int qb = (pg * 4) * PWr + r16;
@@ -202,6 +226,27 @@
                 __builtin_amdgcn_raw_ptr_buffer_load_lds(rsG, (ldsptr_t)(smem + G_::OFF_GATE + (w * NJ + jj) * 1024), 16, v, 0, 0, 0);
             }
         }
+        [[maybe_unused]] bool touch = false, colin = false;
+        [[maybe_unused]] uint32_t xi[6];
+        if constexpr (C11) {
+            const int wy = ty * TR + pg * 4, x0 = tx * 16;
+            touch = wy < a.c11_wy1 && wy + 4 > a.c11_wy0 && x0 < a.c11_wx1 && x0 + 16 > a.c11_wx0;
+            colin = okw && ow >= a.c11_wx0 && ow < a.c11_wx1;
+            int lv = lane;
+            asm volatile("" : "+v"(lv));
+            const int r = (lv * 57) >> 10, c = lv - r * PWr;
+            const int ir = wy + a.c11_iy0 + r, ic = x0 + a.c11_ix0 + c;
+            const bool cok = touch && r < 3 && (unsigned)ic < (unsigned)a.c11_W;
+            const int e0 = (b * 3 * a.c11_H + ir) * a.c11_W + ic;
+#pragma unroll
+            for (int k = 0; k < 6; ++k) {
+                const int ci = k >> 1, dr = 3 * (k & 1);
+                const bool in = cok && (unsigned)(ir + dr) < (unsigned)a.c11_H;
+                const unsigned off = in ? (unsigned)(e0 + (ci * a.c11_H + dr) * a.c11_W) * 4u : kOOBr;
+                if (k == 0) asm volatile("s_nop 4\n\tbuffer_load_dword %0, %1, %2, 0 offen" : "=v"(xi[k]) : "v"(off), "s"(rsX) : "memory");
+                else asm volatile("buffer_load_dword %0, %1, %2, 0 offen" : "=v"(xi[k]) : "v"(off), "s"(rsX) : "memory");
+            }
+        }
         if (more) issue((buf + NBUF - 1) % NBUF);
 
         f32x4_t acc[2][4];
@@ -273,6 +318,8 @@
         *(f32x4_t*)&bv[4] = *(const f32x4_t*)(smem + G_::OFF_BIAS + cstart * 4 + 16);
         if (NBUF == 3 && more) asm volatile("s_waitcnt vmcnt(%0)" ::"i"(SLOTS) : "memory");
         else asm volatile("s_waitcnt vmcnt(0)" ::: "memory");
+        if constexpr (C11)
+            asm volatile("" : "+v"(xi[0]), "+v"(xi[1]), "+v"(xi[2]), "+v"(xi[3]), "+v"(xi[4]), "+v"(xi[5]));
         if (grpB) {
             asm volatile("s_waitcnt lgkmcnt(0)" ::: "memory");
             __builtin_amdgcn_s_barrier();
@@ -309,6 +356,12 @@
             pk.y = pack2<T>(v[2], v[3]);
             pk.z = pack2<T>(v[4], v[5]);
             pk.w = pack2<T>(v[6], v[7]);
+            if constexpr (C11) {
+                if (touch) {
+                    const bool in = ok && colin && oh0 + j >= a.c11_wy0 && oh0 + j < a.c11_wy1;
+                    *(u32x4_t*)(smem + G_::OFF_GATE + (w * NJ + j) * 1024 + lane * 16) = in ? pk : u32x4_t{0u, 0u, 0u, 0u};
+                }
+            } else
             if (!a.skip_x && !nostore)
                 __builtin_amdgcn_raw_buffer_store_b128(pk, rsO, ok ? ((m0 + j * a.Wo) * a.ldo + cstart) * 2u : kOOBst, 0, 0);
             if constexpr (!GATED) {
@@ -371,6 +424,52 @@
                 }
             }
         }
+        if constexpr (C11) {
+            if (touch) {
+                u32x2_t At[2][2][2];
+                const unsigned la = (unsigned)(uintptr_t)(ldsptr_t)smem + (unsigned)c11_la;
+#pragma unroll
+                for (int s = 0; s < 2; ++s)
+#pragma unroll
+                    for (int i = 0; i < 2; ++i)
+#pragma unroll
+                        for (int h = 0; h < 2; ++h)
+                            asm volatile("ds_read_b64_tr_b16 %0, %1 offset:%2" : "=v"(At[i][s][h]) : "v"(la), "i"((2 * s + h) * 1024 + i * 256) : "memory");
+                asm volatile("s_waitcnt lgkmcnt(0)"
+                             : "+v"(At[0][0][0]), "+v"(At[0][0][1]), "+v"(At[0][1][0]), "+v"(At[0][1][1]), "+v"(At[1][0][0]), "+v"(At[1][0][1]),
+                               "+v"(At[1][1][0]), "+v"(At[1][1][1])
+                             :: "memory");
+                u32x4_t Af[2][2];
+#pragma unroll
+                for (int s = 0; s < 2; ++s)
+#pragma unroll
+                    for (int i = 0; i < 2; ++i) Af[i][s] = u32x4_t{At[i][s][0].x, At[i][s][0].y, At[i][s][1].x, At[i][s][1].y};
+                uint16_t* tp = (uint16_t*)(smem + G_::OFF_GATE + w * (NJ * 1024));
+                if (lane < 3 * PWr) {
+#pragma unroll
+                    for (int k = 0; k < 6; ++k) tp[3 * PWr * k + lane] = to_bits16<T>(__uint_as_float(xi[k]));
+                }
+#pragma unroll
+                for (int f = 0; f < 2; ++f) {
+                    const bool tv = r16 + 16 * f < 27;
+                    const uint16_t* tq = (const uint16_t*)(smem + c11_lb[f]);
+#pragma unroll
+                    for (int s = 0; s < 2; ++s) {
+                        uint32_t bw[4];
+#pragma unroll
+                        for (int h = 0; h < 4; ++h) {
+                            const int o = (2 * s + (h >> 1)) * PWr + 2 * (h & 1);
+                            const uint32_t v = (uint32_t)tq[o] | ((uint32_t)tq[o + 1] << 16);
+                            bw[h] = tv ? v : 0u;
+                        }
+                        const u32x4_t Bf = {bw[0], bw[1], bw[2], bw[3]};
+#pragma unroll
+                        for (int i = 0; i < 2; ++i) dwa[i][f] = mfma16<T>(Af[i][s], Bf, dwa[i][f]);
+                    }
+                }
+                asm volatile("s_waitcnt lgkmcnt(0)" ::: "memory");
+            }
+        }
         if (!grpB) {
             asm volatile("s_waitcnt lgkmcnt(0)" ::: "memory");
             __builtin_amdgcn_s_barrier();
@@ -386,7 +485,25 @@
             const float x = row16_sum(cst[e]);
             if (r16 == 0) pw[(w * 4 + g) * 8 + e] = x;
         }
+        [[maybe_unused]] float* c11red = (float*)(smem + 4096);
+        if constexpr (C11) {
+#pragma unroll
+            for (int i = 0; i < 2; ++i)
+#pragma unroll
+                for (int f = 0; f < 2; ++f)
+#pragma unroll
+                    for (int e = 0; e < 4; ++e) c11red[(w * 32 + 16 * i + 4 * g + e) * 32 + 16 * f + r16] = dwa[i][f][e];
+        }
         __syncthreads();
+        if constexpr (C11) {
+            float* slab = a.c11_slab + (size_t)blockIdx.x * 2048;
+#pragma unroll
+            for (int k = 0; k < 4; ++k) {
+                const int idx = tid + 512 * k;
+                const float* rp = c11red + ((idx >> 10) * 32 + ((idx >> 5) & 31)) * 32 + (idx & 31);
+                slab[idx] = ((rp[0] + rp[2 * 1024]) + rp[4 * 1024]) + rp[6 * 1024];
+            }
+        }
         if (tid < CO) {
             const int cogc = tid >> 5, rem = tid & 31;
             const int gc = (((rem & 15) >> 3) << 1) | (rem >> 4), ec = rem & 7;
@@ -443,16 +560,16 @@
     }
 }
 
-template <typename T, int COG, int CIG, bool GATED, bool COLSUM>
+template <typename T, int COG, int CIG, bool GATED, bool COLSUM, bool C11 = false>
 int launch_regw(const RwArgs& a, int grid, hipStream_t st) {
     constexpr int lds = RwGeom<COG, CIG>::LDS;
     static bool attr_done = false;
     if (!attr_done) {
-        (void)hipFuncSetAttribute((const void*)conv3x3_regw<T, COG, CIG, GATED, COLSUM>, hipFuncAttributeMaxDynamicSharedMemorySize, lds);
+        (void)hipFuncSetAttribute((const void*)conv3x3_regw<T, COG, CIG, GATED, COLSUM, C11>, hipFuncAttributeMaxDynamicSharedMemorySize, lds);
         attr_done = true;
     }
-    hipLaunchKernelGGL((conv3x3_regw<T, COG, CIG, GATED, COLSUM>), dim3((unsigned)grid), dim3(512), lds, st, a);
-    SZN_CHECK_LAUNCH("conv3x3_regw");
+    hipLaunchKernelGGL((conv3x3_regw<T, COG, CIG, GATED, COLSUM, C11>), dim3((unsigned)grid), dim3(512), lds, st, a);
+    SZN_CHECK_LAUNCH(C11 ? "conv3x3_regw_c11" : "conv3x3_regw");
     return SZN_OK;
 }
 
@@ -478,8 +595,39 @@
     return c.per_image > 0 && (all - c.per_image) * 10 >= all;
 }
 
+int szn_conv1_1_wgrad_reduce_launch(const float* ws, float* dw, int nblocks, szn_stream_t stream);
+
+static bool regw_c11_plan(const szn_conv_desc_t* d, const float* bias, const void* gate, int grid, RwArgs& a) {
+    if (!d->c11_x || !d->c11_dw || !d->c11_ws || ((uintptr_t)d->c11_ws & 15)) return false;
+    if (!szn_is16(d->dtype) || d->Co != 64 || d->Ci != 64 || d->pad != 1 || !gate || !d->colsum || bias || d->relu || d->pool_out) return false;
+    const int B = d->c11_B, H = d->c11_H, W = d->c11_W, pad = d->c11_pad;
+    if (B != d->B || H <= 0 || W <= 0 || pad < 0) return false;
+    const int H1 = H + 2 * pad - 2, W1 = W + 2 * pad - 2;
+    if (H1 <= 0 || W1 <= 0 || (size_t)B * 3 * H * W * 4 >= 0x7fff0000ul) return false;
+    BandCut c = {0, 0, H1, H1, 0, 0, W1, W1};
+    if (d->c11_cut_on) {
+        const int* v = d->c11_cut;
+        c = BandCut{v[0], v[1], v[2], v[3], v[4], v[5], v[6], v[7]};
+        if (c.ya < 0 || c.ye < c.ya || c.ya2 < c.ye || c.ye2 < c.ya2 || c.ye2 > H1 || c.xa < 0 || c.xe < c.xa || c.xa2 < c.xe || c.xe2 < c.xa2 || c.xe2 > W1)
+            return false;
+    }
+    if (H1 - (c.ye - c.ya) - (c.ye2 - c.ya2) != d->Ho || W1 - (c.xe - c.xa) - (c.xe2 - c.xa2) != d->Wo) return false;
+    const int oh_lo = std::max(pad - 2, 0), oh_hi = std::min(pad + H, H1), ow_lo = std::max(pad - 2, 0), ow_hi = std::min(pad + W, W1);
+    if (oh_hi <= oh_lo || ow_hi <= ow_lo) return false;
+    if ((c.ye > c.ya && c.ye > oh_lo) || (c.ye2 > c.ya2 && c.ya2 < oh_hi) || (c.xe > c.xa && c.xe > ow_lo) || (c.xe2 > c.xa2 && c.xa2 < ow_hi))
+        return false;
+    const int dy = c.ye - c.ya, dx = c.xe - c.xa;
+    a.c11_wy0 = oh_lo - dy; a.c11_wy1 = oh_hi - dy; a.c11_wx0 = ow_lo - dx; a.c11_wx1 = ow_hi - dx;
+    if (a.cb.on && (a.c11_wy0 < a.cb.wy0 * 16 || a.c11_wy1 > a.cb.wy1 * 16 || a.c11_wx0 < a.cb.wx0 * 16 || a.c11_wx1 > a.cb.wx1 * 16))
+        return false;
+    if (d->c11_ws_bytes < (size_t)grid * 2048 * sizeof(float)) return false;
+    a.c11_x = d->c11_x; a.c11_slab = (float*)d->c11_ws; a.c11_xbytes = (unsigned)((size_t)B * 3 * H * W * 4);
+    a.c11_H = H; a.c11_W = W; a.c11_iy0 = dy - pad; a.c11_ix0 = dx - pad;
+    return true;
+}
+
 int szn_conv_regw_try(const szn_conv_desc_t* d, const void* in, const void* w, const float* bias, const void* gate,
-                      const float* chan_scale, void* out, int min_tiles, szn_stream_t stream) {
+                      const float* chan_scale, void* out, int min_tiles, szn_stream_t stream, int* c11_query) {
     if (!szn_is16(d->dtype) || d->KH != 3 || d->KW != 3 || d->pad > 2 || d->out_f32 || chan_scale) return 1;
     if ((d->Ci != 64 && d->Ci != 128) || (d->Co != 64 && d->Co != 128)) return 1;
     if ((d->ldo & 7) || (d->ldi & 7) || (gate && (d->ldg & 7))) return 1;
@@ -563,6 +711,21 @@
     hipStream_t st = (hipStream_t)stream;
     if (a.cslab && d->colsum_slab_rows < grid_cus) SZN_FAIL(SZN_ERR_ARG, "conv2d: colsum_slab holds %d rows, %d needed", d->colsum_slab_rows, grid_cus);
     szn_note_colsum_rows(a.cslab ? grid_cus : 0);
+    a.c11_x = nullptr; a.c11_slab = nullptr; a.c11_xbytes = 0u;
+    a.c11_H = a.c11_W = a.c11_iy0 = a.c11_ix0 = a.c11_wy0 = a.c11_wy1 = a.c11_wx0 = a.c11_wx1 = 0;
+    const bool c11 = regw_c11_plan(d, bias, gate, grid_cus, a);
+    if (c11_query) { *c11_query = c11 ? 1 : 0; return SZN_OK; }
+    if (!c11 && !out) return 1;
+    if (c11) {
+        a.out = nullptr; a.out_bytes = 0u;
+        int rc1 = d->dtype == SZN_F16 ? launch_regw<f16_raw, 2, 1, true, true, true>(a, grid_cus, st)
+                                      : launch_regw<bf16_raw, 2, 1, true, true, true>(a, grid_cus, st);
+        if (rc1) return rc1;
+        rc1 = szn_conv1_1_wgrad_reduce_launch(a.c11_slab, d->c11_dw, grid_cus, stream);
+        if (rc1) return rc1;
+        if (d->result) d->result->c11_fused = 1;
+        return SZN_OK;
+    }
     int rc;
     if (d->dtype == SZN_F16) {
         if (cog == 2 && cig == 1) rc = launch_regw_flags<f16_raw, 2, 1>(a, grid_cus, st);
diff --git a/zeroshotsemanticsegmentation_amd/models.py b/zeroshotsemanticsegmentation_amd/models.py
--- a/zeroshotsemanticsegmentation_amd/models.py
+++ b/zeroshotsemanticsegmentation_amd/models.py
@@ -215,6 +215,9 @@
         self._splitk_ws = None
         self._gemm_ws = None
         self._wg_ws = None
+        self.fuse_c11_wgrad = True
+        self.c11_fused_last = False
+        self._c11_ws = None
         self._wg_stream = None
         self._wg_masked = None
         self.keep_prepool = False
@@ -762,10 +765,10 @@
             if after is not None:
                 after()
 
-    def _dgrad(self, dout, name, in_shape, pad, gate=None, scale=None, colsum=None, wT=None, cb=None, border_sum=None):
+    def _dgrad(self, dout, name, in_shape, pad, gate=None, scale=None, colsum=None, wT=None, cb=None, border_sum=None, c11=None):
         B, Hi, Wi, Ci = in_shape
         Ho, Wo, Co = dout.shape[1:]
-        din = torch.empty(B, Hi, Wi, Ci, device=dout.device, dtype=self.dtype)
+        din = None if c11 is not None else torch.empty(B, Hi, Wi, Ci, device=dout.device, dtype=self.dtype)
         if wT is None and (name + ".wG") in self._images:
             if gate is not None or scale is not None or colsum is not None:
                 raise L.SznError("dgrad of %s: the GEMM form has no gate / scale / colsum epilogue" % name)
@@ -808,7 +811,24 @@
             d.cb_on = 2 if (border_sum is not None and colsum is not None) else 1
             for i in range(4):
                 d.cb_rect[i], d.cb_const[i] = grect[i], srect[i]
+        if c11 is not None:
+            ctx, dw = c11
+            if self._c11_ws is None or self._c11_ws.device != dout.device:
+                self._c11_ws = torch.empty(512 * 8192, dtype=torch.uint8, device=dout.device)
+            d.c11_x, d.c11_B, d.c11_H, d.c11_W, d.c11_pad = ctx.x.data_ptr(), ctx.B, ctx.H, ctx.W, PAD1
+            if ctx.crop and "c11cut" in ctx.crop:
+                d.c11_cut_on = 1
+                for i in range(8):
+                    d.c11_cut[i] = ctx.crop["c11cut"][i]
+            d.c11_ws, d.c11_ws_bytes, d.c11_dw = self._c11_ws.data_ptr(), self._c11_ws.numel(), dw.data_ptr()
+            if L.load().szn_conv2d_dgrad_c11_fusable(C.byref(d)) != 1:
+                d.c11_x = None
+                din = torch.empty(B, Hi, Wi, Ci, device=dout.device, dtype=self.dtype)
         L.call("szn_conv2d_dgrad", C.byref(d), L.ptr(dout), L.ptr(wT), L.ptr(gate), L.ptr(scale), L.ptr(din), L.stream_ptr())
+        if c11 is not None:
+            self.c11_fused_last = bool(d.res.c11_fused)
+            if (din is None) != self.c11_fused_last:
+                raise L.SznError("dgrad of %s: szn_conv2d_dgrad_c11_fusable and the call disagree" % name)
         cs_rows = d.res.colsum_rows
         if d.cb_on == 2 and d.res.work_fraction < 1.0:
             bws = torch.empty(2 * 24 * B * Co, device=dout.device)
@@ -953,6 +973,12 @@
             name, pad = item
             if name == "conv1_1":
                 dw, db = grads[name]
+                if d is None:
+                    with self._wgrad_stream(dw):
+                        if name in lp:
+                            L.call("szn_cast", L.SZN_F32, L.dtype_code(lp[name].dtype), dw.numel(), L.ptr(dw), L.ptr(lp[name]), L.stream_ptr())
+                        done(name)
+                    break
                 nb = L.load().szn_conv1_1_wgrad_workspace_bytes(code, ctx.B, ctx.H, ctx.W, PAD1)
                 ws = torch.empty(nb, dtype=torch.uint8, device=d.device)
                 with self._wgrad_stream(d, ws):
@@ -995,7 +1021,14 @@
                     d = d + side.to(d.dtype)
             else:
                 cb = self._conv1_1_dgrad_cb(ctx) if (prev[0] == "conv1_1" and not cropped_in) else None
-                d = self._dgrad(d, name, xin.shape, pad, gate=xin, colsum=grads[prev[0]][1], cb=cb, border_sum=border_sums.pop(name, None))
+                c11 = (ctx, grads["conv1_1"][0]) if (prev[0] == "conv1_1" and self.fuse_c11_wgrad and self.dtype != torch.float32 and
+                                                     (not cropped_in or "c11cut" in ctx.crop)) else None
+                if prev[0] == "conv1_1":
+                    self.c11_fused_last = False
+                d = self._dgrad(d, name, xin.shape, pad, gate=xin, colsum=grads[prev[0]][1], cb=cb, border_sum=border_sums.pop(name, None),
+                                c11=c11)
+                if d is None:
+                    continue
                 if cropped_in and "c11cut" not in ctx.crop:
                     band = ctx.crop[("in", name)][0]
                     d = self._band_remap(d, band, "crop_bwd", band.H, band.W)
```
